# joejep/FOCNeRF

Measured on AMD Instinct MI355X. Metric: train_samples_per_sec, higher is better.
Workload: dtype f16

## Files before the change

focnerf_amd/_lib.py:

```python
import ctypes
import os

import torch

_HERE = os.path.dirname(os.path.abspath(__file__))
LIB_PATH = os.environ.get("FOCNERF_LIB_PATH") or os.path.join(_HERE, "libfocnerf_hip.so")

c_u8p = ctypes.c_void_p
c_vp = ctypes.c_void_p
u32 = ctypes.c_uint32
u64 = ctypes.c_uint64
f32 = ctypes.c_float
f64 = ctypes.c_double
i32 = ctypes.c_int

FOC_F32 = 0
FOC_F16 = 1
FOC_U8 = 2


class FocOccTrainNode(ctypes.Structure):
    _fields_ = [
        ("struct_bytes", u32),
        ("n_rays", u32), ("max_steps", u32), ("cascade", u32), ("grid_size", u32), ("cap", u32), ("pad_align", u32),
# ... 153 lines not shown
                                                      u32, i32, u32, i32, i32, c_vp, c_vp, u64, c_vp]),
    "foc_grad_total_variation": (i32, [c_vp, c_vp, c_vp, c_vp, f32, u32, u32, u32, u32, f32, u32, u32, i32, i32, c_vp]),
    "foc_freq_encode_forward": (i32, [c_vp, u32, u32, u32, u32, c_vp, c_vp]),
    "foc_freq_encode_backward": (i32, [c_vp, c_vp, u32, u32, u32, u32, c_vp, c_vp]),
    "foc_ffmlp_forward": (i32, [c_vp, c_vp, u32, u32, u32, u32, u32, u32, u32, c_vp, c_vp, c_vp]),
    "foc_ffmlp_inference": (i32, [c_vp, c_vp, u32, u32, u32, u32, u32, u32, u32, c_vp, c_vp, c_vp]),
    "foc_ffmlp_backward": (i32, [c_vp, c_vp, c_vp, c_vp, u32, u32, u32, u32, u32, u32, u32, i32,
                                 c_vp, c_vp, c_vp, c_vp, u64, c_vp]),
    "foc_ffmlp_backward_workspace_bytes": (u64, [u32, u32, u32]),
    "foc_ffmlp_forward_planar": (i32, [c_vp, c_vp, u32, u32, u32, u32, u32, u32, u32, c_vp, c_vp]),
    "foc_ffmlp_backward_planar": (i32, [c_vp, c_vp, c_vp, u32, u32, u32, u32, u32, u32, u32, i32, c_vp, c_vp, c_vp, u64, c_vp]),
    "foc_allocate_splitk": (i32, [u64]),
    "foc_free_splitk": (i32, []),
    "foc_combine_select": (i32, [c_vp, c_vp, c_vp, c_vp, u64, c_vp]),
    "foc_combine_pack_keys": (i32, [c_vp, u32, c_vp, u64, c_vp]),
    "foc_combine_unpack": (i32, [c_vp, u32, c_vp, c_vp, c_vp, u64, c_vp]),
    "foc_combine_select_composite": (i32, [c_vp, u32, c_vp, c_vp, u32, u32, c_vp, u32, c_vp, c_vp, c_vp, c_vp]),
    "foc_combine_select4": (i32, [c_vp, c_vp, u64, c_vp]),
    "foc_combine_select_composite_attr": (i32, [c_vp, u32, c_vp, c_vp, u32, c_vp, c_vp, u32, u32, c_vp, u32, c_vp, c_vp, c_vp, c_vp, c_vp, c_vp, c_vp, c_vp]),
    "foc_combine_select_composite_culled": (i32, [ctypes.POINTER(FocCulledField), u32, u32, c_vp, u32, c_vp, c_vp, u32, u32, c_vp, u32, c_vp, c_vp, c_vp, c_vp,
                                                  c_vp, c_vp, c_vp, c_vp]),
    "foc_combine_select4_ids": (i32, [c_vp, u32, c_vp, c_vp, u64, c_vp]),
    "foc_mo_select": (i32, [c_vp, c_vp, c_vp, c_vp, u64, u32, u32, c_vp]),
    "foc_fixed_field_pack": (i32, [c_vp, c_vp, c_vp, c_vp, c_vp, c_vp, f32, u32, u32, f32, f32, c_vp, c_vp, c_vp, c_vp, u32, c_vp]),
    "foc_fixed_cull_scratch_bytes": (u64, [u32, u32]),
    "foc_fixed_cull": (i32, [c_vp, c_vp, c_vp, c_vp, c_vp, u32, u32, f32, c_vp, u32, u32, c_vp, c_vp, c_vp, c_vp, u64, c_vp]),
    "foc_fixed_cull_emit": (i32, [c_vp, c_vp, c_vp, c_vp, c_vp, u32, u32, f32, c_vp, c_vp, u32, c_vp, c_vp, c_vp]),
    "foc_fixed_field_pack_culled": (i32, [c_vp, c_vp, c_vp, c_vp, u32, c_vp, c_vp, u32, u32, f32, f32, c_vp, c_vp]),
    "foc_fixed_cull_placed": (i32, [c_vp, c_vp, c_vp, c_vp, c_vp, u32, u32, c_vp, c_vp, f32, c_vp, u32, u32, c_vp, c_vp, c_vp, c_vp, u64, c_vp]),
    "foc_fixed_cull_emit_placed": (i32, [c_vp, c_vp, c_vp, c_vp, c_vp, u32, u32, c_vp, f32, f32, c_vp, c_vp, u32, c_vp, c_vp, c_vp]),
    "foc_fixed_field_pack_culled_gain": (i32, [c_vp, c_vp, c_vp, c_vp, u32, c_vp, c_vp, u32, u32, f32, f32, f32, c_vp, c_vp]),
    "foc_composite_fixed_steps":(i32, [c_vp, c_vp, c_vp, c_vp, u32, u32, f32, c_vp, c_vp, c_vp]),
    "foc_fixed_sample": (i32, [c_vp, c_vp, c_vp, c_vp, c_vp, c_vp, u32, u32, f32, c_vp, c_vp, c_vp, u32, c_vp]),
    "foc_fixed_tail_forward": (i32, [c_vp, c_vp, c_vp, c_vp, c_vp, c_vp, f32, u32, u32, f32, f32, c_vp, c_vp, c_vp, c_vp, c_vp, c_vp, u32, c_vp, c_vp]),
    "foc_fixed_tail_backward": (i32, [c_vp, c_vp, c_vp, c_vp, c_vp, c_vp, c_vp, c_vp, c_vp, c_vp, c_vp, f32, u32, u32, f32, f32, c_vp, c_vp, u32, c_vp, c_vp]),
    "foc_fixed_tail_forward_dist": (i32, [c_vp, c_vp, c_vp, c_vp, c_vp, c_vp, f32, u32, u32, f32, f32, c_vp, c_vp, c_vp, c_vp, c_vp, c_vp, u32, c_vp, c_vp,
                                          c_vp, c_vp]),
    "foc_fixed_tail_backward_dist": (i32, [c_vp, c_vp, c_vp, c_vp, c_vp, c_vp, c_vp, c_vp, c_vp, c_vp, c_vp, c_vp, f32, u32, u32, f32, f32, c_vp, c_vp, u32,
                                           c_vp, c_vp, c_vp, c_vp, c_vp]),
    "foc_fixed_head_forward": (i32, [c_vp, c_vp, c_vp, c_vp, c_vp, u32, u32, f32, c_vp, c_vp, c_vp, c_vp, c_vp, c_vp, c_vp, u32, c_vp]),
    "foc_fixed_head_backward": (i32, [c_vp, c_vp, c_vp, c_vp, c_vp, c_vp, c_vp, c_vp, c_vp, c_vp, u32, u32, f32, c_vp, u32, c_vp]),
    "foc_color_head_forward": (i32, [c_vp, c_vp, u32, c_vp, u32, u32, u32, u32, c_vp, u32, c_vp, c_vp]),
    "foc_field_forward_train": (i32, [c_vp, c_vp, u32, c_vp, u32, c_vp, u32, u32, u32, u32, c_vp, c_vp, u32, c_vp, c_vp]),
    "foc_color_head_backward": (i32, [c_vp, c_vp, c_vp, u32, c_vp, c_vp, u32, u32, u32, u32, c_vp, c_vp, c_vp, u64, u32, c_vp, c_vp, c_vp]),
    "foc_color_head_forward_pad": (i32, [c_vp, c_vp, u32, c_vp, u32, u32, u32, u32, c_vp, u32, c_vp, f32, c_vp]),
    "foc_color_head_backward_pad": (i32, [c_vp, c_vp, c_vp, u32, c_vp, c_vp, u32, u32, u32, u32, c_vp, c_vp, c_vp, u64, u32, c_vp, c_vp, f32, c_vp]),
    "foc_field_forward_train_pad": (i32, [c_vp, c_vp, u32, c_vp, u32, c_vp, u32, u32, u32, u32, c_vp, c_vp, u32, c_vp, f32, c_vp]),
    "foc_color_head_forward_pad31": (i32, [c_vp, c_vp, u32, c_vp, u32, u32, u32, u32, c_vp, u32, c_vp, f32, c_vp]),
    "foc_color_head_backward_pad31": (i32, [c_vp, c_vp, c_vp, u32, c_vp, c_vp, u32, u32, u32, u32, c_vp, c_vp, c_vp, u64, u32, c_vp, c_vp, f32, c_vp]),
    "foc_field_forward_train_pad31": (i32, [c_vp, c_vp, u32, c_vp, u32, c_vp, u32, u32, u32, u32, c_vp, c_vp, u32, c_vp, f32, c_vp]),
    "foc_fixed_composite_forward": (i32, [c_vp, c_vp, c_vp, f32, u32, u32, f32, c_vp, c_vp]),
    "foc_fixed_composite_backward": (i32, [c_vp, c_vp, c_vp, c_vp, f32, u32, u32, f32, c_vp, c_vp, c_vp]),
    "foc_sample_head_forward": (i32, [c_vp, c_vp, u64, c_vp, c_vp, c_vp, u32, c_vp]),
    "foc_sample_head_backward": (i32, [c_vp, c_vp, c_vp, u64, c_vp, u32, c_vp]),
    "foc_sh_encode": (i32, [c_vp, u64, c_vp, c_vp]),
    "foc_rgb_head_forward": (i32, [c_vp, u64, c_vp, c_vp]),
    "foc_rgb_head_backward": (i32, [c_vp, c_vp, u64, c_vp, c_vp]),
    "foc_fixed_render_inference": (i32, [c_vp, c_vp, c_vp, c_vp, c_vp, c_vp, f32, u32, u32, f32, f32, c_vp, c_vp, c_vp, c_vp, u32, c_vp, c_vp]),
    "foc_nerf_field_inference": (i32, [c_vp, i32, c_vp, u32, u32, u32, c_vp, u32, c_vp, u32, u32, u32, u32, c_vp, c_vp, c_vp, c_vp]),
    "foc_nerf_field_inference_pad": (i32, [c_vp, i32, c_vp, u32, u32, u32, c_vp, u32, c_vp, u32, u32, u32, u32, c_vp, c_vp, c_vp, f32, c_vp]),
    "foc_nerf_field_inference_pad31": (i32, [c_vp, i32, c_vp, u32, u32, u32, c_vp, u32, c_vp, u32, u32, u32, u32, c_vp, c_vp, c_vp, f32, c_vp]),
    "foc_field_normals": (i32, [c_vp, u32, c_vp, c_vp, u32, u32, u32, f32, u32, u32, i32, u32, i32, c_vp, c_vp, u32, u32, u32, c_vp, c_vp, c_vp, c_vp, c_vp,
                                c_vp]),
    "foc_mark_untrained_grid": (i32, [c_vp, u32, f32, f32, f32, f32, f32, u32, u32, c_vp, c_vp, c_vp]),
    "foc_grid_cells_xyz": (i32, [u32, u32, f32, c_vp, c_vp, c_vp]),
    "foc_grid_update_sample_workspace_bytes": (u64, [u32, u32]),
    "foc_grid_update_sample": (i32, [c_vp, u32, u32, f32, u32, c_vp, c_vp, c_vp, c_vp, c_vp, c_vp, u64, c_vp]),
    "foc_grid_update_apply_workspace_bytes": (u64, [u32, u32]),
    "foc_grid_update_apply": (i32, [c_vp, u32, u32, c_vp, c_vp, u32, f32, f32, f32, c_vp, c_vp, c_vp, u64, c_vp]),
    "foc_background_forward": (i32, [c_vp, c_vp, c_vp, f32, u32, c_vp, c_vp, f32, u32, c_vp, c_vp, c_vp]),
    "foc_background_backward_workspace_bytes": (u64, [u32]),
    "foc_background_backward": (i32, [c_vp, c_vp, c_vp, c_vp, f32, u32, c_vp, c_vp, f32, u32, c_vp, c_vp, c_vp, c_vp, u64, c_vp]),
    "foc_mc_workspace_bytes": (u64, [u32, u32, u32]),
    "foc_mc_count": (i32, [c_vp, u32, u32, u32, f32, c_vp, c_vp, c_vp]),
    "foc_mc_emit": (i32, [c_vp, u32, u32, u32, f32, c_vp, c_vp, c_vp, c_vp, c_vp, c_vp, c_vp]),
    "foc_lattice_cull_scratch_bytes": (u64, [u32]),
    "foc_lattice_cull": (i32, [c_vp, c_vp, c_vp, u32, u32, u32, u32, u32, c_vp, c_vp, f32, c_vp, u32, u32, c_vp, c_vp, c_vp, c_vp, u64, c_vp]),
    "foc_lattice_cull_emit": (i32, [c_vp, c_vp, c_vp, u32, u32, u32, u32, u32, c_vp, c_vp, c_vp, u32, c_vp, c_vp]),
    "foc_volume_scatter_max": (i32, [c_vp, c_vp, c_vp, f32, c_vp, u32, c_vp]),
    "foc_score_workspace_bytes": (u64, [u32, u32, u32]),
    "foc_score_quantize": (i32, [c_vp, c_vp, c_vp, c_vp, u32, u32, u32, c_vp, c_vp, c_vp, c_vp]),
    "foc_score_view": (i32, [c_vp, c_vp, u32, u32, u32, c_vp, u32, f64, f64, c_vp, c_vp, u64, c_vp]),
    "foc_optim_workspace_bytes": (ctypes.c_size_t, [i32]),
# ... 16 lines not shown
    try:
        lib = ctypes.CDLL(LIB_PATH)
    except OSError as e:
        raise ImportError(f"focnerf_amd: failed to load {LIB_PATH}: {e}") from e
    for name, (res, args) in SIGNATURES.items():
        fn = getattr(lib, name)
        fn.restype = res
        fn.argtypes = args
    return lib


class _Stream(ctypes.c_void_p):
    device_index = None


_multi_device = None


def _on_tensor_device(fn):
    def call(*args):
        global _multi_device
        if _multi_device is None:
            _multi_device = torch.cuda.device_count() > 1
        if _multi_device and args:
            idx = getattr(args[-1], "device_index", None)
            if idx is not None and idx != torch.cuda.current_device():
                with torch.cuda.device(idx):
                    return fn(*args)
        return fn(*args)
    call.__name__ = getattr(fn, "__name__", "foc_call")
    return call


class _Lib:

    def __init__(self, cdll):
        self._cdll = cdll
        for name, (_, args) in SIGNATURES.items():
            fn = getattr(cdll, name)
            setattr(self, name, _on_tensor_device(fn) if args and args[-1] is c_vp and not name.endswith("_bytes") else fn)


lib = _Lib(_load())


def check(rc, what=""):
    if rc != 0:
        msg = lib.foc_last_error().decode("utf-8", "replace")
        raise RuntimeError(f"focnerf_amd {what}: {msg} (code {rc})")


def ptr(t):
    if t is None:
        return None
    return ctypes.c_void_p(t.data_ptr())


_raw_stream = getattr(torch._C, "_cuda_getCurrentRawStream", None) if os.environ.get("FOC_RAW_STREAM", "1") != "0" else None


def raw_stream(index):
    if _raw_stream is not None:
        return _raw_stream(index)
    return torch.cuda.current_stream(index).cuda_stream


def stream_of(t=None):
    dev = t.device if t is not None else None
    index = dev.index if dev is not None and dev.index is not None else torch.cuda.current_device()
    s = _Stream(raw_stream(index))
    s.device_index = index
    return s

# ... 39 lines not shown
```

focnerf_amd/csrc/combine.hip:

```cpp
#include "common.h"
#include "fs_common.h"
#include <string.h>
#include <cmath>

static thread_local char g_err[512] = "";

void foc_set_error(const char *fmt, ...) {
    va_list ap;
    va_start(ap, fmt);
    vsnprintf(g_err, sizeof(g_err), fmt, ap);
    va_end(ap);
}

__global__ void __launch_bounds__(256) k_combine_select(const float *__restrict__ dens, const float *__restrict__ rgb,
                                                        float *__restrict__ max_dens, float *__restrict__ best_rgb, uint64_t n) {
    for (uint64_t i = (uint64_t)blockIdx.x * 256 + threadIdx.x; i < n; i += (uint64_t)gridDim.x * 256) {
        const float d = dens[i], m = max_dens[i];
        if (d > m) { best_rgb[i * 3] = rgb[i * 3]; best_rgb[i * 3 + 1] = rgb[i * 3 + 1]; best_rgb[i * 3 + 2] = rgb[i * 3 + 2]; }
        max_dens[i] = (d != d || m != m) ? __builtin_nanf("") : (d > m ? d : m);
    }
}

__global__ void __launch_bounds__(256) k_combine_pack(const float *__restrict__ dens, uint32_t rank, uint64_t *__restrict__ keys, uint64_t n) {
    for (uint64_t i = (uint64_t)blockIdx.x * 256 + threadIdx.x; i < n; i += (uint64_t)gridDim.x * 256) {
// ... 327 lines not shown
        best.x = (f.x != f.x || m != m) ? __builtin_nanf("") : (f.x > m ? f.x : m);
        acc4[i] = best;
    }
}

template <typename T>
__global__ void __launch_bounds__(256) k_mo_select(const T *__restrict__ sig_new, const T *__restrict__ feat_new, T *__restrict__ sig_best,
                                                   T *__restrict__ feat_best, uint64_t n, uint32_t width) {
    const uint64_t s0 = ((uint64_t)blockIdx.x * 4u + (threadIdx.x >> 6)) * 64u;
    if (s0 >= n) return;
    const uint32_t lane = threadIdx.x & 63u;
    bool take = false;
    if (s0 + lane < n) {
        const T a_raw = sig_new[s0 + lane];
        const float a = (float)a_raw, b = (float)sig_best[s0 + lane];
        take = (a != a) || (b == b && a >= b);
        if (take) sig_best[s0 + lane] = a_raw;
    }
    const uint64_t rows = __ballot(take);
    const uint32_t live = (uint32_t)(n - s0 < 64u ? n - s0 : 64u);
    const uint64_t base = s0 * width;
    for (uint32_t e = lane; e < live * width; e += 64u)
        if ((rows >> (e / width)) & 1ull) feat_best[base + e] = feat_new[base + e];
}

#include <stdlib.h>
#include <string.h>
#include <atomic>
#include <mutex>
struct FocOptionRow { const char *name; std::atomic<int> value; };
static FocOptionRow foc_option_table[FOC_OPT_COUNT] = {
    {"FOC_MLP_BWD_FUSED", 1}, {"FOC_FIELD_FWD_FUSED", 1}, {"FOC_GB_MERGE_MAX_RES", 480}, {"FOC_GB_FACTORED", 1}, {"FOC_GB_TAIL_SPLIT", 16}, {"FOC_GRID_FUSE_SMALL", 1},
    {"FOC_GRID_PAIRS", 1}, {"FOC_GRID_FAST", 1}, {"FOC_MARCH_SERIAL", -1}, {"FOC_MARCH_RAYS_ROW_MAX", 131072}, {"FOC_OCC_MARCH_FORM", -1},
    {"FOC_OCC_SAMPLE_MAJOR", 1}, {"FOC_OCC_FIELD_PIECE", 1 << 23}, {"FOC_DETERMINISTIC", 0},
};
static int foc_option_parse(int which, const char *text) {
    if (which == FOC_OPT_OCC_MARCH_FORM) {
        if (text[0] == 't') return 0;
        if (text[0] == 'r') return 1;
        if (text[0] == 'l') return 2;
        if (text[0] == 's') return 3;
    }
    return atoi(text);
}
static void foc_options_init() {
    static std::once_flag once;
    std::call_once(once, [] {
        for (int i = 0; i < FOC_OPT_COUNT; i++) {
            const char *e = getenv(foc_option_table[i].name);
            if (e && e[0]) foc_option_table[i].value.store(foc_option_parse(i, e), std::memory_order_relaxed);
        }
    });
}
int foc_opt(FocOpt which) { foc_options_init(); return foc_option_table[which].value.load(std::memory_order_relaxed); }

extern "C" {

int foc_set_option(const char *name, int value) {
    foc_options_init();
    for (int i = 0; i < FOC_OPT_COUNT; i++)
        if (name && strcmp(name, foc_option_table[i].name) == 0) { foc_option_table[i].value.store(value, std::memory_order_relaxed); return FOC_OK; }
    foc_set_error("set_option: unknown option '%s'", name ? name : "(null)");
    return FOC_E_INVALID;
}

int foc_get_option(const char *name, int *value) {
    foc_options_init();
// ... 213 lines not shown
```

focnerf_amd/csrc/common.h:

```cpp
#pragma once
#include <hip/hip_runtime.h>
#include <hip/hip_fp16.h>
#include <stdint.h>
#include <stdio.h>
#include <stdarg.h>
#include "../../include/focnerf.h"

#define FOC_WAVE 64

void foc_set_error(const char *fmt, ...);

enum FocOpt {
    FOC_OPT_MLP_BWD_FUSED,
    FOC_OPT_FIELD_FWD_FUSED,
    FOC_OPT_GB_MERGE_MAX_RES,
    FOC_OPT_GB_FACTORED,
    FOC_OPT_GB_TAIL_SPLIT,
    FOC_OPT_GRID_FUSE_SMALL,
    FOC_OPT_GRID_PAIRS,
    FOC_OPT_GRID_FAST,
    FOC_OPT_MARCH_SERIAL,
    FOC_OPT_MARCH_RAYS_ROW_MAX,
    FOC_OPT_OCC_MARCH_FORM,
    FOC_OPT_OCC_SAMPLE_MAJOR,
    FOC_OPT_OCC_FIELD_PIECE,
    FOC_OPT_DETERMINISTIC,
    FOC_OPT_COUNT
};
int foc_opt(FocOpt which);

#define FOC_REQUIRE(cond, code, ...)                    \
    do {                                                \
        if (!(cond)) {                                  \
            foc_set_error(__VA_ARGS__);                 \
            return (code);                              \
        }                                               \
    } while (0)

#define FOC_CHECK_LAUNCH(name)                                                     \
    do {                                                                           \
        hipError_t e_ = hipGetLastError();                                         \
        if (e_ != hipSuccess) {                                                    \
            foc_set_error("%s: launch failed: %s", name, hipGetErrorString(e_));   \
            return FOC_E_LAUNCH;                                                   \
        }                                                                          \
    } while (0)

static inline int foc_guard_pick(bool stream_is_null, int stream_device, int pointer_device, int current_device) {
    if (!stream_is_null && stream_device >= 0) return stream_device;
    if (pointer_device >= 0) return pointer_device;
    return current_device;
}
struct FocDeviceGuard {
    int prev = -1;
    explicit FocDeviceGuard(void *stream, const void *first_pointer = nullptr) {
        static int n_devices = -1;
        if (n_devices < 0 && hipGetDeviceCount(&n_devices) != hipSuccess) { (void)hipGetLastError(); n_devices = 0; }
        if (n_devices == 1) return;
        int cur = 0;
// ... 83 lines not shown
```

focnerf_amd/csrc/ffmlp.hip:

```cpp
#include "common.h"
#include "activations.h"
#include <stdlib.h>

#include <type_traits>
#include "mlp_common.h"

template <int HIDDEN, int NB, bool TRAIN, int IMODE, bool GEN = false>
__global__ void __launch_bounds__(MLP_BLOCK, 2) k_mlp_fwd(const _Float16 *__restrict__ inputs, const _Float16 *__restrict__ weights,
                                                       _Float16 *__restrict__ fwd_buf, _Float16 *__restrict__ outputs,
                                                       uint32_t B, uint32_t in_dim, uint32_t num_layers, int act, MlpHead hd) {
    const int relu = act == FOC_ACT_RELU;
    constexpr int MT = (HIDDEN + 31) / 32, KC = HIDDEN / 16;
    constexpr bool planar = IMODE == 1;
    extern __shared__ __attribute__((aligned(16))) _Float16 lds[];
    const uint32_t KS0 = IMODE == 2 ? 2u : in_dim / 16;
    const uint32_t f_hidden = MT * KS0, f_out = f_hidden + (num_layers - 1) * MT * KC;
    const float *obj_bias = reinterpret_cast<const float *>(lds + (size_t)(f_out + KC) * 512);
    if constexpr (IMODE == 2) {
        stage_weights_fwd<HIDDEN>(weights, lds, in_dim, num_layers, true, head_ld0(hd));
        if (head_bias(hd)) stage_head_bias(weights, hd, const_cast<float *>(obj_bias), HIDDEN);
    } else stage_weights_fwd<HIDDEN>(weights, lds, in_dim, num_layers);
    __syncthreads();

    const uint32_t lane = threadIdx.x & 63, wave = threadIdx.x >> 6;
// ... 301 lines not shown
                    if (!(o < OUT)) av = u32x4{0u, 0u, 0u, 0u};
                    if (!(i < IN)) bv = u32x4{0u, 0u, 0u, 0u};
                    acc[t] = mfma16(__builtin_bit_cast(h8, av), __builtin_bit_cast(h8, bv), acc[t]);
                }
            }
        }
    }
#pragma unroll
    for (int t = 0; t < 4; t++) {
        const uint32_t tile = wave + t * MLP_WAVES + 16 * blockIdx.z;
        if (tile < n_out_tiles) {
            const uint32_t mt = tile / NTi, nt = tile % NTi;
            const uint32_t i = 32 * nt + r;
#pragma unroll
            for (int reg = 0; reg < 16; reg++) {
                const uint32_t o = 32 * mt + acc_row(reg, h);
                if (o < OUT && i < IN) (void)__hip_atomic_fetch_add(ws + ws_off + (uint64_t)o * IN + i, acc[t][reg], __ATOMIC_RELAXED, __HIP_MEMORY_SCOPE_AGENT);
            }
        }
    }
}

__global__ void __launch_bounds__(256) k_mlp_dw_finalize(const float *__restrict__ ws, _Float16 *__restrict__ gw, uint32_t n) {
    for (uint32_t i = blockIdx.x * 256 + threadIdx.x; i < n; i += gridDim.x * 256) gw[i] = (_Float16)ws[i];
}
__global__ void __launch_bounds__(256) k_mlp_dw_finalize_slots(const float *__restrict__ ws, uint32_t slots, uint64_t stride, _Float16 *__restrict__ gw, uint32_t n) {
    for (uint32_t i = blockIdx.x * 256 + threadIdx.x; i < n; i += gridDim.x * 256) {
        float v = 0.0f;
        for (uint32_t k = 0; k < slots; k++) v += ws[k * stride + i];
        gw[i] = (_Float16)v;
    }
}

template <int HIDDEN, int NL, int NB, bool RECOMP, int IMODE, bool RELU_CT, bool IN32 = false, bool LEAN = false>
__global__ void __launch_bounds__(MLP_BLOCK, 2) k_mlp_bwd_fused(const _Float16 *__restrict__ grad, const _Float16 *__restrict__ inputs,
                                                             const _Float16 *__restrict__ weights, const _Float16 *__restrict__ fwd_buf,
                                                             _Float16 *__restrict__ bwd_buf_arg, _Float16 *__restrict__ grad_inputs, float *__restrict__ ws,
                                                             uint32_t B, uint32_t in_dim, int relu_rt, uint32_t lds_w_halfs, MlpHead hd) {
    const int relu = RELU_CT ? 1 : relu_rt;
    f16v FZ;
#pragma unroll
    for (int e = 0; e < 16; e++) FZ[e] = 0.0f;
    constexpr int MT = (HIDDEN + 31) / 32, KC = HIDDEN / 16, RW = 32 * NB;
    constexpr bool planar = IMODE == 1, HEAD = IMODE >= 2, NARROW = IMODE == 3;
    static_assert(!HEAD || RECOMP, "the head input modes have no stored-activation form");
    constexpr int WD = (HIDDEN < 32 ? 32 : HIDDEN) + 8;
    extern __shared__ __attribute__((aligned(16))) _Float16 lds[];
    const bool with_dx = LEAN ? true : grad_inputs != nullptr;
    _Float16 *const bwd_buf = LEAN ? nullptr : bwd_buf_arg;
    uint32_t ld0 = in_dim;
    bool has_obj = false;
    if constexpr (HEAD) { ld0 = head_ld0(hd); has_obj = hd.obj != nullptr; }
    bool col31_set = false;
    _Float16 col31 = (_Float16)0.0f;
    if constexpr (HEAD) { col31_set = head_bias(hd); col31 = has_obj ? (_Float16)1.0f : (_Float16)hd.pad; }
    stage_weights_bwd<HIDDEN>(weights, lds, in_dim, NL, with_dx, HEAD, ld0);
    const uint32_t WA = (in_dim > (uint32_t)HIDDEN ? in_dim : (uint32_t)(HIDDEN < 32 ? 32 : HIDDEN)) + 8;
    _Float16 *sD = lds + lds_w_halfs;
    _Float16 *sA = sD + 4 * RW * WD;
    _Float16 *ldsF = sA + 4 * RW * WA;
    const float *obj_bias = reinterpret_cast<const float *>(ldsF + (size_t)(((HIDDEN + 31) / 32) * (in_dim / 16) + (NL - 1) * ((HIDDEN + 31) / 32) * (HIDDEN / 16)) * 512);
    if constexpr (RECOMP) {
        stage_weights_fwd<HIDDEN>(weights, ldsF, in_dim, NL, false, ld0);
        if constexpr (HEAD) { if (head_bias(hd)) stage_head_bias(weights, hd, const_cast<float *>(obj_bias), HIDDEN); }
    }
    __syncthreads();

    const uint32_t lane = threadIdx.x & 63, wave = threadIdx.x >> 6;
    const int c = lane & 31, h = lane >> 5;
    const uint32_t MT0 = (HEAD || IN32) ? 1u : (in_dim + 31) / 32;
    const uint32_t f_hidden = MT, f_dx = MT + (NL - 1) * MT * KC;
    _Float16 *myD = sD + wave * RW * WD, *myA = sA + wave * RW * WA;

    f16v dwacc[NL + 1];
#pragma unroll
    for (int s = 0; s <= NL; s++)
#pragma unroll
        for (int e = 0; e < 16; e++) dwacc[s][e] = 0.0f;

    const uint32_t rows_per_group = 4 * RW;
    const uint32_t n_groups = (B + rows_per_group - 1) / rows_per_group;
    constexpr int KS0M = (HEAD || IN32) ? 2 : 4;
    const uint32_t KS0 = HEAD ? 2u : in_dim / 16;
    h8 g_nxt[(RW * 2 + 63) / 64];
    h8 x_nxt[KS0M][NB];
    _Float16 h0_nxt[NB];
    uint32_t hx_nxt[NB];
    static_assert((RW * 2) % 64 == 0, "a wave's grad rows are whole 64-lane passes");
    auto fetch_group = [&](uint32_t grp) {
        const uint64_t r0 = (uint64_t)grp * rows_per_group + wave * RW;
        if constexpr (HEAD) {
#pragma unroll
            for (int nb = 0; nb < NB; nb++) {
                const uint64_t row = min(r0 + nb * 32 + c, (uint64_t)B - 1);
                const _Float16 *p = hd.grad_h0 ? hd.grad_h0 + row : grad;
                h0_nxt[nb] = *p;
            }
// ... 334 lines not shown
                        }
            }
            __builtin_amdgcn_s_setprio(0);
#ifndef FOC_TIMING_NO_BARRIER
            foc_lds_barrier();
#endif
        }
    }
    float *slot = ws + (uint64_t)blockIdx.x * ((NL + 1) * MLP_DW_SLOT_STAGE);
    float *meet = reinterpret_cast<float *>(sD);
#pragma unroll
    for (int s = 0; s <= NL; s++) {
        const uint32_t OUT = s == 0 ? 16u : (uint32_t)HIDDEN;
        const uint32_t IN = s < NL ? (uint32_t)HIDDEN : in_dim;
        const uint32_t ntile = ((OUT + 31) / 32) * ((IN + 31) / 32), ksplit = (ntile * 2 <= 4) ? 2u : 1u;
        if (ksplit == 2u) {
            __syncthreads();
            if (wave >= ntile && wave < 2u * ntile) {
#pragma unroll
                for (int reg = 0; reg < 16; reg++) meet[((wave - ntile) * 16 + reg) * 64 + lane] = dwacc[s][reg];
            }
            __syncthreads();
            if (wave < ntile) {
#pragma unroll
                for (int reg = 0; reg < 16; reg++) slot[(s * 4 + wave) * 1024 + reg * 64 + lane] = dwacc[s][reg] + meet[(wave * 16 + reg) * 64 + lane];
            }
        } else if (wave < ntile) {
#pragma unroll
            for (int reg = 0; reg < 16; reg++) slot[(s * 4 + wave) * 1024 + reg * 64 + lane] = dwacc[s][reg];
        }
    }
}

template <int HIDDEN>
__global__ void __launch_bounds__(1024) k_mlp_dw_reduce(const float *__restrict__ slots, uint32_t n_slots, uint32_t NL, uint32_t in_dim, uint32_t ld0,
                                                        _Float16 *__restrict__ gw, float *__restrict__ wsb) {
    __shared__ float part[16][64];
    const uint32_t lane = threadIdx.x & 63, slice = threadIdx.x >> 6;
    const uint32_t s = blockIdx.x / 64, w = (blockIdx.x / 16) % 4, reg = blockIdx.x % 16;
    const uint32_t OUT = s == 0 ? 16u : (uint32_t)HIDDEN, IN = s < NL ? (uint32_t)HIDDEN : in_dim;
    const uint32_t NTi = (IN + 31) / 32, MTo = (OUT + 31) / 32, ntile = MTo * NTi, ksplit = 1u;
    if (w >= ntile) return;
    const uint32_t mt = w / NTi, nt = w % NTi, h = lane >> 5;
    const uint32_t o = 32 * mt + (uint32_t)acc_row((int)reg, (int)h), i = 32 * nt + (lane & 31);
    if (!(o < OUT) && !(32 * mt + (uint32_t)acc_row((int)reg, 1 - (int)h) < OUT)) return;
    const uint64_t stride = (uint64_t)(NL + 1) * MLP_DW_SLOT_STAGE;
    const float *p = slots + (uint64_t)(s * 4 + w) * 1024 + reg * 64 + lane;
    float a0 = 0.f, a1 = 0.f, a2 = 0.f, a3 = 0.f;
    for (uint32_t k = 0; k < ksplit; k++) {
        const float *q = p + (uint64_t)k * ntile * 1024;
        uint32_t g = slice;
        for (; g + 48 < n_slots; g += 64) {
            a0 += q[(uint64_t)g * stride]; a1 += q[(uint64_t)(g + 16) * stride]; a2 += q[(uint64_t)(g + 32) * stride]; a3 += q[(uint64_t)(g + 48) * stride];
        }
        for (; g < n_slots; g += 16) a0 += q[(uint64_t)g * stride];
    }
    part[slice][lane] = (a0 + a1) + (a2 + a3);
    __syncthreads();
    if (slice == 0 && o < OUT && i < IN) {
        float v = 0.f;
#pragma unroll
        for (int k = 0; k < 16; k++) v += part[k][lane];
        const uint64_t first = (uint64_t)HIDDEN * ld0, lsz = (uint64_t)HIDDEN * HIDDEN;
        const uint32_t fl = NL - s;
        const uint64_t off = (s == 0 ? first + (uint64_t)(NL - 1) * lsz : (fl == 0 ? 0 : first + (uint64_t)(fl - 1) * lsz)) + (uint64_t)o * (s == NL ? ld0 : IN) + i;
        if (wsb) wsb[off] = v; else gw[off] = (_Float16)v;
    }
}

__global__ void __launch_bounds__(256) k_mlp_dw_finalize_obj(const float *__restrict__ ws, _Float16 *__restrict__ gw, uint32_t n, uint32_t hidden,
                                                             const _Float16 *__restrict__ W, const _Float16 *__restrict__ obj, float *__restrict__ grad_obj,
                                                             float pad) {
    const uint32_t n0 = hidden * HEAD_OBJ_LD;
    for (uint32_t i = blockIdx.x * 256 + threadIdx.x; i < n; i += gridDim.x * 256) {
        float v = ws[i];
        if (i < n0) {
            const uint32_t o = i / HEAD_OBJ_LD, col = i % HEAD_OBJ_LD;
            if (col >= 31) v = col < 47 ? ws[o * HEAD_OBJ_LD + 31] * (float)obj[col - 31] : (pad != 0.0f ? ws[o * HEAD_OBJ_LD + 31] * pad : 0.0f);
        }
        gw[i] = (_Float16)v;
    }
    if (blockIdx.x == 0 && threadIdx.x < 16 && grad_obj) {
        float a = 0.0f;
        for (uint32_t o = 0; o < hidden; o++) a = fmaf((float)W[o * HEAD_OBJ_LD + 31 + threadIdx.x], ws[o * HEAD_OBJ_LD + 31], a);
        grad_obj[threadIdx.x] = a;
    }
}

__device__ __forceinline__ void nf_sh16_half(float x, float y, float z, int h, h8 &out) {
    const float xy = x * y, xz = x * z, yz = y * z, x2 = x * x, y2 = y * y, z2 = z * z;
    float o[8];
    if (h == 0) {
        o[0] = 0.28209479177387814f; o[1] = -0.48860251190291987f * y; o[2] = 0.48860251190291987f * z; o[3] = -0.48860251190291987f * x;
        o[4] = 1.0925484305920792f * xy; o[5] = -1.0925484305920792f * yz; o[6] = 0.94617469575755997f * z2 - 0.31539156525251999f;
        o[7] = -1.0925484305920792f * xz;
    } else {
        o[0] = 0.54627421529603959f * x2 - 0.54627421529603959f * y2; o[1] = 0.59004358992664352f * y * (-3.0f * x2 + y2);
        o[2] = 2.8906114426405538f * xy * z; o[3] = 0.45704579946446572f * y * (1.0f - 5.0f * z2);
        o[4] = 0.3731763325901154f * z * (5.0f * z2 - 3.0f); o[5] = 0.45704579946446572f * x * (1.0f - 5.0f * z2);
// ... 277 lines not shown
    if (lds > 64 * 1024) (void)hipFuncSetAttribute(reinterpret_cast<const void *>(kern), hipFuncAttributeMaxDynamicSharedMemorySize, (int)lds);
    const uint32_t n_tiles = foc_div_up(B, 32 * NB);
    uint32_t grid = foc_div_up(n_tiles, MLP_WAVES);
    const uint32_t cap = mlp_num_cus() * mlp_resident_blocks(reinterpret_cast<const void *>(kern), lds);
    if (grid > cap) grid = cap;
    hipLaunchKernelGGL(kern, dim3(grid), dim3(MLP_BLOCK), lds, st, (const _Float16 *)inputs, (const _Float16 *)weights, (_Float16 *)fwd_buf,
                       (_Float16 *)outputs, B, in_dim, num_layers, act, head ? *head : MlpHead{nullptr, nullptr, 1u, 16u, nullptr, 0.0f});
    FOC_CHECK_LAUNCH(TRAIN ? "ffmlp_forward" : "ffmlp_inference");
    return FOC_OK;
}

template <bool TRAIN>
static int mlp_fwd(const void *inputs, const void *weights, uint32_t B, uint32_t input_dim, uint32_t output_dim, uint32_t hidden_dim,
                   uint32_t num_layers, uint32_t activation, uint32_t output_activation, void *buffer, void *outputs, void *stream, int planar = 0) {
    const char *who = TRAIN ? "ffmlp_forward" : "ffmlp_inference";
    int rc = mlp_check(who, B, input_dim, output_dim, hidden_dim, num_layers, activation, output_activation);
    if (rc) return rc;
    if (B == 0) return FOC_OK;
    FOC_REQUIRE(inputs && weights && outputs && (!TRAIN || buffer), FOC_E_INVALID, "%s: null pointer", who);
    const int act = (int)activation;
    hipStream_t st = (hipStream_t)stream;
    switch (hidden_dim) {
        case 16: return mlp_fwd_launch<16, TRAIN>(inputs, weights, B, input_dim, num_layers, act, buffer, outputs, planar, st);
        case 32: return mlp_fwd_launch<32, TRAIN>(inputs, weights, B, input_dim, num_layers, act, buffer, outputs, planar, st);
        case 64: return mlp_fwd_launch<64, TRAIN>(inputs, weights, B, input_dim, num_layers, act, buffer, outputs, planar, st);
        case 128: return mlp_fwd_launch<128, TRAIN>(inputs, weights, B, input_dim, num_layers, act, buffer, outputs, planar, st);
        case 256:
            FOC_REQUIRE(!planar, FOC_E_INVALID, "%s: planar inputs are served up to hidden_dim 128", who);
            return mlp_wide_forward(TRAIN, inputs, weights, B, input_dim, 256, num_layers, act, buffer, outputs, st);
    }
    return FOC_E_INVALID;
}

template <int HIDDEN, int NL>
static int mlp_bwd_fused_launch(const void *grad, const void *inputs, const void *weights, const void *fwd_buf, uint32_t B, uint32_t in_dim, int relu,
                                void *bwd_buf, void *grad_inputs, void *grad_weights, float *ws, int planar, hipStream_t st, const MlpHead *head = nullptr,
                                float *grad_obj = nullptr) {
    FOC_REQUIRE(!planar || fwd_buf == nullptr, FOC_E_INVALID, "ffmlp_backward: planar inputs need the re-evaluating form (forward_buffer NULL)");
    constexpr int NB = 1, RW = 32 * NB, WD = (HIDDEN < 32 ? 32 : HIDDEN) + 8;
    const bool dx = grad_inputs != nullptr;
    const size_t lds_w = mlp_bwd_lds<HIDDEN>(in_dim, NL, dx);
    const uint32_t WA = (in_dim > (uint32_t)HIDDEN ? in_dim : (uint32_t)(HIDDEN < 32 ? 32 : HIDDEN)) + 8;
    const bool recomp = fwd_buf == nullptr;
    constexpr int MT = (HIDDEN + 31) / 32, KC = HIDDEN / 16;
    const bool has_obj = head && head->obj;
    const size_t lds = lds_w + (size_t)4 * RW * (WD + WA) * sizeof(_Float16) + (recomp ? (size_t)(MT * (in_dim / 16) + (NL - 1) * MT * KC) * 1024 : 0) +
                       (head && head_bias(*head) ? 256 : 0);
    FOC_REQUIRE(lds <= 160 * 1024, FOC_E_INVALID, "ffmlp_backward: fused kernel needs %zu B of LDS", lds);
#ifdef FOC_TIMING_ONE_WG
    const size_t lds_launch = lds < 84 * 1024 ? 84 * 1024 : lds;
#else
    const size_t lds_launch = lds;
#endif
    auto kern = recomp ? (planar ? (relu ? k_mlp_bwd_fused<HIDDEN, NL, NB, true, 1, true> : k_mlp_bwd_fused<HIDDEN, NL, NB, true, 1, false>)
                                 : (relu ? k_mlp_bwd_fused<HIDDEN, NL, NB, true, 0, true> : k_mlp_bwd_fused<HIDDEN, NL, NB, true, 0, false>))
                       : k_mlp_bwd_fused<HIDDEN, NL, NB, false, 0, false>;
    const bool lean = !bwd_buf && dx;
    if constexpr (HIDDEN == 64) {
        if (recomp && relu && in_dim <= 32 && !head) {
            if (lean) kern = planar ? k_mlp_bwd_fused<HIDDEN, NL, NB, true, 1, true, true, true> : k_mlp_bwd_fused<HIDDEN, NL, NB, true, 0, true, true, true>;
            else kern = planar ? k_mlp_bwd_fused<HIDDEN, NL, NB, true, 1, true, true> : k_mlp_bwd_fused<HIDDEN, NL, NB, true, 0, true, true>;
        }
    }
    if constexpr (HIDDEN == 64 && NL >= 2 && NL <= 3) {
        if (head) kern = head->out_width == 4u ? (relu ? (lean ? k_mlp_bwd_fused<HIDDEN, NL, NB, true, 3, true, false, true> : k_mlp_bwd_fused<HIDDEN, NL, NB, true, 3, true>)
                                                       : k_mlp_bwd_fused<HIDDEN, NL, NB, true, 3, false>)
                                               : (relu ? (lean ? k_mlp_bwd_fused<HIDDEN, NL, NB, true, 2, true, false, true> : k_mlp_bwd_fused<HIDDEN, NL, NB, true, 2, true>)
                                                       : k_mlp_bwd_fused<HIDDEN, NL, NB, true, 2, false>);
    }
    else FOC_REQUIRE(!head, FOC_E_INVALID, "color_head_backward: hidden_dim must be 64 and num_layers 2 or 3");
    if (lds_launch > 64 * 1024) (void)hipFuncSetAttribute(reinterpret_cast<const void *>(kern), hipFuncAttributeMaxDynamicSharedMemorySize, (int)lds_launch);
    const uint32_t n_w = HIDDEN * ((has_obj ? HEAD_OBJ_LD : in_dim) + HIDDEN * (NL - 1) + 16);
    uint32_t grid = foc_div_up(B, 4 * RW);
    const uint32_t cap = min(mlp_num_cus() * 2, MLP_DW_MAX_SLOTS);
    if (grid > cap) grid = cap;
    float *slots = ws + mlp_dw_blob_floats(has_obj ? HEAD_OBJ_LD : in_dim, HIDDEN, NL);
    hipLaunchKernelGGL(kern, dim3(grid), dim3(MLP_BLOCK), lds_launch, st, (const _Float16 *)grad, (const _Float16 *)inputs, (const _Float16 *)weights,
                       (const _Float16 *)fwd_buf, (_Float16 *)bwd_buf, (_Float16 *)grad_inputs, slots, B, in_dim, relu, (uint32_t)(lds_w / sizeof(_Float16)),
                       head ? *head : MlpHead{nullptr, nullptr, 1u, 16u, nullptr, 0.0f});
    FOC_CHECK_LAUNCH("ffmlp_backward(fused)");
    hipLaunchKernelGGL((k_mlp_dw_reduce<HIDDEN>), dim3((NL + 1) * 64), dim3(1024), 0, st, (const float *)slots, grid, (uint32_t)NL, in_dim,
                       has_obj ? (uint32_t)HEAD_OBJ_LD : in_dim, (_Float16 *)grad_weights, has_obj ? ws : (float *)nullptr);
    FOC_CHECK_LAUNCH("ffmlp_backward(reduce)");
    if (has_obj) {
        hipLaunchKernelGGL(k_mlp_dw_finalize_obj, dim3(foc_grid_1d(n_w, 256)), dim3(256), 0, st, ws, (_Float16 *)grad_weights, n_w, (uint32_t)HIDDEN,
                           (const _Float16 *)weights, head->obj, grad_obj, head->pad);
        FOC_CHECK_LAUNCH("ffmlp_backward(finalize)");
    }
    return FOC_OK;
}

template <int HIDDEN>
static int mlp_dw_launch(const void *grad, const void *inputs, const void *fwd_buf, const void *bwd_buf, uint32_t B, uint32_t in_dim, uint32_t num_layers,
                         void *grad_weights, float *ws, bool det, hipStream_t st) {
    const uint32_t n_w = HIDDEN * (in_dim + HIDDEN * (num_layers - 1) + 16);
    const uint64_t det_stride = det ? mlp_dw_blob_floats(in_dim, HIDDEN, num_layers) : 0;
    uint32_t gx = foc_div_up(B, DW_CHUNK);
    if (det && gx > MLP_DW_DET_SLOTS) gx = MLP_DW_DET_SLOTS;
    if (foc_zero_async(ws, det ? (size_t)gx * det_stride * sizeof(float) : (size_t)n_w * sizeof(float), st) != hipSuccess) { foc_set_error("ffmlp_backward: memset of workspace failed"); return FOC_E_LAUNCH; }
    const int wgs_per_cu = 8;
    const uint32_t tiles = ((HIDDEN + 31) / 32) * ((max((uint32_t)HIDDEN, in_dim) + 31) / 32), GZ = (tiles + 15) / 16;
    const uint32_t capx = foc_div_up(mlp_num_cus() * (uint32_t)wgs_per_cu, (num_layers + 1) * GZ);
    if (gx > capx) gx = capx;
    if (gx < 1) gx = 1;
    auto kern = k_mlp_dw<HIDDEN>;
    if constexpr (HIDDEN <= 128) { if (in_dim > 128) kern = k_mlp_dw<HIDDEN, 256>; }
    hipLaunchKernelGGL(kern, dim3(gx, num_layers + 1, GZ), dim3(MLP_BLOCK), 0, st, (const _Float16 *)grad, (const _Float16 *)inputs,
                       (const _Float16 *)fwd_buf, (const _Float16 *)bwd_buf, ws, B, in_dim, num_layers, det_stride);
    FOC_CHECK_LAUNCH("ffmlp_backward(weights)");
    if (det) hipLaunchKernelGGL(k_mlp_dw_finalize_slots, dim3(foc_grid_1d(n_w, 256)), dim3(256), 0, st, ws, gx, det_stride, (_Float16 *)grad_weights, n_w);
    else hipLaunchKernelGGL(k_mlp_dw_finalize, dim3(foc_grid_1d(n_w, 256)), dim3(256), 0, st, ws, (_Float16 *)grad_weights, n_w);
    FOC_CHECK_LAUNCH("ffmlp_backward(finalize)");
    return FOC_OK;
}

// ... 256 lines not shown
                "color_head_backward: workspace of %llu bytes, foc_ffmlp_backward_workspace_bytes(%u, 64, %u) asks for %llu", (unsigned long long)workspace_bytes,
                obj_feat ? HEAD_OBJ_LD : 32u, num_layers, (unsigned long long)foc_ffmlp_backward_workspace_bytes(obj_feat ? HEAD_OBJ_LD : 32u, 64, num_layers));
    FOC_REQUIRE(out_width == 16 || out_width == 4, FOC_E_INVALID, "color_head_backward: out_width must be 16 or 4 (got %u)", out_width);
    FOC_REQUIRE(activation == FOC_ACT_RELU || activation == FOC_ACT_NONE, FOC_E_INVALID, "color_head_backward: hidden activation must be relu(0) or none(6)");
    rc = head_pad_check("color_head_backward", pad31, obj_feat, input_pad);
    if (rc) return rc;
    const MlpHead hd{(const _Float16 *)ray_sh, (const _Float16 *)grad_h0, samples_per_ray, out_width, (const _Float16 *)obj_feat, input_pad};
    const int relu = activation == 0;
    if (num_layers == 2) return mlp_bwd_fused_launch<64, 2>(grad, h, weights, nullptr, B, 32, relu, nullptr, grad_h, grad_weights, (float *)workspace, 0, (hipStream_t)stream, &hd, grad_obj);
    return mlp_bwd_fused_launch<64, 3>(grad, h, weights, nullptr, B, 32, relu, nullptr, grad_h, grad_weights, (float *)workspace, 0, (hipStream_t)stream, &hd, grad_obj);
}

int foc_color_head_backward(const void *grad, const void *h, const void *ray_sh, uint32_t samples_per_ray, const void *grad_h0, const void *weights,
                            uint32_t B, uint32_t hidden_dim, uint32_t num_layers, uint32_t activation, void *grad_h, void *grad_weights, void *workspace,
                            uint64_t workspace_bytes, uint32_t out_width, const void *obj_feat, float *grad_obj, void *stream) {
    return color_head_backward(grad, h, ray_sh, samples_per_ray, grad_h0, weights, B, hidden_dim, num_layers, activation, grad_h, grad_weights, workspace,
                               workspace_bytes, out_width, obj_feat, grad_obj, 0.0f, false, stream);
}

int foc_color_head_backward_pad(const void *grad, const void *h, const void *ray_sh, uint32_t samples_per_ray, const void *grad_h0, const void *weights,
                                uint32_t B, uint32_t hidden_dim, uint32_t num_layers, uint32_t activation, void *grad_h, void *grad_weights, void *workspace,
                                uint64_t workspace_bytes, uint32_t out_width, const void *obj_feat, float *grad_obj, float input_pad, void *stream) {
    return color_head_backward(grad, h, ray_sh, samples_per_ray, grad_h0, weights, B, hidden_dim, num_layers, activation, grad_h, grad_weights, workspace,
                               workspace_bytes, out_width, obj_feat, grad_obj, input_pad, false, stream);
}

int foc_color_head_backward_pad31(const void *grad, const void *h, const void *ray_sh, uint32_t samples_per_ray, const void *grad_h0, const void *weights,
                                  uint32_t B, uint32_t hidden_dim, uint32_t num_layers, uint32_t activation, void *grad_h, void *grad_weights, void *workspace,
                                  uint64_t workspace_bytes, uint32_t out_width, const void *obj_feat, float *grad_obj, float input_pad, void *stream) {
    return color_head_backward(grad, h, ray_sh, samples_per_ray, grad_h0, weights, B, hidden_dim, num_layers, activation, grad_h, grad_weights, workspace,
                               workspace_bytes, out_width, obj_feat, grad_obj, input_pad, true, stream);
}

int foc_allocate_splitk(uint64_t size) { (void)size; return FOC_OK; }
int foc_free_splitk(void) { return FOC_OK; }

}
```

focnerf_amd/csrc/field_fwd.hip:

```cpp
#include "mlp_common.h"

typedef uint32_t ff_u2 __attribute__((ext_vector_type(2)));

__device__ __forceinline__ uint32_t ff_pack(float a, float b) {
    typedef _Float16 h2 __attribute__((ext_vector_type(2)));
    const h2 p = {(_Float16)a, (_Float16)b};
    return __builtin_bit_cast(uint32_t, p);
}

#ifndef FF_MIN_WAVES
#define FF_MIN_WAVES 2
#endif
template <int NLS, int NLC, bool RELU>
__global__ void __launch_bounds__(MLP_BLOCK, FF_MIN_WAVES) k_field_fwd_train(const _Float16 *__restrict__ planes, const _Float16 *__restrict__ w_sigma,
                                                               const _Float16 *__restrict__ w_color, _Float16 *__restrict__ h_out,
                                                               _Float16 *__restrict__ c_out, uint32_t B, MlpHead hd) {
    constexpr int HIDDEN = 64, MT = 2, KC = 4, KS0 = 2;
    constexpr int FS = MT * KS0 + (NLS - 1) * MT * KC + KC;
    constexpr int FC = MT * KS0 + (NLC - 1) * MT * KC + KC;
    extern __shared__ __attribute__((aligned(16))) _Float16 lds[];
    _Float16 *ldsS = lds, *ldsC = lds + FS * 512;
    const float *obj_bias = reinterpret_cast<const float *>(ldsC + FC * 512);
    stage_weights_fwd<HIDDEN>(w_sigma, ldsS, 32, NLS);
    stage_weights_fwd<HIDDEN>(w_color, ldsC, 32, NLC, true, head_ld0(hd));
    if (head_bias(hd)) stage_head_bias(w_color, hd, const_cast<float *>(obj_bias), HIDDEN);
    __syncthreads();

    const uint32_t lane = threadIdx.x & 63, wave = threadIdx.x >> 6;
    const int c = lane & 31, h = lane >> 5;
    const uint32_t n_tiles = (B + 31) / 32;
    const uint32_t tstride = gridDim.x * MLP_WAVES;
    uint32_t tile = blockIdx.x * MLP_WAVES + wave;
    h8 x_nxt[KS0], sh_nxt;
    auto fetch = [&](uint32_t t) {
#ifdef FF_TIMING_NO_LOAD
        const uint64_t r = (uint64_t)c + 0 * t;
#else
        const uint64_t r = min((uint64_t)min(t, n_tiles - 1u) * 32 + c, (uint64_t)B - 1);
#endif
#pragma unroll
        for (int kc = 0; kc < KS0; kc++) x_nxt[kc] = ld_planar8(planes, B, r, kc, h);
        sh_nxt = ld_head8(planes, hd, r, 0, h);
    };
    fetch(tile);
    for (; tile < n_tiles; tile += tstride) {
#ifndef FF_TIMING_HOIST
        asm volatile("" ::: "memory");
#endif
        const uint64_t row_raw = (uint64_t)tile * 32 + c;
        h8 x_cur[KS0];
#pragma unroll
        for (int kc = 0; kc < KS0; kc++) x_cur[kc] = x_nxt[kc];
        const h8 sh = sh_nxt;
        fetch(tile + tstride);
        f16v acc[MT];
#pragma unroll
        for (int mt = 0; mt < MT; mt++)
#pragma unroll
// ... 56 lines not shown
            if (l < (uint32_t)NLC) {
                const uint32_t fbase = MT * KS0 + (l - 1) * MT * KC;
#pragma unroll
                for (int mt = 0; mt < MT; mt++)
#pragma unroll
                    for (int e = 0; e < 16; e++) acc[mt][e] = 0.0f;
#pragma unroll
                for (int kc = 0; kc < KC; kc++)
#pragma unroll
                    for (int mt = 0; mt < MT; mt++) acc[mt] = mfma16(ld_frag(ldsC, fbase + mt * KC + kc, lane), bf[kc], acc[mt]);
            } else {
#pragma unroll
                for (int e = 0; e < 16; e++) o[e] = 0.0f;
#pragma unroll
                for (int kc = 0; kc < KC; kc++) o = mfma16(ld_frag(ldsC, FC - KC + kc, lane), bf[kc], o);
                if (hd.out_width == 4u) {
#ifdef FF_TIMING_NO_STORE
                    if (h == 0 && row_raw == 0xFFFFFFFFFFull) *reinterpret_cast<ff_u2 *>(c_out + row_raw * 4) = ff_u2{ff_pack(o[0], o[1]), ff_pack(o[2], o[3])};
#else
                    if (h == 0 && row_raw < B) *reinterpret_cast<ff_u2 *>(c_out + row_raw * 4) = ff_u2{ff_pack(o[0], o[1]), ff_pack(o[2], o[3])};
#endif
                } else store_tile<false>(c_out, 16, row_raw, B, 0, 16, o, h);
            }
        }
    }
}

static uint32_t ff_num_cus() {
    int dev = 0, n = 0;
    if (hipGetDevice(&dev) != hipSuccess || hipDeviceGetAttribute(&n, hipDeviceAttributeMultiprocessorCount, dev) != hipSuccess || n <= 0) n = 256;
    return (uint32_t)n;
}

template <int NLS, int NLC, bool RELU>
static int ff_launch(const void *planes, const void *w_sigma, const void *w_color, void *h, void *c, uint32_t B, const MlpHead &hd, hipStream_t st) {
    auto kern = k_field_fwd_train<NLS, NLC, RELU>;
    const size_t lds = (size_t)((4 + (NLS - 1) * 8 + 4) + (4 + (NLC - 1) * 8 + 4)) * 1024 + 256;
    if (lds > 64 * 1024) (void)hipFuncSetAttribute(reinterpret_cast<const void *>(kern), hipFuncAttributeMaxDynamicSharedMemorySize, (int)lds);
    static int resident = 0;
    if (!resident) {
        int n = 0;
        if (hipOccupancyMaxActiveBlocksPerMultiprocessor(&n, kern, MLP_BLOCK, lds) != hipSuccess || n < 1) n = 2;
        resident = n > 8 ? 8 : n;
    }
    uint32_t grid = foc_div_up(foc_div_up(B, 32), MLP_WAVES);
    const uint32_t cap = ff_num_cus() * (uint32_t)resident;
    if (grid > cap) grid = cap;
    hipLaunchKernelGGL(kern, dim3(grid), dim3(MLP_BLOCK), lds, st, (const _Float16 *)planes, (const _Float16 *)w_sigma, (const _Float16 *)w_color,
                       (_Float16 *)h, (_Float16 *)c, B, hd);
    FOC_CHECK_LAUNCH("field_forward_train");
    return FOC_OK;
}

template <int NLS, int NLC>
static int ff_launch_act(const void *planes, const void *w_sigma, const void *w_color, void *h, void *c, uint32_t B, int relu, const MlpHead &hd, hipStream_t st) {
    return relu ? ff_launch<NLS, NLC, true>(planes, w_sigma, w_color, h, c, B, hd, st) : ff_launch<NLS, NLC, false>(planes, w_sigma, w_color, h, c, B, hd, st);
}

int field_forward_train(const void *planes, const void *sigma_weights, uint32_t sigma_layers, const void *ray_sh, uint32_t samples_per_ray,
                        const void *color_weights, uint32_t color_layers, uint32_t hidden_dim, uint32_t activation, uint32_t B, void *h, void *c,
                        uint32_t out_width, const void *obj_feat, float input_pad, bool pad31, void *stream) {
    FocDeviceGuard foc_guard_(stream, planes);
    if (B == 0) return FOC_OK;
    FOC_REQUIRE(planes && sigma_weights && ray_sh && color_weights && h && c, FOC_E_INVALID, "field_forward_train: null pointer");
    FOC_REQUIRE(hidden_dim == 64 && samples_per_ray >= 1, FOC_E_INVALID, "field_forward_train: hidden_dim must be 64 (got %u), samples_per_ray >= 1", hidden_dim);
    FOC_REQUIRE(activation == FOC_ACT_RELU || activation == FOC_ACT_NONE, FOC_E_INVALID, "field_forward_train: hidden activation must be relu(0) or none(6)");
    FOC_REQUIRE(out_width == 16 || out_width == 4, FOC_E_INVALID, "field_forward_train: out_width must be 16 or 4 (got %u)", out_width);
    const int prc = head_pad_check("field_forward_train", pad31, obj_feat, input_pad);
    if (prc) return prc;
    const MlpHead hd{(const _Float16 *)ray_sh, nullptr, samples_per_ray, out_width, (const _Float16 *)obj_feat, input_pad};
    const int relu = activation == FOC_ACT_RELU;
    hipStream_t st = (hipStream_t)stream;
    switch (sigma_layers * 10 + color_layers) {
        case 12: return ff_launch_act<1, 2>(planes, sigma_weights, color_weights, h, c, B, relu, hd, st);
        case 13: return ff_launch_act<1, 3>(planes, sigma_weights, color_weights, h, c, B, relu, hd, st);
        case 22: return ff_launch_act<2, 2>(planes, sigma_weights, color_weights, h, c, B, relu, hd, st);
        case 23: return ff_launch_act<2, 3>(planes, sigma_weights, color_weights, h, c, B, relu, hd, st);
        case 33: return ff_launch_act<3, 3>(planes, sigma_weights, color_weights, h, c, B, relu, hd, st);
        default: foc_set_error("field_forward_train: layer counts (%u, %u) are not built (1/2, 1/3, 2/2, 2/3, 3/3)", sigma_layers, color_layers); return FOC_E_INVALID;
    }
}

extern "C" {

int foc_field_forward_train(const void *planes, const void *sigma_weights, uint32_t sigma_layers, const void *ray_sh, uint32_t samples_per_ray,
                            const void *color_weights, uint32_t color_layers, uint32_t hidden_dim, uint32_t activation, uint32_t B, void *h, void *c,
                            uint32_t out_width, const void *obj_feat, void *stream) {
    return field_forward_train(planes, sigma_weights, sigma_layers, ray_sh, samples_per_ray, color_weights, color_layers, hidden_dim, activation, B, h, c,
                               out_width, obj_feat, 0.0f, false, stream);
}

int foc_field_forward_train_pad(const void *planes, const void *sigma_weights, uint32_t sigma_layers, const void *ray_sh, uint32_t samples_per_ray,
                                const void *color_weights, uint32_t color_layers, uint32_t hidden_dim, uint32_t activation, uint32_t B, void *h, void *c,
                                uint32_t out_width, const void *obj_feat, float input_pad, void *stream) {
    return field_forward_train(planes, sigma_weights, sigma_layers, ray_sh, samples_per_ray, color_weights, color_layers, hidden_dim, activation, B, h, c,
                               out_width, obj_feat, input_pad, false, stream);
}

int foc_field_forward_train_pad31(const void *planes, const void *sigma_weights, uint32_t sigma_layers, const void *ray_sh, uint32_t samples_per_ray,
                                  const void *color_weights, uint32_t color_layers, uint32_t hidden_dim, uint32_t activation, uint32_t B, void *h, void *c,
                                  uint32_t out_width, const void *obj_feat, float input_pad, void *stream) {
    return field_forward_train(planes, sigma_weights, sigma_layers, ray_sh, samples_per_ray, color_weights, color_layers, hidden_dim, activation, B, h, c,
                               out_width, obj_feat, input_pad, true, stream);
}

}
```

focnerf_amd/csrc/fixedstep.hip:

```cpp
#include "common.h"
#include "fs_common.h"
#include <float.h>

__global__ void __launch_bounds__(256) k_fs_sample(const float *__restrict__ rays_o, const float *__restrict__ rays_d, const float *__restrict__ nears,
                                                   const float *__restrict__ fars, const float *__restrict__ aabb, const float *__restrict__ noise,
                                                   uint32_t N, uint32_t T, float bound, float *__restrict__ xyzs, float *__restrict__ enc_in,
                                                   _Float16 *__restrict__ ray_sh, uint32_t ray_block) {
    const uint64_t total = ray_block ? (uint64_t)((N + FS_RAY_BLOCK - 1) / FS_RAY_BLOCK) * FS_RAY_BLOCK * T : (uint64_t)N * T;
    const FsBox box = fs_box(aabb);
    const float two_b = 2 * bound;
    for (uint64_t s = (uint64_t)blockIdx.x * 256 + threadIdx.x; s < total; s += (uint64_t)gridDim.x * 256) {
        uint32_t n, i;
        bool own = true;
        if (ray_block) {
            const uint32_t blk = (uint32_t)(s / ((uint64_t)FS_RAY_BLOCK * T)), in = (uint32_t)(s - (uint64_t)blk * FS_RAY_BLOCK * T);
            i = in / FS_RAY_BLOCK;
            n = blk * FS_RAY_BLOCK + in % FS_RAY_BLOCK;
            own = n < N;
            n = own ? n : N - 1;
        } else {
            n = (uint32_t)(s / T); i = (uint32_t)(s - (uint64_t)n * T);
        }
        const FsGeom g = fs_geom(nears, fars, n, T);
        const float z = fs_z(g, i, T, noise, (uint64_t)n * T + i);
        float x, y, w;
        fs_point(rays_o[n * 3], rays_o[n * 3 + 1], rays_o[n * 3 + 2], rays_d[n * 3], rays_d[n * 3 + 1], rays_d[n * 3 + 2], z, box, x, y, w);
        if (xyzs) { xyzs[s * 3] = x; xyzs[s * 3 + 1] = y; xyzs[s * 3 + 2] = w; }
        if (enc_in) { enc_in[s * 3] = fs_norm(x, bound, two_b); enc_in[s * 3 + 1] = fs_norm(y, bound, two_b); enc_in[s * 3 + 2] = fs_norm(w, bound, two_b); }
        if (ray_sh && i == 0 && own) {
            h8 lo, hi;
            foc_sh16_h(rays_d[n * 3], rays_d[n * 3 + 1], rays_d[n * 3 + 2], lo, hi);
            h8 *dst = reinterpret_cast<h8 *>(ray_sh + (uint64_t)n * 16);
            dst[0] = lo; dst[1] = hi;
        }
    }
}

__global__ void __launch_bounds__(256) k_fs_head_fwd(const _Float16 *__restrict__ h, const float *__restrict__ rays_d, const float *__restrict__ nears,
                                                     const float *__restrict__ fars, const float *__restrict__ noise, uint32_t N, uint32_t T,
                                                     float density_scale, float *__restrict__ sigma_out, float *__restrict__ trans_out,
                                                     float *__restrict__ weights_out, float *__restrict__ weights_sum, float *__restrict__ depth,
                                                     _Float16 *__restrict__ cin, const _Float16 *__restrict__ obj, uint32_t cin_ld) {
    const uint32_t lane = threadIdx.x & 63;
    const uint32_t n = blockIdx.x * 4 + (threadIdx.x >> 6);
    if (n >= N) return;
    const FsGeom g = fs_geom(nears, fars, n, T);
    h8 shlo, shhi;
    h8 ob1 = {0, 0, 0, 0, 0, 0, 0, 0}, ob2 = {0, 0, 0, 0, 0, 0, 0, 0};
    _Float16 ob0 = (_Float16)0;
    if (cin) {
        foc_sh16_h(rays_d[n * 3], rays_d[n * 3 + 1], rays_d[n * 3 + 2], shlo, shhi);
        if (obj) {
            ob0 = obj[0];
#pragma unroll
            for (int k = 0; k < 8; k++) ob1[k] = obj[1 + k];
#pragma unroll
            for (int k = 0; k < 7; k++) ob2[k] = obj[9 + k];
        }
    }
    float Tc = 1.0f, ws = 0, dp = 0;
    for (uint32_t base = 0; base < T; base += 64) {
        const uint32_t i = base + lane;
        const bool valid = i < T;
        const uint64_t s = (uint64_t)n * T + (valid ? i : T - 1);
// ... 309 lines not shown
    const uint32_t fe = st->first_enc, W = fe ? N - fe + 2u : 0u;
    const uint32_t H = W ? N / W : 0u;
    const bool grid = W >= 16u && N % W == 0u && H >= 8u && st->count == 2u * (H - 1u) && st->bad == 0u;
    for (uint32_t p = blockIdx.x * 256 + threadIdx.x; p < N; p += gridDim.x * 256) {
        uint32_t src = p;
        if (grid) {
            const uint64_t wt = (uint64_t)W * th;
            const uint32_t ty = (uint32_t)(p / wt), rem = (uint32_t)(p - ty * wt);
            const uint32_t rows_here = min(th, H - ty * th);
            const uint32_t tx = min(rem / (rows_here * tw), (W - 1u) / tw), r2 = rem - tx * rows_here * tw;
            const uint32_t cols_here = min(tw, W - tx * tw);
            src = (ty * th + r2 / cols_here) * W + tx * tw + r2 % cols_here;
        }
        perm[p] = (int64_t)src;
    }
}

extern "C" {

int foc_fixed_sample(const float *rays_o, const float *rays_d, const float *nears, const float *fars, const float *aabb, const float *noise,
                     uint32_t N, uint32_t T, float bound, float *xyzs, float *enc_in, void *ray_sh, uint32_t ray_block, void *stream) {
    FocDeviceGuard foc_guard_(stream, rays_o);
    if (N == 0) return FOC_OK;
    FOC_REQUIRE(rays_o && rays_d && nears && fars && aabb && (xyzs || enc_in), FOC_E_INVALID, "fixed_sample: null pointer");
    FOC_REQUIRE(T >= 2, FOC_E_INVALID, "fixed_sample: T must be >= 2");
    FOC_REQUIRE(ray_block == 0 || ray_block == FS_RAY_BLOCK, FOC_E_INVALID, "fixed_sample: ray_block must be 0 (ray-major) or %u (got %u)", FS_RAY_BLOCK, ray_block);
    const uint64_t rows = ray_block ? (uint64_t)foc_div_up(N, FS_RAY_BLOCK) * FS_RAY_BLOCK * T : (uint64_t)N * T;
    hipLaunchKernelGGL(k_fs_sample, dim3(foc_grid_1d(rows, 256, 256 * 16)), dim3(256), 0, (hipStream_t)stream, rays_o, rays_d, nears, fars, aabb,
                       noise, N, T, bound, xyzs, enc_in, (_Float16 *)ray_sh, ray_block);
    FOC_CHECK_LAUNCH("fixed_sample");
    return FOC_OK;
}

int foc_fixed_head_forward(const void *h, const float *rays_d, const float *nears, const float *fars, const float *noise, uint32_t N, uint32_t T,
                           float density_scale, float *sigma, float *trans, float *weights, float *weights_sum, float *depth, void *cin,
                           const void *obj_feat, uint32_t cin_width, void *stream) {
    FocDeviceGuard foc_guard_(stream, h);
    if (N == 0) return FOC_OK;
    FOC_REQUIRE(h && rays_d && nears && fars && sigma && trans && weights && weights_sum && depth, FOC_E_INVALID, "fixed_head_forward: null pointer");
    FOC_REQUIRE(T >= 2, FOC_E_INVALID, "fixed_head_forward: T must be >= 2");
    FOC_REQUIRE(cin_width == 32 || cin_width == 48, FOC_E_INVALID, "fixed_head_forward: cin_width must be 32 or 48 (got %u)", cin_width);
    FOC_REQUIRE(!obj_feat || cin_width == 48, FOC_E_INVALID, "fixed_head_forward: an object feature needs the 48-wide colour input");
    hipLaunchKernelGGL(k_fs_head_fwd, dim3(foc_div_up(N, 4)), dim3(256), 0, (hipStream_t)stream, (const _Float16 *)h, rays_d, nears, fars, noise, N, T,
                       density_scale, sigma, trans, weights, weights_sum, depth, (_Float16 *)cin, (const _Float16 *)obj_feat, cin_width);
    FOC_CHECK_LAUNCH("fixed_head_forward");
    return FOC_OK;
}

int foc_fixed_head_backward(const void *h, const float *sigma, const float *trans, const float *nears, const float *fars, const float *noise,
                            const float *grad_w, const float *grad_ws, const float *grad_depth, const void *grad_cin, uint32_t N, uint32_t T,
                            float density_scale, void *grad_h, uint32_t cin_width, void *stream) {
    FocDeviceGuard foc_guard_(stream, h);
    if (N == 0) return FOC_OK;
    FOC_REQUIRE(h && sigma && trans && nears && fars && grad_h, FOC_E_INVALID, "fixed_head_backward: null pointer");
    FOC_REQUIRE(T >= 2, FOC_E_INVALID, "fixed_head_backward: T must be >= 2");
    FOC_REQUIRE(cin_width == 32 || cin_width == 48, FOC_E_INVALID, "fixed_head_backward: cin_width must be 32 or 48 (got %u)", cin_width);
    hipLaunchKernelGGL(k_fs_head_bwd, dim3(foc_div_up(N, 4)), dim3(256), 0, (hipStream_t)stream, (const _Float16 *)h, sigma, trans, nears, fars, noise,
                       grad_w, grad_ws, grad_depth, (const _Float16 *)grad_cin, N, T, density_scale, (_Float16 *)grad_h, cin_width);
    FOC_CHECK_LAUNCH("fixed_head_backward");
    return FOC_OK;
}

int foc_fixed_composite_forward(const void *c, const float *weights, const float *bg_ray, float bg_scalar, uint32_t N, uint32_t T, float thresh,
                                float *image, void *stream) {
    FocDeviceGuard foc_guard_(stream, c);
    if (N == 0) return FOC_OK;
// ... 149 lines not shown
```

focnerf_amd/csrc/fs_common.h:

```cpp
#pragma once
#include "common.h"
#include "sample_math.h"

struct FsGeom { float near, far, span, sample_dist, step; };

#define FS_RAY_BLOCK 64u
__host__ __device__ __forceinline__ uint64_t fs_block_row(uint32_t n, uint32_t i, uint32_t T) {
    return (uint64_t)(n / FS_RAY_BLOCK) * FS_RAY_BLOCK * T + (uint64_t)i * FS_RAY_BLOCK + n % FS_RAY_BLOCK;
}

__device__ __forceinline__ FsGeom fs_geom(const float *__restrict__ nears, const float *__restrict__ fars, uint32_t n, uint32_t T) {
    FsGeom g;
    g.near = nears[n]; g.far = fars[n];
    g.span = g.far - g.near;
    g.sample_dist = g.span / (float)T;
    g.step = 1.0f / (float)(T - 1);
    return g;
}
__device__ __forceinline__ float fs_z0(const FsGeom &g, uint32_t i, uint32_t T) {
    const float lin = (i < T / 2) ? (g.step * (float)i) : fmaf(-g.step, (float)(T - 1 - i), 1.0f);
    return g.near + g.span * lin;
}
__device__ __forceinline__ float fs_jitter(const FsGeom &g, float z, float u) { return z + (u - 0.5f) * g.sample_dist; }
__device__ __forceinline__ float fs_z(const FsGeom &g, uint32_t i, uint32_t T, const float *__restrict__ noise, uint64_t s) {
    float z = fs_z0(g, i, T);
    if (noise) z = fs_jitter(g, z, noise[s]);
    return z;
}
__device__ __forceinline__ float fs_zu(const FsGeom &g, uint32_t i, uint32_t T, bool jitter, float u) {
    float z = fs_z0(g, i, T);
    if (jitter) z = fs_jitter(g, z, u);
    return z;
}

struct FsSample { float z, delta, oz; };
__device__ __forceinline__ FsSample fs_sample(const FsGeom &g, uint32_t i, uint32_t ic, uint32_t T, bool jitter, float u0, float u1) {
    FsSample p;
    p.z = fs_zu(g, ic, T, jitter, u0);
    p.delta = g.sample_dist;
    if (i + 1 < T) p.delta = fs_zu(g, i + 1, T, jitter, u1) - p.z;
    p.oz = (p.z - g.near) / g.span;
    p.oz = p.oz < 0.0f ? 0.0f : (p.oz > 1.0f ? 1.0f : p.oz);
    return p;
}
__device__ __forceinline__ FsSample fs_sample_ld(const FsGeom &g, uint32_t i, uint32_t ic, uint32_t T, const float *__restrict__ noise, uint64_t s) {
    const bool jitter = noise != nullptr;
    return fs_sample(g, i, ic, T, jitter, jitter ? noise[s] : 0.0f, jitter && i + 1 < T ? noise[s + 1] : 0.0f);
}

__device__ __forceinline__ float fs_trans_scan(float om, uint32_t lane, float &Tc) {
// ... 102 lines not shown
```

focnerf_amd/csrc/mlp_common.h:

```cpp
#pragma once
#include "common.h"
#include "activations.h"

typedef _Float16 h8 __attribute__((ext_vector_type(8)));
typedef _Float16 h4 __attribute__((ext_vector_type(4)));
typedef float f16v __attribute__((ext_vector_type(16)));
typedef short s4 __attribute__((__vector_size__(4 * sizeof(short))));
typedef __attribute__((address_space(3))) s4 lds_s4;
typedef uint32_t u32x2 __attribute__((ext_vector_type(2)));
typedef uint32_t u32x4 __attribute__((ext_vector_type(4)));

#define MLP_BLOCK 256
#define MLP_WAVES 4
#define MLP_DW_SLOT_STAGE 4096u
#define MLP_DW_MAX_SLOTS 1024u
#ifndef FOC_MLP_SETPRIO
#define FOC_MLP_SETPRIO 1
#endif

__device__ __forceinline__ int acc_row(int reg, int h) { return (reg & 3) + 8 * (reg >> 2) + 4 * h; }
__device__ __forceinline__ int chain_k(int kc, int h, int j) { return 16 * kc + 8 * (j >> 2) + 4 * h + (j & 3); }

__device__ __forceinline__ f16v mfma16(const h8 a, const h8 b, const f16v c) {
    return __builtin_amdgcn_mfma_f32_32x32x16_f16(a, b, c, 0, 0, 0);
// ... 100 lines not shown
}
__device__ __forceinline__ void stage_head_bias(const _Float16 *__restrict__ W0, const MlpHead &hd, float *bias, uint32_t hidden) {
    if (hd.obj) stage_obj_bias(W0, hd.obj, bias, hidden, hd.pad);
    else stage_pad31_bias(W0, hd.pad, bias, hidden);
}
__device__ __forceinline__ f16v ld_obj_bias(const float *bias, int mt, int h) {
    typedef float f4 __attribute__((ext_vector_type(4)));
    const f4 *p = reinterpret_cast<const f4 *>(bias + (mt * 2 + h) * 16);
    const f4 a = p[0], b = p[1], c = p[2], d = p[3];
    return f16v{a.x, a.y, a.z, a.w, b.x, b.y, b.z, b.w, c.x, c.y, c.z, c.w, d.x, d.y, d.z, d.w};
}
__device__ __forceinline__ void ld_head_raw(const _Float16 *__restrict__ hrows, uint64_t row, int h, u32x4 &v, uint32_t &nxt) {
    const uint32_t *p = reinterpret_cast<const uint32_t *>(hrows + row * 16) + 4 * h;
    v = *reinterpret_cast<const u32x4 *>(p);
    nxt = h == 0 ? p[4] : 0u;
}
__device__ __forceinline__ void ld_head_raw_all(const _Float16 *__restrict__ hrows, uint64_t row, int h, u32x4 &v, uint32_t &nxt) {
    const uint32_t *p = reinterpret_cast<const uint32_t *>(hrows + row * 16) + 4 * h;
    v = *reinterpret_cast<const u32x4 *>(p);
    nxt = p[h == 0 ? 4 : 3];
}
__device__ __forceinline__ h8 head_shift(const u32x4 v, uint32_t nxt) {
    const u32x4 r = {__builtin_amdgcn_alignbit(v.y, v.x, 16), __builtin_amdgcn_alignbit(v.z, v.y, 16), __builtin_amdgcn_alignbit(v.w, v.z, 16),
                     __builtin_amdgcn_alignbit(nxt, v.w, 16)};
    return __builtin_bit_cast(h8, r);
}
__device__ __forceinline__ h8 ld_head8(const _Float16 *__restrict__ hrows, const MlpHead &hd, uint64_t row, uint32_t kc, int h) {
    if (kc == 0) return *reinterpret_cast<const h8 *>(hd.ray_sh + (uint64_t)((uint32_t)row / hd.samples_per_ray) * 16 + 8 * h);
    u32x4 v; uint32_t nxt;
    ld_head_raw_all(hrows, row, h, v, nxt);
    return head_shift(v, h == 0 ? nxt : 0u);
}

template <int HIDDEN>
__device__ void stage_weights_fwd(const _Float16 *__restrict__ W, _Float16 *lds, uint32_t in_dim, uint32_t num_layers, bool with_out = true, uint32_t ld0 = 0) {
    constexpr int MT = (HIDDEN + 31) / 32, KC = HIDDEN / 16;
    const uint32_t KS0 = in_dim / 16;
    if (!ld0) ld0 = in_dim;
    const uint32_t n0 = MT * KS0, nh = (num_layers - 1) * MT * KC, total = n0 + nh + (with_out ? KC : 0);
    const _Float16 *Wh = W + (size_t)HIDDEN * ld0;
    const _Float16 *Wo = Wh + (size_t)(num_layers - 1) * HIDDEN * HIDDEN;
    for (uint32_t idx = threadIdx.x; idx < total * 64; idx += MLP_BLOCK) {
        const uint32_t f = idx >> 6, lane = idx & 63, r = lane & 31, h = lane >> 5;
        h8 v;
#pragma unroll
        for (int j = 0; j < 8; j++) v[j] = (_Float16)0;
        if (f < n0) {
            const uint32_t mt = f / KS0, kc = f % KS0, row = 32 * mt + r;
            if (row < HIDDEN) v = *reinterpret_cast<const h8 *>(W + (size_t)row * ld0 + 16 * kc + 8 * h);
        } else if (f < n0 + nh) {
            const uint32_t g = f - n0, l = g / (MT * KC), mt = (g / KC) % MT, kc = g % KC, row = 32 * mt + r;
            if (row < HIDDEN) {
                const _Float16 *p = Wh + (size_t)l * HIDDEN * HIDDEN + (size_t)row * HIDDEN + 16 * kc + 4 * h;
                const h4 lo = *reinterpret_cast<const h4 *>(p), hi = *reinterpret_cast<const h4 *>(p + 8);
#pragma unroll
                for (int j = 0; j < 4; j++) { v[j] = lo[j]; v[4 + j] = hi[j]; }
            }
        } else {
            const uint32_t kc = f - n0 - nh;
            if (r < 16) {
                const _Float16 *p = Wo + (size_t)r * HIDDEN + 16 * kc + 4 * h;
                const h4 lo = *reinterpret_cast<const h4 *>(p), hi = *reinterpret_cast<const h4 *>(p + 8);
#pragma unroll
                for (int j = 0; j < 4; j++) { v[j] = lo[j]; v[4 + j] = hi[j]; }
            }
        }
        *reinterpret_cast<h8 *>(lds + (size_t)f * 512 + lane * 8) = v;
    }
}

template <int HIDDEN>
__device__ void stage_weights_bwd(const _Float16 *__restrict__ W, _Float16 *lds, uint32_t in_dim, uint32_t num_layers, bool with_dx, bool head = false,
                                  uint32_t ld0 = 0) {
    constexpr int MT = (HIDDEN + 31) / 32, KC = HIDDEN / 16;
    const uint32_t MT0 = (in_dim + 31) / 32;
    if (!ld0) ld0 = in_dim;
    const uint32_t no = MT, nh = (num_layers - 1) * MT * KC, nx = with_dx ? MT0 * KC : 0, total = no + nh + nx;
    const _Float16 *Wh = W + (size_t)HIDDEN * ld0;
    const _Float16 *Wo = Wh + (size_t)(num_layers - 1) * HIDDEN * HIDDEN;
    for (uint32_t idx = threadIdx.x; idx < total * 64; idx += MLP_BLOCK) {
        const uint32_t f = idx >> 6, lane = idx & 63, r = lane & 31, h = lane >> 5;
        h8 v;
#pragma unroll
        for (int j = 0; j < 8; j++) v[j] = (_Float16)0;
        if (f < no) {
            const uint32_t i = 32 * f + r;
            if (i < HIDDEN) {
#pragma unroll
                for (int j = 0; j < 8; j++) v[j] = Wo[(size_t)(8 * h + j) * HIDDEN + i];
            }
        } else if (f < no + nh) {
            const uint32_t g = f - no, l = g / (MT * KC), mt = (g / KC) % MT, kc = g % KC, i = 32 * mt + r;
            if (i < HIDDEN) {
#pragma unroll
                for (int j = 0; j < 8; j++) v[j] = Wh[(size_t)l * HIDDEN * HIDDEN + (size_t)chain_k(kc, h, j) * HIDDEN + i];
            }
        } else {
            const uint32_t g = f - no - nh, mt0 = g / KC, kc = g % KC, i = 32 * mt0 + r;
            if (head) {
                if (i >= 17 && i < 32) {
#pragma unroll
                    for (int j = 0; j < 8; j++) v[j] = W[(size_t)chain_k(kc, h, j) * ld0 + (i - 1)];
                }
            } else if (i < in_dim) {
#pragma unroll
                for (int j = 0; j < 8; j++) v[j] = W[(size_t)chain_k(kc, h, j) * ld0 + i];
            }
        }
        *reinterpret_cast<h8 *>(lds + (size_t)f * 512 + lane * 8) = v;
    }
}

template <bool RELU>
__device__ __forceinline__ void store_tile(_Float16 *__restrict__ dst, uint32_t ld, uint64_t row, uint64_t nrows, uint32_t col0, uint32_t ncols,
                                           const f16v &acc, int h) {
    if (row >= nrows) return;
#pragma unroll
    for (int q = 0; q < 4; q++) {
        const uint32_t col = col0 + 8 * q + 4 * h;
        if (col < ncols) {
            h4 v;
#pragma unroll
            for (int e = 0; e < 4; e++) {
                _Float16 x = (_Float16)acc[4 * q + e];
                if (RELU) x = x > (_Float16)0 ? x : (_Float16)0;
                v[e] = x;
            }
            *reinterpret_cast<h4 *>(dst + row * ld + col) = v;
        }
    }
}

__device__ __forceinline__ void store_tile_act(_Float16 *__restrict__ dst, uint32_t ld, uint64_t row, uint64_t nrows, uint32_t col0, uint32_t ncols,
                                               const f16v &acc, int h, int act) {
    if (row >= nrows) return;
#pragma unroll
    for (int q = 0; q < 4; q++) {
        const uint32_t col = col0 + 8 * q + 4 * h;
        if (col < ncols) {
// ... 8 lines not shown
```

focnerf_amd/csrc/raymarching.hip:

```cpp
#include "common.h"
#include "occ_cell.h"
#include "sample_math.h"
#include "ragged.h"
#include <float.h>

#define RM_SQRT3 1.7320508075688772f
#define RM_RPI   0.3183098861837907f

__device__ __forceinline__ float rm_sign(float x) { return copysignf(1.0f, x); }

__device__ __forceinline__ void rm_near_far(float ox, float oy, float oz, float dx, float dy, float dz, float a0, float a1, float a2, float a3, float a4, float a5,
                                            float min_near, float &near_out, float &far_out) {
    const float rdx = 1 / dx, rdy = 1 / dy, rdz = 1 / dz;
    float near = (a0 - ox) * rdx, far = (a3 - ox) * rdx, t;
    if (near > far) { t = near; near = far; far = t; }
    float near_y = (a1 - oy) * rdy, far_y = (a4 - oy) * rdy;
    if (near_y > far_y) { t = near_y; near_y = far_y; far_y = t; }
    bool miss = (near > far_y || near_y > far);
    if (!miss) {
        if (near_y > near) near = near_y;
        if (far_y < far) far = far_y;
        float near_z = (a2 - oz) * rdz, far_z = (a5 - oz) * rdz;
        if (near_z > far_z) { t = near_z; near_z = far_z; far_z = t; }
        miss = (near > far_z || near_z > far);
        if (!miss) {
            if (near_z > near) near = near_z;
            if (far_z < far) far = far_z;
            if (near < min_near) near = min_near;
        }
    }
    near_out = miss ? FLT_MAX : near;
    far_out = miss ? FLT_MAX : far;
}

__global__ void __launch_bounds__(256) k_near_far_from_aabb(const float *__restrict__ rays_o, const float *__restrict__ rays_d,
                                     const float *__restrict__ aabb, uint32_t N, float min_near,
                                     float *__restrict__ nears, float *__restrict__ fars) {
    const float a0 = aabb[0], a1 = aabb[1], a2 = aabb[2], a3 = aabb[3], a4 = aabb[4], a5 = aabb[5];
    for (uint32_t n = blockIdx.x * blockDim.x + threadIdx.x; n < N; n += gridDim.x * blockDim.x) {
        float near, far;
        rm_near_far(rays_o[n * 3], rays_o[n * 3 + 1], rays_o[n * 3 + 2], rays_d[n * 3], rays_d[n * 3 + 1], rays_d[n * 3 + 2], a0, a1, a2, a3, a4, a5, min_near, near, far);
        nears[n] = near;
        fars[n] = far;
    }
}

__global__ void __launch_bounds__(256) k_sph_from_ray(const float *__restrict__ rays_o, const float *__restrict__ rays_d, float radius,
                               uint32_t N, float *__restrict__ coords) {
    for (uint32_t n = blockIdx.x * blockDim.x + threadIdx.x; n < N; n += gridDim.x * blockDim.x) {
        const float ox = rays_o[n * 3], oy = rays_o[n * 3 + 1], oz = rays_o[n * 3 + 2];
        const float dx = rays_d[n * 3], dy = rays_d[n * 3 + 1], dz = rays_d[n * 3 + 2];
        const float A = fmaf(dz, dz, fmaf(dy, dy, dx * dx));
        const float B = fmaf(oz, dz, fmaf(oy, dy, ox * dx));
        const float C = fmaf(-radius, radius, fmaf(oz, oz, fmaf(oy, oy, ox * ox)));
        const float t = (-B + sqrtf(fmaf(B, B, -(A * C)))) / A;
        const float x = fmaf(t, dx, ox), y = fmaf(t, dy, oy), z = fmaf(t, dz, oz);
        const float theta = atan2f(sqrtf(fmaf(z, z, x * x)), y);
        const float phi = atan2f(z, x);
        coords[n * 2] = fmaf(2 * theta, RM_RPI, -1.0f);
        coords[n * 2 + 1] = phi * RM_RPI;
    }
}

__global__ void __launch_bounds__(256) k_morton3D(const int32_t *__restrict__ coords, uint32_t N, int32_t *__restrict__ indices) {
    for (uint32_t n = blockIdx.x * blockDim.x + threadIdx.x; n < N; n += gridDim.x * blockDim.x)
        indices[n] = (int32_t)rm_morton3D((uint32_t)coords[n * 3], (uint32_t)coords[n * 3 + 1], (uint32_t)coords[n * 3 + 2]);
// ... 1153 lines not shown
```

focnerf_amd/csrc/sample_math.h:

```cpp
#pragma once
#include "common.h"

typedef _Float16 h8 __attribute__((ext_vector_type(8)));

__device__ __forceinline__ void foc_sh16(float x, float y, float z, float (&o)[16]) {
    const float xy = x * y, xz = x * z, yz = y * z, x2 = x * x, y2 = y * y, z2 = z * z;
    o[0] = 0.28209479177387814f;
    o[1] = -0.48860251190291987f * y;
    o[2] = 0.48860251190291987f * z;
    o[3] = -0.48860251190291987f * x;
    o[4] = 1.0925484305920792f * xy;
    o[5] = -1.0925484305920792f * yz;
    o[6] = 0.94617469575755997f * z2 - 0.31539156525251999f;
    o[7] = -1.0925484305920792f * xz;
    o[8] = 0.54627421529603959f * x2 - 0.54627421529603959f * y2;
    o[9] = 0.59004358992664352f * y * (-3.0f * x2 + y2);
    o[10] = 2.8906114426405538f * xy * z;
    o[11] = 0.45704579946446572f * y * (1.0f - 5.0f * z2);
    o[12] = 0.3731763325901154f * z * (5.0f * z2 - 3.0f);
    o[13] = 0.45704579946446572f * x * (1.0f - 5.0f * z2);
    o[14] = 1.4453057213202769f * z * (x2 - y2);
    o[15] = 0.59004358992664352f * x * (-x2 + 3.0f * y2);
}
__device__ __forceinline__ void foc_sh16_h(float x, float y, float z, h8 &lo, h8 &hi) {
    float sh[16];
    foc_sh16(x, y, z, sh);
#pragma unroll
    for (int k = 0; k < 8; k++) { lo[k] = foc_f2h(sh[k]); hi[k] = foc_f2h(sh[8 + k]); }
}

__device__ __forceinline__ float foc_sigmoid_h(float x) { return (float)(_Float16)(1.0f / (1.0f + expf(-x))); }

__device__ __forceinline__ float foc_clamp15(float x) { return x < -15.0f ? -15.0f : (x > 15.0f ? 15.0f : x); }
__device__ __forceinline__ float foc_trunc_exp_bwd(float x) { return expf(foc_clamp15(x)); }
__device__ __forceinline__ float foc_trunc_exp_bwd(float x, float e) {
    const float xc = foc_clamp15(x);
    return xc != x ? expf(xc) : e;
}
struct FocExp15 { float lo, hi; };
__device__ __forceinline__ FocExp15 foc_exp15() {
    float a = -15.0f, b = 15.0f;
    asm volatile("" : "+v"(a));
    asm volatile("" : "+v"(b));
    return FocExp15{expf(a), expf(b)};
}
__device__ __forceinline__ float foc_trunc_exp_bwd_of_sigma(float sigma, const FocExp15 &e) { return fminf(fmaxf(sigma, e.lo), e.hi); }

struct FocBg { float b0, b1, b2; };
__device__ __forceinline__ FocBg foc_bg(const float *__restrict__ bg_ray, float bg_scalar, uint32_t k) {
    return FocBg{bg_ray ? bg_ray[k * 3] : bg_scalar, bg_ray ? bg_ray[k * 3 + 1] : bg_scalar, bg_ray ? bg_ray[k * 3 + 2] : bg_scalar};
}
```

focnerf_amd/field.py:

```python
import os
from dataclasses import dataclass
from typing import Optional

import torch
from torch.autograd import Function
from torch.amp import custom_bwd, custom_fwd

from .backend import _gridencoder, _ffmlp
from .ffmlp import FFMLP, PackedMLP, single_pass_backward
from .gridencoder import GridEncoder, GridSpec


def fused_mlp(model, name):
    get = getattr(model, "fused_mlp", None)
    return get(name) if get is not None else getattr(model, name, None)


@dataclass(frozen=True)
class MlpShape:
    input_dim: int
    hidden_dim: int
    num_layers: int
    activation: int
    output_activation: int
    padded_output_dim: int

    @staticmethod
    def of(mlp):
        if not isinstance(mlp, (FFMLP, PackedMLP)):
            return None
        return MlpShape(mlp.input_dim, mlp.hidden_dim, mlp.num_layers, mlp.activation, mlp.output_activation, mlp.padded_output_dim)

    def blob_numel(self):
        return self.hidden_dim * (self.input_dim + self.hidden_dim * (self.num_layers - 1) + self.padded_output_dim)


@dataclass(frozen=True)
class FieldPlan:
    grid: Optional[GridSpec]
    levels: int
    sigma: Optional[MlpShape]
    colour: Optional[MlpShape]
    uses_object_feature: bool
    field: bool
    train_forward: bool
    tail: bool
    infer: bool
    occ: bool
    native_loop: bool
    head: bool
    colour_input_pad: float = 0.0
    background: bool = False
    occ_object: bool = False
    native_loop_object: bool = False
    normals: bool = False


def pad_twin(name, pad, obj):
    from ._lib import lib
    if pad == 0:
        return getattr(lib, name), ()
    return getattr(lib, name + ("_pad" if obj else "_pad31")), (float(pad),)


def object_feature_half(obj_feat, who):
    if obj_feat is None:
        return None
    obj16 = obj_feat.detach().reshape(-1).half().contiguous()
    if obj16.numel() != 16:
        raise RuntimeError(f"{who}: the encoded object feature has {obj16.numel()} elements, the colour head takes 16")
    return obj16


def _on(switch):
    return os.environ.get(switch, "1") != "0"


def field_plan(model):
    from ._lib import get_option
    from .shencoder import SHEncoder
    enc, enc_dir = getattr(model, "encoder", None), getattr(model, "encoder_dir", None)
    sigma, colour = MlpShape.of(fused_mlp(model, "sigma_net")), MlpShape.of(fused_mlp(model, "color_net"))
    obj = bool(getattr(model, "uses_object_feature", False))
    pad = float(getattr(model, "colour_input_pad", 0.0))
    grid = enc.spec() if isinstance(enc, GridEncoder) else None

    hash_grid = grid is not None and enc.input_dim == 3 and enc.level_dim == 2 and sigma is not None and sigma.input_dim == enc.output_dim
    plain_grid = grid is not None and grid.gridtype == 0 and not grid.align_corners and grid.interpolation == 0
    sigma_one_pass = sigma is not None and single_pass_backward(sigma.input_dim, sigma.hidden_dim, sigma.num_layers, sigma.activation)
    sigma_16 = sigma is not None and sigma.padded_output_dim == 16
    sigma_32_64 = sigma is not None and sigma.input_dim == 32 and sigma.hidden_dim == 64
    colour_in = 48 if obj else 32
    colour_64 = colour is not None and colour.input_dim == colour_in and colour.hidden_dim == 64 and colour.padded_output_dim == 16
    colour_rows = (isinstance(enc_dir, SHEncoder) and enc_dir.degree == 4 and getattr(model, "geo_feat_dim", 0) == 15
                   and (not obj or getattr(model, "yolo_encoding_dim", 0) == 16))
    colour_relu_or_none = colour is not None and colour.activation in (0, 6)
    both = sigma is not None and colour is not None
    same_activation = both and sigma.activation == colour.activation
    layer_pair = both and (sigma.num_layers, colour.num_layers) in ((1, 2), (1, 3), (2, 2), (2, 3), (3, 3))
    whole_field = sigma_32_64 and colour_64 and colour_rows and layer_pair and same_activation

    field = hash_grid and sigma_one_pass and sigma_16 and _on("FOC_FUSED_FIELD")
    tail = colour_64 and colour.num_layers in (2, 3) and colour_relu_or_none and colour_rows and _on("FOC_FUSED_TAIL")
    infer = field and whole_field and (not obj or sigma.activation == 0) and _on("FOC_FUSED_INFER")
    enc_bg, bg_mlp = getattr(model, "encoder_bg", None), fused_mlp(model, "bg_net")
    bg_grid = enc_bg.spec() if isinstance(enc_bg, GridEncoder) else None
    background = (bg_grid is not None and enc_bg.input_dim == 2 and enc_bg.level_dim == 2 and enc_bg.offsets.numel() == 5
                  and bg_grid.gridtype == 0 and not bg_grid.align_corners and bg_grid.interpolation == 0
                  and isinstance(bg_mlp, PackedMLP) and bg_mlp.in_features == 24 and MlpShape.of(bg_mlp) == MlpShape(32, 64, 1, 0, 6, 16)
                  and bg_mlp.output_dim == 3 and isinstance(enc_dir, SHEncoder) and enc_dir.degree == 4 and _on("FOC_FUSED_BG"))
    bg_radius = getattr(model, "bg_radius", 0)
    occ_common = field and tail and same_activation and _on("FOC_FUSED_OCC")
    native_common = infer and getattr(model, "density_scale", 1) == 1 and plain_grid and _on("FOC_RENDER_NATIVE")
    normals = (hash_grid and plain_grid and enc.offsets.numel() == 17 and sigma_32_64 and sigma_16 and sigma.activation == 0
               and 1 <= sigma.num_layers <= 3 and _on("FOC_FUSED_NORMALS"))
    return FieldPlan(
        grid=grid, levels=enc.offsets.numel() - 1 if grid is not None else 0, sigma=sigma, colour=colour, uses_object_feature=obj,
        field=field, tail=tail, infer=infer,
        train_forward=(field and tail and whole_field and sigma.output_activation == 6 and get_option("FOC_FIELD_FWD_FUSED") != 0),
        occ=occ_common and not obj and (bg_radius <= 0 or background),
        native_loop=native_common and not obj,
        head=both and colour.input_dim == colour_in and colour_rows and pad == 0 and _on("FOC_FUSED_HEAD"), colour_input_pad=pad,
        background=background,
        occ_object=occ_common and obj and whole_field and bg_radius <= 0,
        native_loop_object=native_common and obj and bg_radius <= 0,
        normals=normals)


def _raw_stream_of(device):
    from ._lib import raw_stream
    return raw_stream(device.index if device.index is not None else torch.cuda.current_device())


_half_scope = None


class half_cache_scope:

    def __enter__(self):
        global _half_scope
        self._outer = _half_scope
        if _half_scope is None:
            _half_scope = {}
        return self

    def __exit__(self, *exc):
        global _half_scope
        _half_scope = self._outer
        return False


def _half_of(param):
    if param.dtype == torch.half:
        return param.contiguous()
    if _half_scope is None:
        return param.detach().to(torch.half).contiguous()
    hit = _half_scope.get(id(param))
    if hit is not None and hit[0] is param and hit[1].device == param.device:
        if hit[2] is not None and _raw_stream_of(param.device) != hit[3]:
            torch.cuda.current_stream(param.device).wait_event(hit[2])
        return hit[1]
    h = param.detach().to(torch.half).contiguous()
    ev = st = None
    if h.is_cuda:
        st = _raw_stream_of(h.device)
        ev = torch.cuda.Event()
        ev.record(torch.cuda.current_stream(h.device))
    _half_scope[id(param)] = (param, h, ev, st)
    return h


def scope_cached(key, owner, make):
    if _half_scope is None:
        return make()
    hit = _half_scope.get(key)
    if hit is not None and hit[0] is owner:
        if hit[2] is not None and _raw_stream_of(hit[1].device) != hit[3]:
            torch.cuda.current_stream(hit[1].device).wait_event(hit[2])
        return hit[1]
    v = make()
    ev = st = None
    if v.is_cuda:
        st = _raw_stream_of(v.device)
        ev = torch.cuda.Event()
        ev.record(torch.cuda.current_stream(v.device))
    _half_scope[key] = (owner, v, ev, st)
    return v


def _check_colour_branch(colour, B):
    cweights, shape, ray_sh, T, c_width, obj_feat = colour[:6]
    T = int(T)
    if not (ray_sh.dtype == torch.half and ray_sh.dim() == 2 and ray_sh.shape[1] == 16 and ray_sh.is_contiguous() and T > 0
            and B == ray_sh.shape[0] * T):
        raise RuntimeError(f"hashgrid_mlp colour branch: ray_sh must be a contiguous half [B / T, 16] tensor with B = {B}, T = {T}; got "
                           f"{tuple(ray_sh.shape)} {ray_sh.dtype}{'' if ray_sh.is_contiguous() else ' (strided)'}")
    if c_width not in (4, 16):
        raise RuntimeError(f"hashgrid_mlp colour branch: c_width must be 4 or 16, got {c_width}")
    if shape.input_dim not in (32, 48) or (obj_feat is not None) != (shape.input_dim == 48) or (obj_feat is not None and obj_feat.numel() != 16):
        raise RuntimeError(f"hashgrid_mlp colour branch: a {shape.input_dim}-wide colour input takes "
                           f"{'a 16-element object feature' if shape.input_dim == 48 else 'no object feature'}, got "
                           f"{'none' if obj_feat is None else f'{obj_feat.numel()} elements'}")
    if cweights.numel() != 64 * (shape.input_dim + 64 * (shape.num_layers - 1) + 16):
        raise RuntimeError(f"hashgrid_mlp colour branch: the colour weights hold {cweights.numel()} elements, a {shape.input_dim}-wide "
                           f"{shape.num_layers}-layer network has {64 * (shape.input_dim + 64 * (shape.num_layers - 1) + 16)}")


class _hashgrid_mlp(Function):
    @staticmethod
    @custom_fwd(device_type="cuda")
    def forward(ctx, x, embeddings, weights, offsets, grid, sigma, training, colour=None):
        x = x.contiguous().float()
        B = x.shape[0]
        if colour is not None:
            _check_colour_branch(colour, B)
        S, H, (gridtype, align_corners, interp) = grid.log2_scale, grid.base_resolution, grid.tail()
        L = offsets.shape[0] - 1
        emb = _half_of(embeddings)
        w = _half_of(weights)
        enc = torch.empty(L, B, 2, device=x.device, dtype=torch.half)
        ticket = _gridencoder.grid_encode_forward_counted(x, emb, offsets, enc, B, 3, 2, L, S, H, gridtype, align_corners, interp,
                                                          standalone=_gridencoder.precount_standalone()) if training else None
        if ticket is None:
            _gridencoder.grid_encode_forward(x, emb, offsets, enc, B, 3, 2, L, S, H, None, gridtype, align_corners, interp)
        h = torch.empty(B, 16, device=x.device, dtype=torch.half)
        c = None
        if colour is not None:
            from ._lib import ptr, stream_of, check
            cweights, cshape, ray_sh, T, c_width, obj_feat = colour[:6]
            pad = float(colour[6]) if len(colour) > 6 else 0.0
            wc = _half_of(cweights)
            obj16 = object_feature_half(obj_feat, "hashgrid_mlp colour branch")
            c = torch.empty(B, c_width, device=x.device, dtype=torch.half)
            args = (ptr(enc), ptr(w), sigma.num_layers, ptr(ray_sh), int(T), ptr(wc), int(cshape.num_layers), 64, int(sigma.activation), B, ptr(h),
                    ptr(c), int(c_width), ptr(obj16))
            fn, extra = pad_twin("foc_field_forward_train", pad, obj16 is not None)
            check(fn(*args, *extra, stream_of(enc)), "field_forward_train")
        else:
            _ffmlp.ffmlp_forward_planar(enc, w, B, sigma.input_dim, 16, sigma.hidden_dim, sigma.num_layers, sigma.activation, sigma.output_activation, h)
        if training:
            ctx.save_for_backward(x, emb, w, offsets, enc)
            ctx.cfg = (grid, sigma, B, L)
            ctx.ticket = ticket
        if c is None:
            return h
        ctx.mark_non_differentiable(c)
        ctx.set_materialize_grads(False)
        return h, c

    @staticmethod
    @custom_bwd(device_type="cuda")
    def backward(ctx, grad_h, _grad_c=None):
        x, emb, w, offsets, enc = ctx.saved_tensors
        grid, sigma, B, L = ctx.cfg
        if grad_h is None:
            return (None,) * 8
        grad_h = grad_h.contiguous().half()
        g_enc = torch.empty_like(enc)
        g_w = torch.empty_like(w)
        _ffmlp.ffmlp_backward_planar(grad_h, enc, w, B, sigma.input_dim, 16, sigma.hidden_dim, sigma.num_layers, sigma.activation,
                                     sigma.output_activation, True, g_enc, g_w)
        g_emb = torch.zeros_like(emb)
        _gridencoder.grid_encode_backward(g_enc, x, emb, offsets, g_emb, B, 3, 2, L, grid.log2_scale, grid.base_resolution, None, None, *grid.tail(),
                                          grad_bl=False, precount=ctx.ticket)
        return None, g_emb, g_w, None, None, None, None, None


@torch.no_grad()
def field_infer(model, xn, dirs, dir_div=1, dir_block=0, obj_feat=None):
    from ._lib import ptr, stream_of, check
    enc, sn, cn = model.encoder, fused_mlp(model, "sigma_net"), fused_mlp(model, "color_net")
    grid = enc.spec()
    xn = xn.contiguous().float()
    dirs = dirs.contiguous().float()
    M = xn.shape[0]
    L = enc.offsets.shape[0] - 1
    emb, ws, wc = _half_of(enc.embeddings), _half_of(sn.weights), _half_of(cn.weights)
    planes = torch.empty(L, M, 2, device=xn.device, dtype=torch.half)
    _gridencoder.grid_encode_forward(xn, emb, enc.offsets, planes, M, 3, 2, L, grid.log2_scale, grid.base_resolution, None, *grid.tail())
    sigma = torch.empty(M, dtype=torch.float32, device=xn.device)
    rgb = torch.empty(M, 3, dtype=torch.float32, device=xn.device)
    obj16 = None
    if getattr(model, "uses_object_feature", False):
        if obj_feat is None:
            raise RuntimeError("field_infer: an object-conditioned network needs its encoded object feature")
        obj16 = object_feature_half(obj_feat, "field_infer")
    args = (ptr(planes), 1, ptr(dirs), int(dir_div), int(dir_block), dirs.shape[0], ptr(ws), sn.num_layers, ptr(wc), cn.num_layers, 64, sn.activation, M,
            ptr(sigma), ptr(rgb), ptr(obj16))
    fn, extra = pad_twin("foc_nerf_field_inference", float(getattr(model, "colour_input_pad", 0.0)), obj16 is not None)
    check(fn(*args, *extra, stream_of(xn)), "nerf_field_inference")
    return sigma, rgb


def hashgrid_mlp(encoder, mlp, x, bound=1, colour=None):
# ... 9 lines not shown
```

focnerf_amd/fixedstep.py:

```python
import torch
from torch.autograd import Function

from . import raymarching
from ._lib import lib, ptr, stream_of, check
from .gridencoder import grid_encode


RAY_BLOCK = 64


def ray_block_default():
    import os
    return RAY_BLOCK if os.environ.get("FOC_RAY_BLOCK", str(RAY_BLOCK)) != "0" else 0


def blocked_rows(N, T, ray_block):
    return N * T if not ray_block else -(-N // ray_block) * ray_block * T


def fixed_sample(rays_o, rays_d, nears, fars, aabb, noise, T, bound, want_xyzs=False, want_ray_sh=False, ray_block=0):
    N = rays_o.shape[0]
    dev = rays_o.device
    rows = blocked_rows(N, T, ray_block)
    enc_in = torch.empty(rows, 3, dtype=torch.float32, device=dev)
    xyzs = torch.empty(rows, 3, dtype=torch.float32, device=dev) if want_xyzs else None
    ray_sh = torch.empty(N, 16, dtype=torch.float16, device=dev) if want_ray_sh else None
    check(lib.foc_fixed_sample(ptr(rays_o), ptr(rays_d), ptr(nears), ptr(fars), ptr(aabb), ptr(noise), N, T, float(bound), ptr(xyzs), ptr(enc_in),
                               ptr(ray_sh), int(ray_block), stream_of(rays_o)), "fixed_sample")
    if want_ray_sh:
        return enc_in, xyzs, ray_sh
    return enc_in, xyzs


def ray_sh_rows(rays_d):
    rays_d = rays_d.contiguous().float()
    N, dev = rays_d.shape[0], rays_d.device
    zeros, ones = torch.zeros(N, device=dev), torch.ones(N, device=dev)
    aabb = torch.tensor([-1., -1., -1., 1., 1., 1.], device=dev)
    return fixed_sample(torch.zeros_like(rays_d), rays_d, zeros, ones, aabb, None, 2, 1.0, want_ray_sh=True)[2]


class _density_head(Function):

    @staticmethod
    def forward(ctx, h, rays_d, nears, fars, noise, N, T, density_scale, obj_feat=None):
        from .field import object_feature_half
        h = h.contiguous()
        assert h.dtype == torch.float16 and h.shape == (N * T, 16)
        dev = h.device
        M = N * T
        sigma = torch.empty(M, dtype=torch.float32, device=dev)
        trans = torch.empty(M, dtype=torch.float32, device=dev)
        weights = torch.empty(M, dtype=torch.float32, device=dev)
        ws = torch.empty(N, dtype=torch.float32, device=dev)
        depth = torch.empty(N, dtype=torch.float32, device=dev)
        width = 32 if obj_feat is None else 48
        obj_feat = object_feature_half(obj_feat, "_density_head")
        cin = torch.empty(M, width, dtype=torch.float16, device=dev)
        check(lib.foc_fixed_head_forward(ptr(h), ptr(rays_d), ptr(nears), ptr(fars), ptr(noise), N, T, float(density_scale), ptr(sigma), ptr(trans),
                                         ptr(weights), ptr(ws), ptr(depth), ptr(cin), ptr(obj_feat), width, stream_of(h)), "fixed_head_forward")
        ctx.save_for_backward(h, sigma, trans, nears, fars, noise if noise is not None else torch.empty(0, device=dev))
        ctx.has_noise = noise is not None
        ctx.dims = (N, T, float(density_scale))
        ctx.width = width
# ... 29 lines not shown
        image = torch.empty(N, 3, dtype=torch.float32, device=c.device)
        check(lib.foc_fixed_composite_forward(ptr(c), ptr(weights), ptr(bg_ray), float(bg_scalar), N, T, float(thresh), ptr(image), stream_of(c)),
              "fixed_composite_forward")
        ctx.bg_grad = bg_ray is not None and ctx.needs_input_grad[2]
        if ctx.bg_grad and weights_sum is None:
            raise RuntimeError("_fixed_composite: a background that needs a gradient needs weights_sum")
        empty = torch.empty(0, device=c.device)
        ctx.save_for_backward(c, weights, bg_ray if bg_ray is not None else empty, weights_sum.detach() if ctx.bg_grad else empty)
        ctx.has_bg = bg_ray is not None
        ctx.dims = (N, T, float(thresh), float(bg_scalar))
        return image

    @staticmethod
    def backward(ctx, g_image):
        c, weights, bg_ray, weights_sum = ctx.saved_tensors
        N, T, thresh, bg_scalar = ctx.dims
        bg_ray = bg_ray if ctx.has_bg else None
        g_image = g_image.contiguous().float()
        grad_c = torch.empty_like(c)
        grad_w = torch.empty_like(weights)
        check(lib.foc_fixed_composite_backward(ptr(g_image), ptr(c), ptr(weights), ptr(bg_ray), bg_scalar, N, T, thresh, ptr(grad_c), ptr(grad_w),
                                               stream_of(c)), "fixed_composite_backward")
        g_bg = g_image * (1 - weights_sum).unsqueeze(-1) if ctx.bg_grad else None
        return grad_c, grad_w, g_bg, None, None, None, None, None


_C_WIDTH = 4


class _render_tail(Function):

    @staticmethod
    def forward(ctx, h, cweights, ray_sh, nears, fars, noise, bg_ray, bg_scalar, N, T, density_scale, thresh, num_layers, activation, obj_feat=None,
                want_sumsq=False, c_pre=None, w16_pre=None, input_pad=0.0, want_dist=False):
        from .field import _half_of, pad_twin, object_feature_half
        h = h.contiguous()
        assert h.dtype == torch.float16 and h.shape == (N * T, 16)
        assert ray_sh.dtype == torch.float16 and ray_sh.shape == (N, 16) and ray_sh.is_contiguous()
        dev, M = h.device, N * T
        st = stream_of(h)
        w16 = w16_pre if w16_pre is not None else _half_of(cweights)
        obj16 = object_feature_half(obj_feat, "_render_tail")
        assert obj16 is None or w16.numel() == 64 * (48 + 64 * (int(num_layers) - 1) + 16)
        if c_pre is not None:
            assert c_pre.dtype == torch.float16 and c_pre.shape == (M, _C_WIDTH) and c_pre.is_contiguous()
            c = c_pre
        else:
            c = torch.empty(M, _C_WIDTH, dtype=torch.float16, device=dev)
            args = (ptr(h), ptr(ray_sh), T, ptr(w16), M, 64, int(num_layers), int(activation), ptr(c), _C_WIDTH, ptr(obj16))
            fn, extra = pad_twin("foc_color_head_forward", input_pad, obj16 is not None)
            check(fn(*args, *extra, st), "color_head_forward")
        sigma = torch.empty(M, dtype=torch.float32, device=dev)
        trans = torch.empty(M, dtype=torch.float32, device=dev)
        weights = torch.empty(M, dtype=torch.float32, device=dev)
        ws = torch.empty(N, dtype=torch.float32, device=dev)
        depth = torch.empty(N, dtype=torch.float32, device=dev)
        image = torch.empty(N, 3, dtype=torch.float32, device=dev)
        sumsq = torch.empty(N, dtype=torch.float32, device=dev) if want_sumsq else None
        tail = (ptr(h), ptr(c), ptr(nears), ptr(fars), ptr(noise), ptr(bg_ray), float(bg_scalar), N, T, float(density_scale), float(thresh), ptr(sigma),
                ptr(trans), ptr(weights), ptr(ws), ptr(depth), ptr(image), _C_WIDTH, ptr(sumsq))
        dist = wm = None
        if want_dist:
            dist, wm = torch.empty(N, dtype=torch.float32, device=dev), torch.empty(N, dtype=torch.float32, device=dev)
            check(lib.foc_fixed_tail_forward_dist(*tail, ptr(dist), ptr(wm), st), "fixed_tail_forward_dist")
        else:
            check(lib.foc_fixed_tail_forward(*tail, st), "fixed_tail_forward")
        empty = torch.empty(0, device=dev)
        ctx.bg_grad = bg_ray is not None and ctx.needs_input_grad[6]
        ctx.save_for_backward(h, w16, sigma, trans, weights, c, ray_sh, nears, fars, noise if noise is not None else empty,
                              bg_ray if bg_ray is not None else empty, obj16 if obj16 is not None else empty,
                              ws if ctx.bg_grad or want_dist else empty, wm if want_dist else empty)
        ctx.outputs = (bool(want_sumsq), bool(want_dist))
        ctx.flags = (noise is not None, bg_ray is not None, obj16 is not None, obj_feat.dtype if obj_feat is not None else None,
                     tuple(obj_feat.shape) if obj_feat is not None else None)
        ctx.dims = (N, T, float(density_scale), float(thresh), float(bg_scalar), int(num_layers), int(activation), float(input_pad))
        ctx.mark_non_differentiable(sigma, weights, c)
        ctx.set_materialize_grads(False)
        return (image, ws, depth, sigma, weights, c) + ((sumsq,) if want_sumsq else ()) + ((dist,) if want_dist else ())

    @staticmethod
    def backward(ctx, g_image, g_ws, g_depth, _g_sigma, _g_weights, _g_c, *g_extra):
        from .backend import _scratch
        from .field import pad_twin
        h, w16, sigma, trans, weights, c, ray_sh, nears, fars, noise, bg_ray, obj16, ws, wm = ctx.saved_tensors
        g_extra = list(g_extra)
        g_sumsq = g_extra.pop(0) if ctx.outputs[0] else None
        g_dist = g_extra.pop(0) if ctx.outputs[1] else None
        has_noise, has_bg, has_obj, obj_dtype, obj_shape = ctx.flags
        obj16 = obj16 if has_obj else None
        N, T, ds, thresh, bg_scalar, num_layers, activation, input_pad = ctx.dims
        noise = noise if has_noise else None
        bg_ray = bg_ray if has_bg else None
        dev, M = h.device, N * T
        st = stream_of(h)
        g_image = g_image.contiguous().float() if g_image is not None else torch.zeros(N, 3, dtype=torch.float32, device=dev)
        g_ws = g_ws.contiguous().float() if g_ws is not None else None
        g_depth = g_depth.contiguous().float() if g_depth is not None else None
        g_sumsq = g_sumsq.contiguous().float() if g_sumsq is not None else None
        grad_c = torch.empty_like(c)
        grad_h0 = torch.empty(M, dtype=torch.float16, device=dev)
        if g_dist is not None:
            g_dist = g_dist.contiguous().float()
            check(lib.foc_fixed_tail_backward_dist(ptr(g_image), ptr(g_ws), ptr(g_depth), ptr(c), ptr(sigma), ptr(trans), ptr(weights), ptr(ws), ptr(nears),
                                                   ptr(fars), ptr(noise), ptr(bg_ray), bg_scalar, N, T, ds, thresh, ptr(grad_c), ptr(grad_h0), _C_WIDTH,
                                                   ptr(g_sumsq), ptr(wm), None, ptr(g_dist), st), "fixed_tail_backward_dist")
        else:
            check(lib.foc_fixed_tail_backward(ptr(g_image), ptr(g_ws), ptr(g_depth), ptr(c), ptr(sigma), ptr(trans), ptr(weights), ptr(nears), ptr(fars),
                                              ptr(noise), ptr(bg_ray), bg_scalar, N, T, ds, thresh, ptr(grad_c), ptr(grad_h0), _C_WIDTH, ptr(g_sumsq), st),
                  "fixed_tail_backward")
        grad_h = torch.empty_like(h)
        g_w = torch.empty_like(w16)
        wsb = _scratch.get("ffmlp_ws", lib.foc_ffmlp_backward_workspace_bytes(48 if has_obj else 32, 64, num_layers), dev)
        g_obj32 = torch.empty(16, dtype=torch.float32, device=dev) if has_obj and ctx.needs_input_grad[14] else None
        args = (ptr(grad_c), ptr(h), ptr(ray_sh), T, ptr(grad_h0), ptr(w16), M, 64, num_layers, activation, ptr(grad_h), ptr(g_w), ptr(wsb),
                wsb.numel(), _C_WIDTH, ptr(obj16), ptr(g_obj32))
        fn, extra = pad_twin("foc_color_head_backward", input_pad, has_obj)
        check(fn(*args, *extra, st), "color_head_backward")
        g_obj = g_obj32.to(obj_dtype).view(obj_shape) if g_obj32 is not None else None
        g_bg = g_image * (1 - ws).unsqueeze(-1) if ctx.bg_grad else None
        return (grad_h, g_w, None, None, None, None, g_bg) + (None,) * 7 + (g_obj, None, None, None, None, None)


class _masked_norm(Function):

    @staticmethod
    def forward(ctx, sumsq, outside):
        crit = torch.sqrt((sumsq * outside).sum())
        ctx.save_for_backward(crit, outside)
        return crit

    @staticmethod
    def backward(ctx, g):
        crit, outside = ctx.saved_tensors
        coef = torch.where(crit > 0, g / (2 * crit), torch.zeros_like(crit))
        return outside * coef, None


def _unfused_distortion(weights, nears, fars, noise, N, T):
    from .loss import ray_distortion
    span = (fars - nears).unsqueeze(-1)
    z = span * torch.linspace(0.0, 1.0, T, device=weights.device).unsqueeze(0)
    if noise is not None:
        z = z + (noise.view(N, T) - 0.5) * (span / T)
    delta = torch.cat([z[:, 1:] - z[:, :-1], span / T], dim=-1)
    live = (fars > nears).unsqueeze(-1)
    zero = torch.zeros_like(z)
    return ray_distortion(torch.where(live, weights.view(N, T), zero), torch.where(live, z + 0.5 * delta, zero), torch.where(live, delta, zero))


def _background(bg_color, N, dev):
    if bg_color is None:
        return None, 1.0
    if torch.is_tensor(bg_color):
        if bg_color.numel() > 1:
            return bg_color.to(dev, torch.float32).reshape(-1, 3).expand(N, 3).contiguous(), 0.0
        return None, float(bg_color)
    return None, float(bg_color)


def render_fixed_steps(model, rays_o, rays_d, yolo_details=None, num_steps=512, bg_color=None, perturb=False, weight_thresh=1e-10,
                       return_fields=None, _out=None, distortion=False, **kwargs):
    import time
    if return_fields is None:
        return_fields = not model.training
    t_start = time.time()
    prefix = rays_o.shape[:-1]
    rays_o = rays_o.contiguous().view(-1, 3).float()
    rays_d = rays_d.contiguous().view(-1, 3).float()
    N, T = rays_o.shape[0], int(num_steps)
    dev = rays_o.device
    aabb = model.aabb_train if model.training else model.aabb_infer
    nears, fars = raymarching.near_far_from_aabb(rays_o, rays_d, aabb, model.min_near)
    noise = torch.rand(N * T, dtype=torch.float32, device=dev) if perturb else None
    from .field import field_plan, field_infer
    plan = field_plan(model)
    if getattr(model, "bg_radius", 0) > 0:
        bg_color = model._background_colour(rays_o, rays_d, bg_color)
    want_tail = plan.tail and model.training and torch.is_grad_enabled()
    fused_infer = not torch.is_grad_enabled() and plan.infer
    if distortion and not torch.is_grad_enabled():
        raise ValueError("render_fixed_steps: distortion=True needs the training route (gradients enabled): the inference paths form no "
                         "differentiable weights; call it under torch.enable_grad() with model.train()")
    rb = ray_block_default() if fused_infer else 0
    enc_in, _, ray_sh = fixed_sample(rays_o, rays_d, nears, fars, aabb, noise, T, model.bound, want_ray_sh=True) if want_tail else \
        fixed_sample(rays_o, rays_d, nears, fars, aabb, noise, T, model.bound, ray_block=rb) + (None,)

    if fused_infer:
        obj_feat = model.encode_object_feature(yolo_details, dev) if plan.uses_object_feature else None
        sigma, rgb = field_infer(model, enc_in, rays_d, dir_div=T, dir_block=rb, obj_feat=obj_feat)
        bg_ray, bg_scalar = _background(bg_color, N, dev)
        direct = (_out is not None and _out[0].dtype == torch.float32 and _out[1].dtype == torch.float32 and _out[0].is_contiguous()
                  and _out[1].is_contiguous() and _out[0].numel() == N and _out[1].numel() == 3 * N and _out[0].device == dev)
        depth, image = (_out[0].view(N), _out[1].view(N, 3)) if direct else (torch.empty(N, dtype=torch.float32, device=dev),
                                                                              torch.empty(N, 3, dtype=torch.float32, device=dev))
        weights_sum = torch.empty(N, dtype=torch.float32, device=dev)
        rgb_masked = densities = None
        if return_fields:
            if direct and len(_out) == 4 and all(t.dtype == torch.float32 and t.is_contiguous() and t.device == dev for t in _out[2:]) \
                    and _out[2].numel() == N * T and _out[3].numel() == 3 * N * T and rb:
                densities, rgb_masked = _out[2].view(N * T), _out[3].view(N * T, 3)
            else:
                rgb_masked = torch.empty(N * T, 3, dtype=torch.float32, device=dev)
                densities = torch.empty(N * T, dtype=torch.float32, device=dev) if rb else None
        check(lib.foc_fixed_render_inference(ptr(sigma), ptr(rgb), ptr(nears), ptr(fars), ptr(noise), ptr(bg_ray), float(bg_scalar), N, T,
                                             float(model.density_scale), float(weight_thresh), ptr(image), ptr(depth), ptr(weights_sum), ptr(rgb_masked),
                                             rb, ptr(densities), stream_of(sigma)), "fixed_render_inference")
        t_mid = time.time()
        results = {'depth': depth.view(*prefix), 'image': image.view(*prefix, 3), 'weights_sum': weights_sum, 'criterion_outside_mask': None,
                   'timing': [t_mid - t_start, time.time() - t_mid]}
        if return_fields:
            results['densities'] = (densities if rb else sigma).view(N, T, 1)
            results['rgbs'] = rgb_masked.view(N, T, 3)
        return results

    enc = model.encoder
    from .field import hashgrid_mlp, fused_mlp
    c_pre = obj_feat = None
    cweights = fused_mlp(model, "color_net").weights if want_tail else None
    with torch.autocast("cuda", dtype=torch.float16):
        if plan.uses_object_feature:
            obj_feat = model.encode_object_feature(yolo_details, dev)
        if plan.field:
            colour = wc16 = None
            if want_tail and plan.train_forward:
                from .field import _half_of
                wc16 = _half_of(cweights)
                colour = (wc16, plan.colour, ray_sh, T, _C_WIDTH, obj_feat, plan.colour_input_pad)
            h = hashgrid_mlp(enc, fused_mlp(model, "sigma_net"), enc_in, None, colour)
            if colour is not None:
                h, c_pre = h
        else:
            feats = grid_encode(enc_in, enc.embeddings, enc.offsets, enc.per_level_scale, enc.base_resolution, False, enc.gridtype_id,
                                enc.align_corners, enc.interp_id)
            h = fused_mlp(model, "sigma_net")(feats)
        if h.shape[1] != 16:
            raise RuntimeError("render_fixed_steps expects a 16-wide sigma head (1 + geo_feat_dim = 16)")
        fused_tail = want_tail
        want_crit = model.training and yolo_details is not None and yolo_details[0] is not None
        criterion_outside_mask = None
        if fused_tail:
            cn = fused_mlp(model, "color_net")
            bg_ray, bg_scalar = _background(bg_color, N, dev)
            outs = _render_tail.apply(h, cweights, ray_sh, nears, fars, noise, bg_ray, bg_scalar, N, T, model.density_scale, weight_thresh,
                                      cn.num_layers, cn.activation, obj_feat, want_crit and yolo_details[0].numel() == N, c_pre,
                                      wc16 if c_pre is not None else None, plan.colour_input_pad, *((True,) if distortion else ()))
            image, weights_sum, depth, sigma, weights, c = outs[:6]
            ray_dist = outs[-1] if distortion else None
            if len(outs) - bool(distortion) == 7:
                criterion_outside_mask = _masked_norm.apply(outs[6], (~yolo_details[0].reshape(N)).to(torch.float32))
        else:
            weights, weights_sum, depth, sigma, cin = _density_head.apply(h, rays_d, nears, fars, noise, N, T, model.density_scale, obj_feat)
            if plan.colour_input_pad != 0:
                cin = torch.cat([cin[:, :-1], cin.new_full((cin.shape[0], 1), plan.colour_input_pad)], dim=1)
            if distortion:
                ray_dist = _unfused_distortion(weights, nears, fars, noise, N, T)
        if want_crit and criterion_outside_mask is None:
            from .activation import trunc_exp
            criterion_outside_mask = torch.norm(trunc_exp(h[:, 0]).view(N, T)[~yolo_details[0].squeeze(0)] - 0)
        if not fused_tail:
            c = fused_mlp(model, "color_net").forward_padded(cin)
    t_mid = time.time()

    if not fused_tail:
        bg_ray, bg_scalar = _background(bg_color, N, dev)
        image = _fixed_composite.apply(c, weights, bg_ray, bg_scalar, N, T, weight_thresh, weights_sum)

    results = {'depth': depth.view(*prefix), 'image': image.view(*prefix, 3), 'weights_sum': weights_sum,
               'criterion_outside_mask': criterion_outside_mask, 'timing': [t_mid - t_start, time.time() - t_mid]}
    if distortion:
        results['distortion'] = ray_dist.view(*prefix)
    if return_fields:
        from .head import rgb_head
        c16 = c.detach()
        if c16.shape[1] != 16:
            c16 = torch.nn.functional.pad(c16, (0, 16 - c16.shape[1]))
        rgb = rgb_head(c16) * (weights > weight_thresh).unsqueeze(-1)
        results['densities'] = sigma.view(N, T, 1)
        results['rgbs'] = rgb.view(N, T, 3)
# ... 51 lines not shown
```

include/focnerf.h:

```cpp
#ifndef FOCNERF_H
#define FOCNERF_H

#include <stddef.h>
#include <stdint.h>

#ifdef __cplusplus
extern "C" {
#endif

#define FOC_OK            0
#define FOC_E_INVALID     1
#define FOC_E_DTYPE       2
#define FOC_E_LAUNCH      3

#define FOC_F32 0
#define FOC_F16 1

#define FOC_ABI_VERSION 2
int         foc_abi_version(void);
const char *foc_last_error(void);
int foc_set_option(const char *name, int value);
int foc_get_option(const char *name, int *value);
int foc_guard_pick_device(int stream_is_null, int stream_device, int pointer_device, int current_device);
const char *foc_arch(void);
// ... 196 lines not shown
                           uint32_t B, uint32_t hidden_dim, uint32_t num_layers, uint32_t activation,
                           void *outputs, uint32_t out_width, const void *obj_feat, void *stream);
int foc_color_head_backward(const void *grad, const void *h, const void *ray_sh, uint32_t samples_per_ray,
                            const void *grad_h0, const void *weights, uint32_t B, uint32_t hidden_dim,
                            uint32_t num_layers, uint32_t activation, void *grad_h, void *grad_weights,
                            void *workspace, uint64_t workspace_bytes, uint32_t out_width, const void *obj_feat, float *grad_obj, void *stream);
int foc_color_head_forward_pad(const void *h, const void *ray_sh, uint32_t samples_per_ray, const void *weights,
                               uint32_t B, uint32_t hidden_dim, uint32_t num_layers, uint32_t activation,
                               void *outputs, uint32_t out_width, const void *obj_feat, float input_pad, void *stream);
int foc_color_head_backward_pad(const void *grad, const void *h, const void *ray_sh, uint32_t samples_per_ray,
                                const void *grad_h0, const void *weights, uint32_t B, uint32_t hidden_dim,
                                uint32_t num_layers, uint32_t activation, void *grad_h, void *grad_weights,
                                void *workspace, uint64_t workspace_bytes, uint32_t out_width, const void *obj_feat, float *grad_obj,
                                float input_pad, void *stream);
int foc_color_head_forward_pad31(const void *h, const void *ray_sh, uint32_t samples_per_ray, const void *weights,
                                 uint32_t B, uint32_t hidden_dim, uint32_t num_layers, uint32_t activation,
                                 void *outputs, uint32_t out_width, const void *obj_feat, float input_pad, void *stream);
int foc_color_head_backward_pad31(const void *grad, const void *h, const void *ray_sh, uint32_t samples_per_ray,
                                  const void *grad_h0, const void *weights, uint32_t B, uint32_t hidden_dim,
                                  uint32_t num_layers, uint32_t activation, void *grad_h, void *grad_weights,
                                  void *workspace, uint64_t workspace_bytes, uint32_t out_width, const void *obj_feat, float *grad_obj,
                                  float input_pad, void *stream);

int foc_field_forward_train(const void *planes, const void *sigma_weights, uint32_t sigma_layers, const void *ray_sh, uint32_t samples_per_ray,
                            const void *color_weights, uint32_t color_layers, uint32_t hidden_dim, uint32_t activation, uint32_t B,
                            void *h, void *c, uint32_t out_width, const void *obj_feat, void *stream);
int foc_field_forward_train_pad(const void *planes, const void *sigma_weights, uint32_t sigma_layers, const void *ray_sh, uint32_t samples_per_ray,
                                const void *color_weights, uint32_t color_layers, uint32_t hidden_dim, uint32_t activation, uint32_t B,
                                void *h, void *c, uint32_t out_width, const void *obj_feat, float input_pad, void *stream);
int foc_field_forward_train_pad31(const void *planes, const void *sigma_weights, uint32_t sigma_layers, const void *ray_sh, uint32_t samples_per_ray,
                                  const void *color_weights, uint32_t color_layers, uint32_t hidden_dim, uint32_t activation, uint32_t B,
                                  void *h, void *c, uint32_t out_width, const void *obj_feat, float input_pad, void *stream);

int foc_allocate_splitk(uint64_t size);
int foc_free_splitk(void);


int foc_combine_select(const float *dens, const float *rgb, float *max_dens, float *best_rgb,
                       uint64_t n, void *stream);

int foc_combine_pack_keys(const float *dens, uint32_t rank, uint64_t *keys, uint64_t n, void *stream);
int foc_combine_unpack(const uint64_t *keys, uint32_t rank, const float *rgb,
                       float *max_dens, float *masked_rgb, uint64_t n, void *stream);

int foc_composite_fixed_steps(const float *sigmas, const float *rgbs, const float *nears,
                              const float *fars, uint32_t N, uint32_t T, float bg,
                              float *image4, float *depth, void *stream);

#define FOC_COMBINE_MAX_OBJECTS 16

int foc_combine_select_composite(const float *const *fields4, uint32_t K, const float *nears, const float *fars,
                                 uint32_t N, uint32_t T, const float *bgs, uint32_t n_bg, float *image4, float *depth,
                                 float *merged4, void *stream);

int foc_combine_select4(const float *field4, float *acc4, uint64_t n, void *stream);

int foc_combine_select_composite_attr(const float *const *fields4, uint32_t K, const uint8_t *const *id_planes,
                                      const uint32_t *ids, uint32_t n_obj, const float *nears, const float *fars,
                                      uint32_t N, uint32_t T, const float *bgs, uint32_t n_bg, float *image4, float *depth,
                                      float *merged4, float *obj_weights, float *obj_depth, int32_t *instance,
                                      uint8_t *winner, void *stream);

typedef struct FocCulledField {
    const uint64_t *mask;
    const uint32_t *offsets;
    const float *sigma_c;
    const float *rgb_c;
    uint32_t m_occ;
    float density_scale;
    float thresh;
    float sigma_gain;
} FocCulledField;
int foc_combine_select_composite_culled(const FocCulledField *objs, uint32_t K, uint32_t struct_bytes, const uint32_t *ids,
                                        uint32_t n_obj, const float *nears, const float *fars, uint32_t N, uint32_t T,
                                        const float *bgs, uint32_t n_bg, float *image4, float *depth, float *merged4,
                                        float *obj_weights, float *obj_depth, int32_t *instance, uint8_t *winner, void *stream);

int foc_combine_select4_ids(const float *field4, uint32_t id, float *acc4, uint8_t *acc_ids, uint64_t n, void *stream);

int foc_mo_select(const void *sigma_new, const void *feat_new, void *sigma_best, void *feat_best, uint64_t n,
                  uint32_t feat_width, uint32_t elem_bytes, void *stream);


int foc_fixed_sample(const float *rays_o, const float *rays_d, const float *nears, const float *fars,
                     const float *aabb, const float *noise, uint32_t N, uint32_t T, float bound,
                     float *xyzs, float *enc_in, void *ray_sh, uint32_t ray_block, void *stream);

int foc_fixed_head_forward(const void *h, const float *rays_d, const float *nears, const float *fars,
                           const float *noise, uint32_t N, uint32_t T, float density_scale,
                           float *sigma, float *trans, float *weights, float *weights_sum, float *depth,
                           void *cin, const void *obj_feat, uint32_t cin_width, void *stream);
int foc_fixed_head_backward(const void *h, const float *sigma, const float *trans, const float *nears,
                            const float *fars, const float *noise, const float *grad_w, const float *grad_ws,
                            const float *grad_depth, const void *grad_cin, uint32_t N, uint32_t T,
                            float density_scale, void *grad_h, uint32_t cin_width, void *stream);

int foc_fixed_tail_forward(const void *h, const void *c, const float *nears, const float *fars, const float *noise,
                           const float *bg_ray, float bg_scalar, uint32_t N, uint32_t T, float density_scale, float thresh,
                           float *sigma, float *trans, float *weights, float *weights_sum, float *depth, float *image,
                           uint32_t c_width, float *ray_sumsq, void *stream);
int foc_fixed_tail_backward(const float *grad_image, const float *grad_ws, const float *grad_depth, const void *c,
                            const float *sigma, const float *trans, const float *weights, const float *nears,
                            const float *fars, const float *noise, const float *bg_ray, float bg_scalar, uint32_t N,
                            uint32_t T, float density_scale, float thresh, void *grad_c, void *grad_h0, uint32_t c_width,
                            const float *grad_sumsq, void *stream);

int foc_occ_tail_forward(const void *h, const void *c, uint32_t c_width, const float *deltas, const int32_t *rays,
                         uint32_t M, uint32_t N, float T_thresh, float density_scale, const float *bg_ray, float bg_scalar,
                         const float *nears, const float *fars, float *weights_sum, float *image_raw, float *image,
                         float *depth, void *stream);
int foc_occ_tail_backward(const float *grad_image, const float *grad_ws, const void *h, const void *c, uint32_t c_width,
                          const float *deltas, const int32_t *rays, const int32_t *counter, const float *weights_sum,
                          const float *image_raw, uint32_t M, uint32_t N, float T_thresh, float density_scale,
                          const float *bg_ray, float bg_scalar, void *grad_c, void *grad_h0, void *stream);
int foc_occ_tail_forward_sumsq(const void *h, const void *c, uint32_t c_width, const float *deltas, const int32_t *rays,
                               uint32_t M, uint32_t N, float T_thresh, float density_scale, const float *bg_ray, float bg_scalar,
                               const float *nears, const float *fars, float *weights_sum, float *image_raw, float *image,
                               float *depth, float *ray_sumsq, void *stream);
int foc_occ_tail_backward_sumsq(const float *grad_image, const float *grad_ws, const void *h, const void *c, uint32_t c_width,
// ... 232 lines not shown
```

Baseline: 1.414 billion.

## Read fp32 weight blobs directly in MLP kernels and fuse near/far into sampling

Adds fp32-weight variants of the fused field forward, sigma MLP backward and colour head backward kernels. They convert the master fp32 weights to half while staging them into LDS and write fp32 gradients straight from the reduction, so the separate per-step half casts of weights and gradients go away. A new sampling entry point computes ray near/far inside the sampling kernel instead of a separate launch. Both are on by default through a FOC_STEP_DIRECT option. The price is more kernel instances, stricter shape requirements, and the gradient is rounded through half before being stored as fp32.

```diff
diff --git a/focnerf_amd/_lib.py b/focnerf_amd/_lib.py
--- a/focnerf_amd/_lib.py
+++ b/focnerf_amd/_lib.py
@@ -209,6 +209,7 @@
     "foc_fixed_field_pack_culled_gain": (i32, [c_vp, c_vp, c_vp, c_vp, u32, c_vp, c_vp, u32, u32, f32, f32, f32, c_vp, c_vp]),
     "foc_composite_fixed_steps":(i32, [c_vp, c_vp, c_vp, c_vp, u32, u32, f32, c_vp, c_vp, c_vp]),
     "foc_fixed_sample": (i32, [c_vp, c_vp, c_vp, c_vp, c_vp, c_vp, u32, u32, f32, c_vp, c_vp, c_vp, u32, c_vp]),
+    "foc_fixed_sample_near_far": (i32, [c_vp, c_vp, c_vp, f32, c_vp, u32, u32, f32, c_vp, c_vp, c_vp, c_vp, c_vp, u32, c_vp]),
     "foc_fixed_tail_forward": (i32, [c_vp, c_vp, c_vp, c_vp, c_vp, c_vp, f32, u32, u32, f32, f32, c_vp, c_vp, c_vp, c_vp, c_vp, c_vp, u32, c_vp, c_vp]),
     "foc_fixed_tail_backward": (i32, [c_vp, c_vp, c_vp, c_vp, c_vp, c_vp, c_vp, c_vp, c_vp, c_vp, c_vp, f32, u32, u32, f32, f32, c_vp, c_vp, u32, c_vp, c_vp]),
     "foc_fixed_tail_forward_dist": (i32, [c_vp, c_vp, c_vp, c_vp, c_vp, c_vp, f32, u32, u32, f32, f32, c_vp, c_vp, c_vp, c_vp, c_vp, c_vp, u32, c_vp, c_vp,
@@ -226,6 +227,9 @@
     "foc_color_head_forward_pad31": (i32, [c_vp, c_vp, u32, c_vp, u32, u32, u32, u32, c_vp, u32, c_vp, f32, c_vp]),
     "foc_color_head_backward_pad31": (i32, [c_vp, c_vp, c_vp, u32, c_vp, c_vp, u32, u32, u32, u32, c_vp, c_vp, c_vp, u64, u32, c_vp, c_vp, f32, c_vp]),
     "foc_field_forward_train_pad31": (i32, [c_vp, c_vp, u32, c_vp, u32, c_vp, u32, u32, u32, u32, c_vp, c_vp, u32, c_vp, f32, c_vp]),
+    "foc_field_forward_train_w32": (i32, [c_vp, c_vp, u32, u64, c_vp, u32, u32, c_vp, u32, u64, u32, u32, u32, c_vp, c_vp, u32, c_vp]),
+    "foc_ffmlp_backward_planar_w32": (i32, [c_vp, c_vp, c_vp, u64, u32, u32, u32, u32, u32, c_vp, c_vp, c_vp, u64, c_vp]),
+    "foc_color_head_backward_w32": (i32, [c_vp, c_vp, c_vp, u32, u32, c_vp, c_vp, u64, u32, u32, u32, u32, c_vp, c_vp, c_vp, u64, u32, c_vp]),
     "foc_fixed_composite_forward": (i32, [c_vp, c_vp, c_vp, f32, u32, u32, f32, c_vp, c_vp]),
     "foc_fixed_composite_backward": (i32, [c_vp, c_vp, c_vp, c_vp, f32, u32, u32, f32, c_vp, c_vp, c_vp]),
     "foc_sample_head_forward": (i32, [c_vp, c_vp, u64, c_vp, c_vp, c_vp, u32, c_vp]),
@@ -308,6 +312,24 @@
     return call
 
 
+class _BlobForm:
+    """Type of `W32`."""
+
+
+W32 = _BlobForm()
+W32_FORMS = {"foc_field_forward_train": "foc_field_forward_train_w32", "foc_ffmlp_backward_planar": "foc_ffmlp_backward_planar_w32",
+             "foc_color_head_backward": "foc_color_head_backward_w32"}
+
+
+def _two_forms(f16, f32):
+    def call(*args):
+        if args and args[0] is W32:
+            return f32(*args[1:])
+        return f16(*args)
+    call.__name__ = getattr(f16, "__name__", "foc_call")
+    return call
+
+
 class _Lib:
 
     def __init__(self, cdll):
@@ -315,6 +337,8 @@
         for name, (_, args) in SIGNATURES.items():
             fn = getattr(cdll, name)
             setattr(self, name, _on_tensor_device(fn) if args and args[-1] is c_vp and not name.endswith("_bytes") else fn)
+        for name, form in W32_FORMS.items():
+            setattr(self, name, _two_forms(getattr(self, name), getattr(self, form)))
 
 
 lib = _Lib(_load())
diff --git a/focnerf_amd/csrc/combine.hip b/focnerf_amd/csrc/combine.hip
--- a/focnerf_amd/csrc/combine.hip
+++ b/focnerf_amd/csrc/combine.hip
@@ -383,7 +383,7 @@
 static FocOptionRow foc_option_table[FOC_OPT_COUNT] = {
     {"FOC_MLP_BWD_FUSED", 1}, {"FOC_FIELD_FWD_FUSED", 1}, {"FOC_GB_MERGE_MAX_RES", 480}, {"FOC_GB_FACTORED", 1}, {"FOC_GB_TAIL_SPLIT", 16}, {"FOC_GRID_FUSE_SMALL", 1},
     {"FOC_GRID_PAIRS", 1}, {"FOC_GRID_FAST", 1}, {"FOC_MARCH_SERIAL", -1}, {"FOC_MARCH_RAYS_ROW_MAX", 131072}, {"FOC_OCC_MARCH_FORM", -1},
-    {"FOC_OCC_SAMPLE_MAJOR", 1}, {"FOC_OCC_FIELD_PIECE", 1 << 23}, {"FOC_DETERMINISTIC", 0},
+    {"FOC_OCC_SAMPLE_MAJOR", 1}, {"FOC_OCC_FIELD_PIECE", 1 << 23}, {"FOC_DETERMINISTIC", 0}, {"FOC_STEP_DIRECT", 1},
 };
 static int foc_option_parse(int which, const char *text) {
     if (which == FOC_OPT_OCC_MARCH_FORM) {
diff --git a/focnerf_amd/csrc/common.h b/focnerf_amd/csrc/common.h
--- a/focnerf_amd/csrc/common.h
+++ b/focnerf_amd/csrc/common.h
@@ -25,6 +25,7 @@
     FOC_OPT_OCC_SAMPLE_MAJOR,
     FOC_OPT_OCC_FIELD_PIECE,
     FOC_OPT_DETERMINISTIC,
+    FOC_OPT_STEP_DIRECT,
     FOC_OPT_COUNT
 };
 int foc_opt(FocOpt which);
diff --git a/focnerf_amd/csrc/ffmlp.hip b/focnerf_amd/csrc/ffmlp.hip
--- a/focnerf_amd/csrc/ffmlp.hip
+++ b/focnerf_amd/csrc/ffmlp.hip
@@ -357,7 +357,7 @@
     }
 }
 
-template <int HIDDEN, int NL, int NB, bool RECOMP, int IMODE, bool RELU_CT, bool IN32 = false, bool LEAN = false>
+template <int HIDDEN, int NL, int NB, bool RECOMP, int IMODE, bool RELU_CT, bool IN32 = false, bool LEAN = false, bool W32 = false>
 __global__ void __launch_bounds__(MLP_BLOCK, 2) k_mlp_bwd_fused(const _Float16 *__restrict__ grad, const _Float16 *__restrict__ inputs,
                                                              const _Float16 *__restrict__ weights, const _Float16 *__restrict__ fwd_buf,
                                                              _Float16 *__restrict__ bwd_buf_arg, _Float16 *__restrict__ grad_inputs, float *__restrict__ ws,
@@ -379,15 +379,17 @@
     bool col31_set = false;
     _Float16 col31 = (_Float16)0.0f;
     if constexpr (HEAD) { col31_set = head_bias(hd); col31 = has_obj ? (_Float16)1.0f : (_Float16)hd.pad; }
-    stage_weights_bwd<HIDDEN>(weights, lds, in_dim, NL, with_dx, HEAD, ld0);
+    if constexpr (W32) stage_weights_bwd<HIDDEN>(reinterpret_cast<const float *>(weights), lds, in_dim, NL, with_dx, HEAD, ld0);
+    else stage_weights_bwd<HIDDEN>(weights, lds, in_dim, NL, with_dx, HEAD, ld0);
     const uint32_t WA = (in_dim > (uint32_t)HIDDEN ? in_dim : (uint32_t)(HIDDEN < 32 ? 32 : HIDDEN)) + 8;
     _Float16 *sD = lds + lds_w_halfs;
     _Float16 *sA = sD + 4 * RW * WD;
     _Float16 *ldsF = sA + 4 * RW * WA;
     const float *obj_bias = reinterpret_cast<const float *>(ldsF + (size_t)(((HIDDEN + 31) / 32) * (in_dim / 16) + (NL - 1) * ((HIDDEN + 31) / 32) * (HIDDEN / 16)) * 512);
     if constexpr (RECOMP) {
-        stage_weights_fwd<HIDDEN>(weights, ldsF, in_dim, NL, false, ld0);
-        if constexpr (HEAD) { if (head_bias(hd)) stage_head_bias(weights, hd, const_cast<float *>(obj_bias), HIDDEN); }
+        if constexpr (W32) stage_weights_fwd<HIDDEN>(reinterpret_cast<const float *>(weights), ldsF, in_dim, NL, false, ld0);
+        else stage_weights_fwd<HIDDEN>(weights, ldsF, in_dim, NL, false, ld0);
+        if constexpr (HEAD && !W32) { if (head_bias(hd)) stage_head_bias(weights, hd, const_cast<float *>(obj_bias), HIDDEN); }
     }
     __syncthreads();
 
@@ -788,7 +790,7 @@
     }
 }
 
-template <int HIDDEN>
+template <int HIDDEN, bool F32R = false>
 __global__ void __launch_bounds__(1024) k_mlp_dw_reduce(const float *__restrict__ slots, uint32_t n_slots, uint32_t NL, uint32_t in_dim, uint32_t ld0,
                                                         _Float16 *__restrict__ gw, float *__restrict__ wsb) {
     __shared__ float part[16][64];
@@ -820,7 +822,8 @@
         const uint64_t first = (uint64_t)HIDDEN * ld0, lsz = (uint64_t)HIDDEN * HIDDEN;
         const uint32_t fl = NL - s;
         const uint64_t off = (s == 0 ? first + (uint64_t)(NL - 1) * lsz : (fl == 0 ? 0 : first + (uint64_t)(fl - 1) * lsz)) + (uint64_t)o * (s == NL ? ld0 : IN) + i;
-        if (wsb) wsb[off] = v; else gw[off] = (_Float16)v;
+        if constexpr (F32R) wsb[off] = (float)(_Float16)v;
+        else if (wsb) wsb[off] = v; else gw[off] = (_Float16)v;
     }
 }
 
@@ -1164,7 +1167,7 @@
     return FOC_E_INVALID;
 }
 
-template <int HIDDEN, int NL>
+template <int HIDDEN, int NL, bool W32 = false>
 static int mlp_bwd_fused_launch(const void *grad, const void *inputs, const void *weights, const void *fwd_buf, uint32_t B, uint32_t in_dim, int relu,
                                 void *bwd_buf, void *grad_inputs, void *grad_weights, float *ws, int planar, hipStream_t st, const MlpHead *head = nullptr,
                                 float *grad_obj = nullptr) {
@@ -1201,6 +1204,17 @@
                                                        : k_mlp_bwd_fused<HIDDEN, NL, NB, true, 2, false>);
     }
     else FOC_REQUIRE(!head, FOC_E_INVALID, "color_head_backward: hidden_dim must be 64 and num_layers 2 or 3");
+    if constexpr (W32) {
+        static_assert(HIDDEN == 64 && NL >= 1 && NL <= 3, "the fp32-blob instances are built for 64 neurons and 1..3 layers");
+        FOC_REQUIRE(recomp && lean && relu && in_dim == 32 && (head ? (!head_bias(*head) && head->out_width == 4u) : planar != 0), FOC_E_INVALID,
+                    "ffmlp_backward(w32): built for relu, 32 inputs, input gradients and no stored buffers; the sigma network planar, the colour head "
+                    "with [B,4] gradients and no object feature or pad");
+        if constexpr (NL >= 2) kern = head ? k_mlp_bwd_fused<HIDDEN, NL, NB, true, 3, true, false, true, true> : k_mlp_bwd_fused<HIDDEN, NL, NB, true, 1, true, true, true, true>;
+        else {
+            FOC_REQUIRE(!head, FOC_E_INVALID, "color_head_backward_w32: num_layers must be 2 or 3");
+            kern = k_mlp_bwd_fused<HIDDEN, NL, NB, true, 1, true, true, true, true>;
+        }
+    }
     if (lds_launch > 64 * 1024) (void)hipFuncSetAttribute(reinterpret_cast<const void *>(kern), hipFuncAttributeMaxDynamicSharedMemorySize, (int)lds_launch);
     const uint32_t n_w = HIDDEN * ((has_obj ? HEAD_OBJ_LD : in_dim) + HIDDEN * (NL - 1) + 16);
     uint32_t grid = foc_div_up(B, 4 * RW);
@@ -1211,8 +1225,12 @@
                        (const _Float16 *)fwd_buf, (_Float16 *)bwd_buf, (_Float16 *)grad_inputs, slots, B, in_dim, relu, (uint32_t)(lds_w / sizeof(_Float16)),
                        head ? *head : MlpHead{nullptr, nullptr, 1u, 16u, nullptr, 0.0f});
     FOC_CHECK_LAUNCH("ffmlp_backward(fused)");
-    hipLaunchKernelGGL((k_mlp_dw_reduce<HIDDEN>), dim3((NL + 1) * 64), dim3(1024), 0, st, (const float *)slots, grid, (uint32_t)NL, in_dim,
-                       has_obj ? (uint32_t)HEAD_OBJ_LD : in_dim, (_Float16 *)grad_weights, has_obj ? ws : (float *)nullptr);
+    if constexpr (W32)
+        hipLaunchKernelGGL((k_mlp_dw_reduce<HIDDEN, true>), dim3((NL + 1) * 64), dim3(1024), 0, st, (const float *)slots, grid, (uint32_t)NL, in_dim, in_dim,
+                           (_Float16 *)nullptr, (float *)grad_weights);
+    else
+        hipLaunchKernelGGL((k_mlp_dw_reduce<HIDDEN>), dim3((NL + 1) * 64), dim3(1024), 0, st, (const float *)slots, grid, (uint32_t)NL, in_dim,
+                           has_obj ? (uint32_t)HEAD_OBJ_LD : in_dim, (_Float16 *)grad_weights, has_obj ? ws : (float *)nullptr);
     FOC_CHECK_LAUNCH("ffmlp_backward(reduce)");
     if (has_obj) {
         hipLaunchKernelGGL(k_mlp_dw_finalize_obj, dim3(foc_grid_1d(n_w, 256)), dim3(256), 0, st, ws, (_Float16 *)grad_weights, n_w, (uint32_t)HIDDEN,
@@ -1535,6 +1553,60 @@
                                workspace_bytes, out_width, obj_feat, grad_obj, input_pad, true, stream);
 }
 
+static int mlp_w32_check(const char *who, const void *weights, const void *grad_weights, uint64_t weight_elems, uint32_t hidden_dim, uint32_t num_layers,
+                         uint32_t min_layers, uint32_t activation, const void *workspace, uint64_t workspace_bytes) {
+    FOC_REQUIRE(hidden_dim == 64 && activation == FOC_ACT_RELU && num_layers >= min_layers && num_layers <= 3, FOC_E_INVALID,
+                "%s: built for hidden_dim 64, relu(0) and %u..3 layers (got %u, %u, %u)", who, min_layers, hidden_dim, activation, num_layers);
+    FOC_REQUIRE(weight_elems == 64ull * (32 + 64 * (num_layers - 1) + 16), FOC_E_INVALID, "%s: a blob of %llu elements, %u layers of 64 on 32 inputs hold %llu",
+                who, (unsigned long long)weight_elems, num_layers, 64ull * (32 + 64 * (num_layers - 1) + 16));
+    FOC_REQUIRE(weights && grad_weights && workspace, FOC_E_INVALID, "%s: null pointer", who);
+    FOC_REQUIRE((((uintptr_t)weights | (uintptr_t)grad_weights) & 15) == 0, FOC_E_INVALID, "%s: the weight and gradient blobs must be 16-byte aligned", who);
+    FOC_REQUIRE(workspace_bytes >= foc_ffmlp_backward_workspace_bytes(32, 64, num_layers), FOC_E_INVALID,
+                "%s: workspace of %llu bytes, foc_ffmlp_backward_workspace_bytes(32, 64, %u) asks for %llu", who, (unsigned long long)workspace_bytes, num_layers,
+                (unsigned long long)foc_ffmlp_backward_workspace_bytes(32, 64, num_layers));
+    return FOC_OK;
+}
+
+int foc_ffmlp_backward_planar_w32(const void *grad, const void *inputs_planar, const float *weights, uint64_t weight_elems, uint32_t B, uint32_t input_dim,
+                                  uint32_t hidden_dim, uint32_t num_layers, uint32_t activation, void *grad_inputs_planar, float *grad_weights,
+                                  void *workspace, uint64_t workspace_bytes, void *stream) {
+    FocDeviceGuard foc_guard_(stream, grad);
+    FOC_REQUIRE(input_dim == 32, FOC_E_INVALID, "ffmlp_backward_planar_w32: input_dim must be 32 (got %u)", input_dim);
+    int rc = mlp_w32_check("ffmlp_backward_planar_w32", weights, grad_weights, weight_elems, hidden_dim, num_layers, 1, activation, workspace, workspace_bytes);
+    if (rc) return rc;
+    hipStream_t st = (hipStream_t)stream;
+    if (B == 0) {
+        if (foc_zero_async(grad_weights, weight_elems * sizeof(float), st) != hipSuccess) { foc_set_error("ffmlp_backward_planar_w32: memset failed"); return FOC_E_LAUNCH; }
+        return FOC_OK;
+    }
+    FOC_REQUIRE(grad && inputs_planar && grad_inputs_planar, FOC_E_INVALID, "ffmlp_backward_planar_w32: null pointer");
+    switch (num_layers) {
+        case 1: return mlp_bwd_fused_launch<64, 1, true>(grad, inputs_planar, weights, nullptr, B, 32, 1, nullptr, grad_inputs_planar, grad_weights, (float *)workspace, 1, st);
+        case 2: return mlp_bwd_fused_launch<64, 2, true>(grad, inputs_planar, weights, nullptr, B, 32, 1, nullptr, grad_inputs_planar, grad_weights, (float *)workspace, 1, st);
+        default: return mlp_bwd_fused_launch<64, 3, true>(grad, inputs_planar, weights, nullptr, B, 32, 1, nullptr, grad_inputs_planar, grad_weights, (float *)workspace, 1, st);
+    }
+}
+
+int foc_color_head_backward_w32(const void *grad, const void *h, const void *ray_sh, uint32_t ray_sh_rows, uint32_t samples_per_ray, const void *grad_h0,
+                                const float *weights, uint64_t weight_elems, uint32_t B, uint32_t hidden_dim, uint32_t num_layers, uint32_t activation,
+                                void *grad_h, float *grad_weights, void *workspace, uint64_t workspace_bytes, uint32_t out_width, void *stream) {
+    FocDeviceGuard foc_guard_(stream, grad);
+    int rc = mlp_w32_check("color_head_backward_w32", weights, grad_weights, weight_elems, hidden_dim, num_layers, 2, activation, workspace, workspace_bytes);
+    if (rc) return rc;
+    FOC_REQUIRE(out_width == 4, FOC_E_INVALID, "color_head_backward_w32: built for [B,4] output gradients (out_width 4, got %u)", out_width);
+    FOC_REQUIRE(samples_per_ray >= 1 && (uint64_t)ray_sh_rows * samples_per_ray == B, FOC_E_INVALID,
+                "color_head_backward_w32: B = %u is not ray_sh_rows %u x samples_per_ray %u", B, ray_sh_rows, samples_per_ray);
+    hipStream_t st = (hipStream_t)stream;
+    if (B == 0) {
+        if (foc_zero_async(grad_weights, weight_elems * sizeof(float), st) != hipSuccess) { foc_set_error("color_head_backward_w32: memset failed"); return FOC_E_LAUNCH; }
+        return FOC_OK;
+    }
+    FOC_REQUIRE(grad && h && ray_sh && grad_h, FOC_E_INVALID, "color_head_backward_w32: null pointer");
+    const MlpHead hd{(const _Float16 *)ray_sh, (const _Float16 *)grad_h0, samples_per_ray, out_width, nullptr, 0.0f};
+    if (num_layers == 2) return mlp_bwd_fused_launch<64, 2, true>(grad, h, weights, nullptr, B, 32, 1, nullptr, grad_h, grad_weights, (float *)workspace, 0, st, &hd, nullptr);
+    return mlp_bwd_fused_launch<64, 3, true>(grad, h, weights, nullptr, B, 32, 1, nullptr, grad_h, grad_weights, (float *)workspace, 0, st, &hd, nullptr);
+}
+
 int foc_allocate_splitk(uint64_t size) { (void)size; return FOC_OK; }
 int foc_free_splitk(void) { return FOC_OK; }
 
diff --git a/focnerf_amd/csrc/field_fwd.hip b/focnerf_amd/csrc/field_fwd.hip
--- a/focnerf_amd/csrc/field_fwd.hip
+++ b/focnerf_amd/csrc/field_fwd.hip
@@ -11,7 +11,7 @@
 #ifndef FF_MIN_WAVES
 #define FF_MIN_WAVES 2
 #endif
-template <int NLS, int NLC, bool RELU>
+template <int NLS, int NLC, bool RELU, bool W32 = false>
 __global__ void __launch_bounds__(MLP_BLOCK, FF_MIN_WAVES) k_field_fwd_train(const _Float16 *__restrict__ planes, const _Float16 *__restrict__ w_sigma,
                                                                const _Float16 *__restrict__ w_color, _Float16 *__restrict__ h_out,
                                                                _Float16 *__restrict__ c_out, uint32_t B, MlpHead hd) {
@@ -21,9 +21,14 @@
     extern __shared__ __attribute__((aligned(16))) _Float16 lds[];
     _Float16 *ldsS = lds, *ldsC = lds + FS * 512;
     const float *obj_bias = reinterpret_cast<const float *>(ldsC + FC * 512);
-    stage_weights_fwd<HIDDEN>(w_sigma, ldsS, 32, NLS);
-    stage_weights_fwd<HIDDEN>(w_color, ldsC, 32, NLC, true, head_ld0(hd));
-    if (head_bias(hd)) stage_head_bias(w_color, hd, const_cast<float *>(obj_bias), HIDDEN);
+    if constexpr (W32) {
+        stage_weights_fwd<HIDDEN>(reinterpret_cast<const float *>(w_sigma), ldsS, 32, NLS);
+        stage_weights_fwd<HIDDEN>(reinterpret_cast<const float *>(w_color), ldsC, 32, NLC, true, head_ld0(hd));
+    } else {
+        stage_weights_fwd<HIDDEN>(w_sigma, ldsS, 32, NLS);
+        stage_weights_fwd<HIDDEN>(w_color, ldsC, 32, NLC, true, head_ld0(hd));
+        if (head_bias(hd)) stage_head_bias(w_color, hd, const_cast<float *>(obj_bias), HIDDEN);
+    }
     __syncthreads();
 
     const uint32_t lane = threadIdx.x & 63, wave = threadIdx.x >> 6;
@@ -146,9 +151,9 @@
     return (uint32_t)n;
 }
 
-template <int NLS, int NLC, bool RELU>
+template <int NLS, int NLC, bool RELU, bool W32 = false>
 static int ff_launch(const void *planes, const void *w_sigma, const void *w_color, void *h, void *c, uint32_t B, const MlpHead &hd, hipStream_t st) {
-    auto kern = k_field_fwd_train<NLS, NLC, RELU>;
+    auto kern = k_field_fwd_train<NLS, NLC, RELU, W32>;
     const size_t lds = (size_t)((4 + (NLS - 1) * 8 + 4) + (4 + (NLC - 1) * 8 + 4)) * 1024 + 256;
     if (lds > 64 * 1024) (void)hipFuncSetAttribute(reinterpret_cast<const void *>(kern), hipFuncAttributeMaxDynamicSharedMemorySize, (int)lds);
     static int resident = 0;
@@ -195,7 +200,45 @@
     }
 }
 
+static int field_forward_train_w32(const void *planes, const float *sigma_weights, uint32_t sigma_layers, uint64_t sigma_weight_elems, const void *ray_sh,
+                                   uint32_t ray_sh_rows, uint32_t samples_per_ray, const float *color_weights, uint32_t color_layers,
+                                   uint64_t color_weight_elems, uint32_t hidden_dim, uint32_t activation, uint32_t B, void *h, void *c, uint32_t out_width,
+                                   void *stream) {
+    FocDeviceGuard foc_guard_(stream, planes);
+    const char *who = "field_forward_train_w32";
+    FOC_REQUIRE(hidden_dim == 64 && activation == FOC_ACT_RELU, FOC_E_INVALID, "%s: built for hidden_dim 64 and relu(0) (got %u, %u)", who, hidden_dim, activation);
+    FOC_REQUIRE(head_layer_pair(sigma_layers, color_layers), FOC_E_INVALID, "%s: layer counts (%u, %u) are not built (1/2, 1/3, 2/2, 2/3, 3/3)", who,
+                sigma_layers, color_layers);
+    FOC_REQUIRE(sigma_weight_elems == 64ull * (32 + 64 * (sigma_layers - 1) + 16) && color_weight_elems == 64ull * (32 + 64 * (color_layers - 1) + 16),
+                FOC_E_INVALID, "%s: blobs of %llu and %llu elements, %u and %u layers of 64 on 32 inputs hold %llu and %llu", who,
+                (unsigned long long)sigma_weight_elems, (unsigned long long)color_weight_elems, sigma_layers, color_layers,
+                64ull * (32 + 64 * (sigma_layers - 1) + 16), 64ull * (32 + 64 * (color_layers - 1) + 16));
+    FOC_REQUIRE(samples_per_ray >= 1 && (uint64_t)ray_sh_rows * samples_per_ray == B, FOC_E_INVALID, "%s: B = %u is not ray_sh_rows %u x samples_per_ray %u",
+                who, B, ray_sh_rows, samples_per_ray);
+    FOC_REQUIRE(out_width == 16 || out_width == 4, FOC_E_INVALID, "%s: out_width must be 16 or 4 (got %u)", who, out_width);
+    if (B == 0) return FOC_OK;
+    FOC_REQUIRE(planes && sigma_weights && ray_sh && color_weights && h && c, FOC_E_INVALID, "%s: null pointer", who);
+    FOC_REQUIRE((((uintptr_t)sigma_weights | (uintptr_t)color_weights) & 15) == 0, FOC_E_INVALID, "%s: the weight blobs must be 16-byte aligned", who);
+    const MlpHead hd{(const _Float16 *)ray_sh, nullptr, samples_per_ray, out_width, nullptr, 0.0f};
+    hipStream_t st = (hipStream_t)stream;
+    switch (sigma_layers * 10 + color_layers) {
+        case 12: return ff_launch<1, 2, true, true>(planes, sigma_weights, color_weights, h, c, B, hd, st);
+        case 13: return ff_launch<1, 3, true, true>(planes, sigma_weights, color_weights, h, c, B, hd, st);
+        case 22: return ff_launch<2, 2, true, true>(planes, sigma_weights, color_weights, h, c, B, hd, st);
+        case 23: return ff_launch<2, 3, true, true>(planes, sigma_weights, color_weights, h, c, B, hd, st);
+        default: return ff_launch<3, 3, true, true>(planes, sigma_weights, color_weights, h, c, B, hd, st);
+    }
+}
+
 extern "C" {
+
+int foc_field_forward_train_w32(const void *planes, const float *sigma_weights, uint32_t sigma_layers, uint64_t sigma_weight_elems, const void *ray_sh,
+                                uint32_t ray_sh_rows, uint32_t samples_per_ray, const float *color_weights, uint32_t color_layers,
+                                uint64_t color_weight_elems, uint32_t hidden_dim, uint32_t activation, uint32_t B, void *h, void *c, uint32_t out_width,
+                                void *stream) {
+    return field_forward_train_w32(planes, sigma_weights, sigma_layers, sigma_weight_elems, ray_sh, ray_sh_rows, samples_per_ray, color_weights, color_layers,
+                                   color_weight_elems, hidden_dim, activation, B, h, c, out_width, stream);
+}
 
 int foc_field_forward_train(const void *planes, const void *sigma_weights, uint32_t sigma_layers, const void *ray_sh, uint32_t samples_per_ray,
                             const void *color_weights, uint32_t color_layers, uint32_t hidden_dim, uint32_t activation, uint32_t B, void *h, void *c,
diff --git a/focnerf_amd/csrc/fixedstep.hip b/focnerf_amd/csrc/fixedstep.hip
--- a/focnerf_amd/csrc/fixedstep.hip
+++ b/focnerf_amd/csrc/fixedstep.hip
@@ -30,6 +30,39 @@
         if (ray_sh && i == 0 && own) {
             h8 lo, hi;
             foc_sh16_h(rays_d[n * 3], rays_d[n * 3 + 1], rays_d[n * 3 + 2], lo, hi);
+            h8 *dst = reinterpret_cast<h8 *>(ray_sh + (uint64_t)n * 16);
+            dst[0] = lo; dst[1] = hi;
+        }
+    }
+}
+
+__global__ void __launch_bounds__(256) k_fs_sample_nf(const float *__restrict__ rays_o, const float *__restrict__ rays_d, const float *__restrict__ aabb,
+                                                      float min_near, const float *__restrict__ noise, uint32_t N, uint32_t T, float bound,
+                                                      float *__restrict__ nears_out, float *__restrict__ fars_out, float *__restrict__ xyzs,
+                                                      float *__restrict__ enc_in, _Float16 *__restrict__ ray_sh, uint32_t ray_block) {
+    const uint32_t lane = threadIdx.x & 63;
+    const uint32_t n_rows = ray_block ? (N + FS_RAY_BLOCK - 1) / FS_RAY_BLOCK * FS_RAY_BLOCK : N;
+    const FsBox box = fs_box(aabb);
+    const float two_b = 2 * bound;
+    for (uint32_t r = blockIdx.x * 4 + (threadIdx.x >> 6); r < n_rows; r += gridDim.x * 4) {
+        const bool own = r < N;
+        const uint32_t n = own ? r : N - 1;
+        const float ox = rays_o[n * 3], oy = rays_o[n * 3 + 1], oz = rays_o[n * 3 + 2], dx = rays_d[n * 3], dy = rays_d[n * 3 + 1], dz = rays_d[n * 3 + 2];
+        float near, far;
+        rm_near_far(ox, oy, oz, dx, dy, dz, box.a0, box.a1, box.a2, box.a3, box.a4, box.a5, min_near, near, far);
+        if (lane == 0 && own) { nears_out[n] = near; fars_out[n] = far; }
+        const FsGeom g = fs_geom_of(near, far, T);
+        for (uint32_t i = lane; i < T; i += 64) {
+            const float z = fs_z(g, i, T, noise, (uint64_t)n * T + i);
+            float x, y, w;
+            fs_point(ox, oy, oz, dx, dy, dz, z, box, x, y, w);
+            const uint64_t s = ray_block ? fs_block_row(r, i, T) : (uint64_t)r * T + i;
+            if (xyzs) { xyzs[s * 3] = x; xyzs[s * 3 + 1] = y; xyzs[s * 3 + 2] = w; }
+            if (enc_in) { enc_in[s * 3] = fs_norm(x, bound, two_b); enc_in[s * 3 + 1] = fs_norm(y, bound, two_b); enc_in[s * 3 + 2] = fs_norm(w, bound, two_b); }
+        }
+        if (ray_sh && lane == 0 && own) {
+            h8 lo, hi;
+            foc_sh16_h(dx, dy, dz, lo, hi);
             h8 *dst = reinterpret_cast<h8 *>(ray_sh + (uint64_t)n * 16);
             dst[0] = lo; dst[1] = hi;
         }
@@ -405,6 +438,21 @@
     return FOC_OK;
 }
 
+int foc_fixed_sample_near_far(const float *rays_o, const float *rays_d, const float *aabb, float min_near, const float *noise, uint32_t N, uint32_t T,
+                              float bound, float *nears, float *fars, float *xyzs, float *enc_in, void *ray_sh, uint32_t ray_block, void *stream) {
+    FocDeviceGuard foc_guard_(stream, rays_o);
+    if (N == 0) return FOC_OK;
+    FOC_REQUIRE(rays_o && rays_d && nears && fars && aabb && (xyzs || enc_in), FOC_E_INVALID, "fixed_sample_near_far: null pointer");
+    FOC_REQUIRE(T >= 2, FOC_E_INVALID, "fixed_sample_near_far: T must be >= 2");
+    FOC_REQUIRE(ray_block == 0 || ray_block == FS_RAY_BLOCK, FOC_E_INVALID, "fixed_sample_near_far: ray_block must be 0 (ray-major) or %u (got %u)", FS_RAY_BLOCK,
+                ray_block);
+    const uint64_t n_rows = ray_block ? (uint64_t)foc_div_up(N, FS_RAY_BLOCK) * FS_RAY_BLOCK : N;
+    hipLaunchKernelGGL(k_fs_sample_nf, dim3(foc_grid_1d(n_rows, 4, 256 * 64)), dim3(256), 0, (hipStream_t)stream, rays_o, rays_d, aabb, min_near, noise, N, T,
+                       bound, nears, fars, xyzs, enc_in, (_Float16 *)ray_sh, ray_block);
+    FOC_CHECK_LAUNCH("fixed_sample_near_far");
+    return FOC_OK;
+}
+
 int foc_fixed_head_forward(const void *h, const float *rays_d, const float *nears, const float *fars, const float *noise, uint32_t N, uint32_t T,
                            float density_scale, float *sigma, float *trans, float *weights, float *weights_sum, float *depth, void *cin,
                            const void *obj_feat, uint32_t cin_width, void *stream) {
diff --git a/focnerf_amd/csrc/fs_common.h b/focnerf_amd/csrc/fs_common.h
--- a/focnerf_amd/csrc/fs_common.h
+++ b/focnerf_amd/csrc/fs_common.h
@@ -9,13 +9,16 @@
     return (uint64_t)(n / FS_RAY_BLOCK) * FS_RAY_BLOCK * T + (uint64_t)i * FS_RAY_BLOCK + n % FS_RAY_BLOCK;
 }
 
-__device__ __forceinline__ FsGeom fs_geom(const float *__restrict__ nears, const float *__restrict__ fars, uint32_t n, uint32_t T) {
+__device__ __forceinline__ FsGeom fs_geom_of(float near, float far, uint32_t T) {
     FsGeom g;
-    g.near = nears[n]; g.far = fars[n];
+    g.near = near; g.far = far;
     g.span = g.far - g.near;
     g.sample_dist = g.span / (float)T;
     g.step = 1.0f / (float)(T - 1);
     return g;
+}
+__device__ __forceinline__ FsGeom fs_geom(const float *__restrict__ nears, const float *__restrict__ fars, uint32_t n, uint32_t T) {
+    return fs_geom_of(nears[n], fars[n], T);
 }
 __device__ __forceinline__ float fs_z0(const FsGeom &g, uint32_t i, uint32_t T) {
     const float lin = (i < T / 2) ? (g.step * (float)i) : fmaf(-g.step, (float)(T - 1 - i), 1.0f);
diff --git a/focnerf_amd/csrc/mlp_common.h b/focnerf_amd/csrc/mlp_common.h
--- a/focnerf_amd/csrc/mlp_common.h
+++ b/focnerf_amd/csrc/mlp_common.h
@@ -156,14 +156,27 @@
     return head_shift(v, h == 0 ? nxt : 0u);
 }
 
-template <int HIDDEN>
-__device__ void stage_weights_fwd(const _Float16 *__restrict__ W, _Float16 *lds, uint32_t in_dim, uint32_t num_layers, bool with_out = true, uint32_t ld0 = 0) {
+__device__ __forceinline__ _Float16 ld_w(const _Float16 *p) { return *p; }
+__device__ __forceinline__ _Float16 ld_w(const float *p) { return (_Float16)*p; }
+__device__ __forceinline__ h4 ld_w4(const _Float16 *p) { return *reinterpret_cast<const h4 *>(p); }
+__device__ __forceinline__ h4 ld_w4(const float *p) {
+    typedef float f4 __attribute__((ext_vector_type(4)));
+    const f4 a = *reinterpret_cast<const f4 *>(p);
+    return h4{(_Float16)a.x, (_Float16)a.y, (_Float16)a.z, (_Float16)a.w};
+}
+__device__ __forceinline__ h8 ld_w8(const _Float16 *p) { return *reinterpret_cast<const h8 *>(p); }
+__device__ __forceinline__ h8 ld_w8(const float *p) {
+    const h4 lo = ld_w4(p), hi = ld_w4(p + 4);
+    return h8{lo[0], lo[1], lo[2], lo[3], hi[0], hi[1], hi[2], hi[3]};
+}
+template <int HIDDEN, typename WT = _Float16>
+__device__ void stage_weights_fwd(const WT *__restrict__ W, _Float16 *lds, uint32_t in_dim, uint32_t num_layers, bool with_out = true, uint32_t ld0 = 0) {
     constexpr int MT = (HIDDEN + 31) / 32, KC = HIDDEN / 16;
     const uint32_t KS0 = in_dim / 16;
     if (!ld0) ld0 = in_dim;
     const uint32_t n0 = MT * KS0, nh = (num_layers - 1) * MT * KC, total = n0 + nh + (with_out ? KC : 0);
-    const _Float16 *Wh = W + (size_t)HIDDEN * ld0;
-    const _Float16 *Wo = Wh + (size_t)(num_layers - 1) * HIDDEN * HIDDEN;
+    const WT *Wh = W + (size_t)HIDDEN * ld0;
+    const WT *Wo = Wh + (size_t)(num_layers - 1) * HIDDEN * HIDDEN;
     for (uint32_t idx = threadIdx.x; idx < total * 64; idx += MLP_BLOCK) {
         const uint32_t f = idx >> 6, lane = idx & 63, r = lane & 31, h = lane >> 5;
         h8 v;
@@ -171,20 +184,20 @@
         for (int j = 0; j < 8; j++) v[j] = (_Float16)0;
         if (f < n0) {
             const uint32_t mt = f / KS0, kc = f % KS0, row = 32 * mt + r;
-            if (row < HIDDEN) v = *reinterpret_cast<const h8 *>(W + (size_t)row * ld0 + 16 * kc + 8 * h);
+            if (row < HIDDEN) v = ld_w8(W + (size_t)row * ld0 + 16 * kc + 8 * h);
         } else if (f < n0 + nh) {
             const uint32_t g = f - n0, l = g / (MT * KC), mt = (g / KC) % MT, kc = g % KC, row = 32 * mt + r;
             if (row < HIDDEN) {
-                const _Float16 *p = Wh + (size_t)l * HIDDEN * HIDDEN + (size_t)row * HIDDEN + 16 * kc + 4 * h;
-                const h4 lo = *reinterpret_cast<const h4 *>(p), hi = *reinterpret_cast<const h4 *>(p + 8);
+                const WT *p = Wh + (size_t)l * HIDDEN * HIDDEN + (size_t)row * HIDDEN + 16 * kc + 4 * h;
+                const h4 lo = ld_w4(p), hi = ld_w4(p + 8);
 #pragma unroll
                 for (int j = 0; j < 4; j++) { v[j] = lo[j]; v[4 + j] = hi[j]; }
             }
         } else {
             const uint32_t kc = f - n0 - nh;
             if (r < 16) {
-                const _Float16 *p = Wo + (size_t)r * HIDDEN + 16 * kc + 4 * h;
-                const h4 lo = *reinterpret_cast<const h4 *>(p), hi = *reinterpret_cast<const h4 *>(p + 8);
+                const WT *p = Wo + (size_t)r * HIDDEN + 16 * kc + 4 * h;
+                const h4 lo = ld_w4(p), hi = ld_w4(p + 8);
 #pragma unroll
                 for (int j = 0; j < 4; j++) { v[j] = lo[j]; v[4 + j] = hi[j]; }
             }
@@ -193,15 +206,15 @@
     }
 }
 
-template <int HIDDEN>
-__device__ void stage_weights_bwd(const _Float16 *__restrict__ W, _Float16 *lds, uint32_t in_dim, uint32_t num_layers, bool with_dx, bool head = false,
+template <int HIDDEN, typename WT = _Float16>
+__device__ void stage_weights_bwd(const WT *__restrict__ W, _Float16 *lds, uint32_t in_dim, uint32_t num_layers, bool with_dx, bool head = false,
                                   uint32_t ld0 = 0) {
     constexpr int MT = (HIDDEN + 31) / 32, KC = HIDDEN / 16;
     const uint32_t MT0 = (in_dim + 31) / 32;
     if (!ld0) ld0 = in_dim;
     const uint32_t no = MT, nh = (num_layers - 1) * MT * KC, nx = with_dx ? MT0 * KC : 0, total = no + nh + nx;
-    const _Float16 *Wh = W + (size_t)HIDDEN * ld0;
-    const _Float16 *Wo = Wh + (size_t)(num_layers - 1) * HIDDEN * HIDDEN;
+    const WT *Wh = W + (size_t)HIDDEN * ld0;
+    const WT *Wo = Wh + (size_t)(num_layers - 1) * HIDDEN * HIDDEN;
     for (uint32_t idx = threadIdx.x; idx < total * 64; idx += MLP_BLOCK) {
         const uint32_t f = idx >> 6, lane = idx & 63, r = lane & 31, h = lane >> 5;
         h8 v;
@@ -211,24 +224,24 @@
             const uint32_t i = 32 * f + r;
             if (i < HIDDEN) {
 #pragma unroll
-                for (int j = 0; j < 8; j++) v[j] = Wo[(size_t)(8 * h + j) * HIDDEN + i];
+                for (int j = 0; j < 8; j++) v[j] = ld_w(Wo + (size_t)(8 * h + j) * HIDDEN + i);
             }
         } else if (f < no + nh) {
             const uint32_t g = f - no, l = g / (MT * KC), mt = (g / KC) % MT, kc = g % KC, i = 32 * mt + r;
             if (i < HIDDEN) {
 #pragma unroll
-                for (int j = 0; j < 8; j++) v[j] = Wh[(size_t)l * HIDDEN * HIDDEN + (size_t)chain_k(kc, h, j) * HIDDEN + i];
+                for (int j = 0; j < 8; j++) v[j] = ld_w(Wh + (size_t)l * HIDDEN * HIDDEN + (size_t)chain_k(kc, h, j) * HIDDEN + i);
             }
         } else {
             const uint32_t g = f - no - nh, mt0 = g / KC, kc = g % KC, i = 32 * mt0 + r;
             if (head) {
                 if (i >= 17 && i < 32) {
 #pragma unroll
-                    for (int j = 0; j < 8; j++) v[j] = W[(size_t)chain_k(kc, h, j) * ld0 + (i - 1)];
+                    for (int j = 0; j < 8; j++) v[j] = ld_w(W + (size_t)chain_k(kc, h, j) * ld0 + (i - 1));
                 }
             } else if (i < in_dim) {
 #pragma unroll
-                for (int j = 0; j < 8; j++) v[j] = W[(size_t)chain_k(kc, h, j) * ld0 + i];
+                for (int j = 0; j < 8; j++) v[j] = ld_w(W + (size_t)chain_k(kc, h, j) * ld0 + i);
             }
         }
         *reinterpret_cast<h8 *>(lds + (size_t)f * 512 + lane * 8) = v;
diff --git a/focnerf_amd/csrc/raymarching.hip b/focnerf_amd/csrc/raymarching.hip
--- a/focnerf_amd/csrc/raymarching.hip
+++ b/focnerf_amd/csrc/raymarching.hip
@@ -8,30 +8,6 @@
 #define RM_RPI   0.3183098861837907f
 
 __device__ __forceinline__ float rm_sign(float x) { return copysignf(1.0f, x); }
-
-__device__ __forceinline__ void rm_near_far(float ox, float oy, float oz, float dx, float dy, float dz, float a0, float a1, float a2, float a3, float a4, float a5,
-                                            float min_near, float &near_out, float &far_out) {
-    const float rdx = 1 / dx, rdy = 1 / dy, rdz = 1 / dz;
-    float near = (a0 - ox) * rdx, far = (a3 - ox) * rdx, t;
-    if (near > far) { t = near; near = far; far = t; }
-    float near_y = (a1 - oy) * rdy, far_y = (a4 - oy) * rdy;
-    if (near_y > far_y) { t = near_y; near_y = far_y; far_y = t; }
-    bool miss = (near > far_y || near_y > far);
-    if (!miss) {
-        if (near_y > near) near = near_y;
-        if (far_y < far) far = far_y;
-        float near_z = (a2 - oz) * rdz, far_z = (a5 - oz) * rdz;
-        if (near_z > far_z) { t = near_z; near_z = far_z; far_z = t; }
-        miss = (near > far_z || near_z > far);
-        if (!miss) {
-            if (near_z > near) near = near_z;
-            if (far_z < far) far = far_z;
-            if (near < min_near) near = min_near;
-        }
-    }
-    near_out = miss ? FLT_MAX : near;
-    far_out = miss ? FLT_MAX : far;
-}
 
 __global__ void __launch_bounds__(256) k_near_far_from_aabb(const float *__restrict__ rays_o, const float *__restrict__ rays_d,
                                      const float *__restrict__ aabb, uint32_t N, float min_near,
diff --git a/focnerf_amd/csrc/sample_math.h b/focnerf_amd/csrc/sample_math.h
--- a/focnerf_amd/csrc/sample_math.h
+++ b/focnerf_amd/csrc/sample_math.h
@@ -1,5 +1,6 @@
 #pragma once
 #include "common.h"
+#include <float.h>
 
 typedef _Float16 h8 __attribute__((ext_vector_type(8)));
 
@@ -50,3 +51,27 @@
 __device__ __forceinline__ FocBg foc_bg(const float *__restrict__ bg_ray, float bg_scalar, uint32_t k) {
     return FocBg{bg_ray ? bg_ray[k * 3] : bg_scalar, bg_ray ? bg_ray[k * 3 + 1] : bg_scalar, bg_ray ? bg_ray[k * 3 + 2] : bg_scalar};
 }
+
+__device__ __forceinline__ void rm_near_far(float ox, float oy, float oz, float dx, float dy, float dz, float a0, float a1, float a2, float a3, float a4, float a5,
+                                            float min_near, float &near_out, float &far_out) {
+    const float rdx = 1 / dx, rdy = 1 / dy, rdz = 1 / dz;
+    float near = (a0 - ox) * rdx, far = (a3 - ox) * rdx, t;
+    if (near > far) { t = near; near = far; far = t; }
+    float near_y = (a1 - oy) * rdy, far_y = (a4 - oy) * rdy;
+    if (near_y > far_y) { t = near_y; near_y = far_y; far_y = t; }
+    bool miss = (near > far_y || near_y > far);
+    if (!miss) {
+        if (near_y > near) near = near_y;
+        if (far_y < far) far = far_y;
+        float near_z = (a2 - oz) * rdz, far_z = (a5 - oz) * rdz;
+        if (near_z > far_z) { t = near_z; near_z = far_z; far_z = t; }
+        miss = (near > far_z || near_z > far);
+        if (!miss) {
+            if (near_z > near) near = near_z;
+            if (far_z < far) far = far_z;
+            if (near < min_near) near = min_near;
+        }
+    }
+    near_out = miss ? FLT_MAX : near;
+    far_out = miss ? FLT_MAX : far;
+}
diff --git a/focnerf_amd/field.py b/focnerf_amd/field.py
--- a/focnerf_amd/field.py
+++ b/focnerf_amd/field.py
@@ -54,6 +54,7 @@
     occ_object: bool = False
     native_loop_object: bool = False
     normals: bool = False
+    step_direct: bool = False
 
 
 def pad_twin(name, pad, obj):
@@ -114,17 +115,18 @@
     native_common = infer and getattr(model, "density_scale", 1) == 1 and plain_grid and _on("FOC_RENDER_NATIVE")
     normals = (hash_grid and plain_grid and enc.offsets.numel() == 17 and sigma_32_64 and sigma_16 and sigma.activation == 0
                and 1 <= sigma.num_layers <= 3 and _on("FOC_FUSED_NORMALS"))
+    train_forward = field and tail and whole_field and sigma.output_activation == 6 and get_option("FOC_FIELD_FWD_FUSED") != 0
     return FieldPlan(
         grid=grid, levels=enc.offsets.numel() - 1 if grid is not None else 0, sigma=sigma, colour=colour, uses_object_feature=obj,
-        field=field, tail=tail, infer=infer,
-        train_forward=(field and tail and whole_field and sigma.output_activation == 6 and get_option("FOC_FIELD_FWD_FUSED") != 0),
+        field=field, tail=tail, infer=infer, train_forward=train_forward,
         occ=occ_common and not obj and (bg_radius <= 0 or background),
         native_loop=native_common and not obj,
         head=both and colour.input_dim == colour_in and colour_rows and pad == 0 and _on("FOC_FUSED_HEAD"), colour_input_pad=pad,
         background=background,
         occ_object=occ_common and obj and whole_field and bg_radius <= 0,
         native_loop_object=native_common and obj and bg_radius <= 0,
-        normals=normals)
+        normals=normals,
+        step_direct=(train_forward and sigma.activation == 0 and not obj and pad == 0 and get_option("FOC_STEP_DIRECT") != 0))
 
 
 def _raw_stream_of(device):
@@ -188,6 +190,10 @@
     return v
 
 
+def direct_blob(weights):
+    return weights.dtype == torch.float32 and weights.is_contiguous() and weights.data_ptr() % 16 == 0
+
+
 def _check_colour_branch(colour, B):
     cweights, shape, ray_sh, T, c_width, obj_feat = colour[:6]
     T = int(T)
@@ -216,8 +222,13 @@
             _check_colour_branch(colour, B)
         S, H, (gridtype, align_corners, interp) = grid.log2_scale, grid.base_resolution, grid.tail()
         L = offsets.shape[0] - 1
+        direct = colour is not None and len(colour) > 7 and bool(colour[7])
+        if direct and not (direct_blob(weights) and direct_blob(colour[0]) and sigma.activation == 0 and colour[5] is None
+                           and (len(colour) < 7 or float(colour[6]) == 0.0)):
+            raise RuntimeError("hashgrid_mlp colour branch: the direct route takes contiguous fp32 weight blobs of ReLU networks without an object "
+                               "feature or pad")
         emb = _half_of(embeddings)
-        w = _half_of(weights)
+        w = weights.detach() if direct else _half_of(weights)
         enc = torch.empty(L, B, 2, device=x.device, dtype=torch.half)
         ticket = _gridencoder.grid_encode_forward_counted(x, emb, offsets, enc, B, 3, 2, L, S, H, gridtype, align_corners, interp,
                                                           standalone=_gridencoder.precount_standalone()) if training else None
@@ -229,19 +240,27 @@
             from ._lib import ptr, stream_of, check
             cweights, cshape, ray_sh, T, c_width, obj_feat = colour[:6]
             pad = float(colour[6]) if len(colour) > 6 else 0.0
-            wc = _half_of(cweights)
-            obj16 = object_feature_half(obj_feat, "hashgrid_mlp colour branch")
             c = torch.empty(B, c_width, device=x.device, dtype=torch.half)
-            args = (ptr(enc), ptr(w), sigma.num_layers, ptr(ray_sh), int(T), ptr(wc), int(cshape.num_layers), 64, int(sigma.activation), B, ptr(h),
-                    ptr(c), int(c_width), ptr(obj16))
-            fn, extra = pad_twin("foc_field_forward_train", pad, obj16 is not None)
-            check(fn(*args, *extra, stream_of(enc)), "field_forward_train")
+            if direct:
+                from ._lib import lib, W32
+                wc = cweights.detach()
+                check(lib.foc_field_forward_train(W32, ptr(enc), ptr(w), sigma.num_layers, w.numel(), ptr(ray_sh), ray_sh.shape[0], int(T), ptr(wc),
+                                                  int(cshape.num_layers), wc.numel(), 64, int(sigma.activation), B, ptr(h), ptr(c), int(c_width),
+                                                  stream_of(enc)), "field_forward_train_w32")
+            else:
+                wc = _half_of(cweights)
+                obj16 = object_feature_half(obj_feat, "hashgrid_mlp colour branch")
+                args = (ptr(enc), ptr(w), sigma.num_layers, ptr(ray_sh), int(T), ptr(wc), int(cshape.num_layers), 64, int(sigma.activation), B, ptr(h),
+                        ptr(c), int(c_width), ptr(obj16))
+                fn, extra = pad_twin("foc_field_forward_train", pad, obj16 is not None)
+                check(fn(*args, *extra, stream_of(enc)), "field_forward_train")
         else:
             _ffmlp.ffmlp_forward_planar(enc, w, B, sigma.input_dim, 16, sigma.hidden_dim, sigma.num_layers, sigma.activation, sigma.output_activation, h)
         if training:
             ctx.save_for_backward(x, emb, w, offsets, enc)
             ctx.cfg = (grid, sigma, B, L)
             ctx.ticket = ticket
+            ctx.direct = direct
         if c is None:
             return h
         ctx.mark_non_differentiable(c)
@@ -258,8 +277,16 @@
         grad_h = grad_h.contiguous().half()
         g_enc = torch.empty_like(enc)
         g_w = torch.empty_like(w)
-        _ffmlp.ffmlp_backward_planar(grad_h, enc, w, B, sigma.input_dim, 16, sigma.hidden_dim, sigma.num_layers, sigma.activation,
-                                     sigma.output_activation, True, g_enc, g_w)
+        if ctx.direct:
+            from ._lib import lib, ptr, stream_of, check, W32
+            from .backend import _scratch
+            ws = _scratch.get("ffmlp_ws", lib.foc_ffmlp_backward_workspace_bytes(sigma.input_dim, sigma.hidden_dim, sigma.num_layers), grad_h.device)
+            check(lib.foc_ffmlp_backward_planar(W32, ptr(grad_h), ptr(enc), ptr(w), w.numel(), B, sigma.input_dim, sigma.hidden_dim, sigma.num_layers,
+                                                sigma.activation, ptr(g_enc), ptr(g_w), ptr(ws), ws.numel(), stream_of(grad_h)),
+                  "ffmlp_backward_planar_w32")
+        else:
+            _ffmlp.ffmlp_backward_planar(grad_h, enc, w, B, sigma.input_dim, 16, sigma.hidden_dim, sigma.num_layers, sigma.activation,
+                                         sigma.output_activation, True, g_enc, g_w)
         g_emb = torch.zeros_like(emb)
         _gridencoder.grid_encode_backward(g_enc, x, emb, offsets, g_emb, B, 3, 2, L, grid.log2_scale, grid.base_resolution, None, None, *grid.tail(),
                                           grad_bl=False, precount=ctx.ticket)
diff --git a/focnerf_amd/fixedstep.py b/focnerf_amd/fixedstep.py
--- a/focnerf_amd/fixedstep.py
+++ b/focnerf_amd/fixedstep.py
@@ -30,6 +30,23 @@
     if want_ray_sh:
         return enc_in, xyzs, ray_sh
     return enc_in, xyzs
+
+
+def fixed_sample_near_far(rays_o, rays_d, aabb, min_near, noise, T, bound, want_xyzs=False, want_ray_sh=False, ray_block=0):
+    N = rays_o.shape[0]
+    dev = rays_o.device
+    rows = blocked_rows(N, T, ray_block)
+    nears = torch.empty(N, dtype=torch.float32, device=dev)
+    fars = torch.empty(N, dtype=torch.float32, device=dev)
+    enc_in = torch.empty(rows, 3, dtype=torch.float32, device=dev)
+    xyzs = torch.empty(rows, 3, dtype=torch.float32, device=dev) if want_xyzs else None
+    ray_sh = torch.empty(N, 16, dtype=torch.float16, device=dev) if want_ray_sh else None
+    aabb = aabb.contiguous().float()
+    check(lib.foc_fixed_sample_near_far(ptr(rays_o), ptr(rays_d), ptr(aabb), float(min_near), ptr(noise), N, T, float(bound), ptr(nears), ptr(fars),
+                                        ptr(xyzs), ptr(enc_in), ptr(ray_sh), int(ray_block), stream_of(rays_o)), "fixed_sample_near_far")
+    if want_ray_sh:
+        return nears, fars, enc_in, xyzs, ray_sh
+    return nears, fars, enc_in, xyzs
 
 
 def ray_sh_rows(rays_d):
@@ -125,14 +142,21 @@
 
     @staticmethod
     def forward(ctx, h, cweights, ray_sh, nears, fars, noise, bg_ray, bg_scalar, N, T, density_scale, thresh, num_layers, activation, obj_feat=None,
-                want_sumsq=False, c_pre=None, w16_pre=None, input_pad=0.0, want_dist=False):
+                want_sumsq=False, c_pre=None, w16_pre=None, input_pad=0.0, want_dist=False, direct=False):
         from .field import _half_of, pad_twin, object_feature_half
         h = h.contiguous()
         assert h.dtype == torch.float16 and h.shape == (N * T, 16)
         assert ray_sh.dtype == torch.float16 and ray_sh.shape == (N, 16) and ray_sh.is_contiguous()
         dev, M = h.device, N * T
         st = stream_of(h)
-        w16 = w16_pre if w16_pre is not None else _half_of(cweights)
+        if direct:
+            from .field import direct_blob
+            if not (c_pre is not None and direct_blob(cweights) and obj_feat is None and float(input_pad) == 0.0 and int(activation) == 0):
+                raise RuntimeError("_render_tail: the direct route takes the colour logits of the fused forward and a contiguous fp32 blob of a ReLU "
+                                   "network without an object feature or pad")
+            w16 = cweights.detach()
+        else:
+            w16 = w16_pre if w16_pre is not None else _half_of(cweights)
         obj16 = object_feature_half(obj_feat, "_render_tail")
         assert obj16 is None or w16.numel() == 64 * (48 + 64 * (int(num_layers) - 1) + 16)
         if c_pre is not None:
@@ -167,6 +191,7 @@
         ctx.flags = (noise is not None, bg_ray is not None, obj16 is not None, obj_feat.dtype if obj_feat is not None else None,
                      tuple(obj_feat.shape) if obj_feat is not None else None)
         ctx.dims = (N, T, float(density_scale), float(thresh), float(bg_scalar), int(num_layers), int(activation), float(input_pad))
+        ctx.direct = bool(direct)
         ctx.mark_non_differentiable(sigma, weights, c)
         ctx.set_materialize_grads(False)
         return (image, ws, depth, sigma, weights, c) + ((sumsq,) if want_sumsq else ()) + ((dist,) if want_dist else ())
@@ -205,13 +230,18 @@
         g_w = torch.empty_like(w16)
         wsb = _scratch.get("ffmlp_ws", lib.foc_ffmlp_backward_workspace_bytes(48 if has_obj else 32, 64, num_layers), dev)
         g_obj32 = torch.empty(16, dtype=torch.float32, device=dev) if has_obj and ctx.needs_input_grad[14] else None
-        args = (ptr(grad_c), ptr(h), ptr(ray_sh), T, ptr(grad_h0), ptr(w16), M, 64, num_layers, activation, ptr(grad_h), ptr(g_w), ptr(wsb),
-                wsb.numel(), _C_WIDTH, ptr(obj16), ptr(g_obj32))
-        fn, extra = pad_twin("foc_color_head_backward", input_pad, has_obj)
-        check(fn(*args, *extra, st), "color_head_backward")
+        if ctx.direct:
+            from ._lib import W32
+            check(lib.foc_color_head_backward(W32, ptr(grad_c), ptr(h), ptr(ray_sh), N, T, ptr(grad_h0), ptr(w16), w16.numel(), M, 64, num_layers, activation,
+                                              ptr(grad_h), ptr(g_w), ptr(wsb), wsb.numel(), _C_WIDTH, st), "color_head_backward_w32")
+        else:
+            args = (ptr(grad_c), ptr(h), ptr(ray_sh), T, ptr(grad_h0), ptr(w16), M, 64, num_layers, activation, ptr(grad_h), ptr(g_w), ptr(wsb),
+                    wsb.numel(), _C_WIDTH, ptr(obj16), ptr(g_obj32))
+            fn, extra = pad_twin("foc_color_head_backward", input_pad, has_obj)
+            check(fn(*args, *extra, st), "color_head_backward")
         g_obj = g_obj32.to(obj_dtype).view(obj_shape) if g_obj32 is not None else None
         g_bg = g_image * (1 - ws).unsqueeze(-1) if ctx.bg_grad else None
-        return (grad_h, g_w, None, None, None, None, g_bg) + (None,) * 7 + (g_obj, None, None, None, None, None)
+        return (grad_h, g_w, None, None, None, None, g_bg) + (None,) * 7 + (g_obj, None, None, None, None, None, None)
 
 
 class _masked_norm(Function):
@@ -263,10 +293,12 @@
     N, T = rays_o.shape[0], int(num_steps)
     dev = rays_o.device
     aabb = model.aabb_train if model.training else model.aabb_infer
-    nears, fars = raymarching.near_far_from_aabb(rays_o, rays_d, aabb, model.min_near)
-    noise = torch.rand(N * T, dtype=torch.float32, device=dev) if perturb else None
     from .field import field_plan, field_infer
     plan = field_plan(model)
+    sample_near_far = plan.tail and plan.step_direct and model.training and torch.is_grad_enabled()
+    if not sample_near_far:
+        nears, fars = raymarching.near_far_from_aabb(rays_o, rays_d, aabb, model.min_near)
+    noise = torch.rand(N * T, dtype=torch.float32, device=dev) if perturb else None
     if getattr(model, "bg_radius", 0) > 0:
         bg_color = model._background_colour(rays_o, rays_d, bg_color)
     want_tail = plan.tail and model.training and torch.is_grad_enabled()
@@ -275,8 +307,11 @@
         raise ValueError("render_fixed_steps: distortion=True needs the training route (gradients enabled): the inference paths form no "
                          "differentiable weights; call it under torch.enable_grad() with model.train()")
     rb = ray_block_default() if fused_infer else 0
-    enc_in, _, ray_sh = fixed_sample(rays_o, rays_d, nears, fars, aabb, noise, T, model.bound, want_ray_sh=True) if want_tail else \
-        fixed_sample(rays_o, rays_d, nears, fars, aabb, noise, T, model.bound, ray_block=rb) + (None,)
+    if sample_near_far:
+        nears, fars, enc_in, _, ray_sh = fixed_sample_near_far(rays_o, rays_d, aabb, model.min_near, noise, T, model.bound, want_ray_sh=True)
+    else:
+        enc_in, _, ray_sh = fixed_sample(rays_o, rays_d, nears, fars, aabb, noise, T, model.bound, want_ray_sh=True) if want_tail else \
+            fixed_sample(rays_o, rays_d, nears, fars, aabb, noise, T, model.bound, ray_block=rb) + (None,)
 
     if fused_infer:
         obj_feat = model.encode_object_feature(yolo_details, dev) if plan.uses_object_feature else None
@@ -309,17 +344,23 @@
     enc = model.encoder
     from .field import hashgrid_mlp, fused_mlp
     c_pre = obj_feat = None
+    direct_step = False
     cweights = fused_mlp(model, "color_net").weights if want_tail else None
     with torch.autocast("cuda", dtype=torch.float16):
         if plan.uses_object_feature:
             obj_feat = model.encode_object_feature(yolo_details, dev)
         if plan.field:
             colour = wc16 = None
+            sigma_mlp = fused_mlp(model, "sigma_net")
             if want_tail and plan.train_forward:
-                from .field import _half_of
-                wc16 = _half_of(cweights)
-                colour = (wc16, plan.colour, ray_sh, T, _C_WIDTH, obj_feat, plan.colour_input_pad)
-            h = hashgrid_mlp(enc, fused_mlp(model, "sigma_net"), enc_in, None, colour)
+                from .field import _half_of, direct_blob
+                direct_step = plan.step_direct and obj_feat is None and direct_blob(cweights) and direct_blob(sigma_mlp.weights)
+                if direct_step:
+                    colour = (cweights, plan.colour, ray_sh, T, _C_WIDTH, None, 0.0, True)
+                else:
+                    wc16 = _half_of(cweights)
+                    colour = (wc16, plan.colour, ray_sh, T, _C_WIDTH, obj_feat, plan.colour_input_pad)
+            h = hashgrid_mlp(enc, sigma_mlp, enc_in, None, colour)
             if colour is not None:
                 h, c_pre = h
         else:
@@ -336,7 +377,7 @@
             bg_ray, bg_scalar = _background(bg_color, N, dev)
             outs = _render_tail.apply(h, cweights, ray_sh, nears, fars, noise, bg_ray, bg_scalar, N, T, model.density_scale, weight_thresh,
                                       cn.num_layers, cn.activation, obj_feat, want_crit and yolo_details[0].numel() == N, c_pre,
-                                      wc16 if c_pre is not None else None, plan.colour_input_pad, *((True,) if distortion else ()))
+                                      wc16 if c_pre is not None else None, plan.colour_input_pad, bool(distortion), c_pre is not None and direct_step)
             image, weights_sum, depth, sigma, weights, c = outs[:6]
             ray_dist = outs[-1] if distortion else None
             if len(outs) - bool(distortion) == 7:
diff --git a/include/focnerf.h b/include/focnerf.h
--- a/include/focnerf.h
+++ b/include/focnerf.h
@@ -252,6 +252,18 @@
                                   const void *color_weights, uint32_t color_layers, uint32_t hidden_dim, uint32_t activation, uint32_t B,
                                   void *h, void *c, uint32_t out_width, const void *obj_feat, float input_pad, void *stream);
 
+int foc_field_forward_train_w32(const void *planes, const float *sigma_weights, uint32_t sigma_layers, uint64_t sigma_weight_elems,
+                                const void *ray_sh, uint32_t ray_sh_rows, uint32_t samples_per_ray,
+                                const float *color_weights, uint32_t color_layers, uint64_t color_weight_elems,
+                                uint32_t hidden_dim, uint32_t activation, uint32_t B, void *h, void *c, uint32_t out_width, void *stream);
+int foc_ffmlp_backward_planar_w32(const void *grad, const void *inputs_planar, const float *weights, uint64_t weight_elems, uint32_t B,
+                                  uint32_t input_dim, uint32_t hidden_dim, uint32_t num_layers, uint32_t activation,
+                                  void *grad_inputs_planar, float *grad_weights, void *workspace, uint64_t workspace_bytes, void *stream);
+int foc_color_head_backward_w32(const void *grad, const void *h, const void *ray_sh, uint32_t ray_sh_rows, uint32_t samples_per_ray,
+                                const void *grad_h0, const float *weights, uint64_t weight_elems, uint32_t B, uint32_t hidden_dim,
+                                uint32_t num_layers, uint32_t activation, void *grad_h, float *grad_weights,
+                                void *workspace, uint64_t workspace_bytes, uint32_t out_width, void *stream);
+
 int foc_allocate_splitk(uint64_t size);
 int foc_free_splitk(void);
 
@@ -305,6 +317,9 @@
 int foc_fixed_sample(const float *rays_o, const float *rays_d, const float *nears, const float *fars,
                      const float *aabb, const float *noise, uint32_t N, uint32_t T, float bound,
                      float *xyzs, float *enc_in, void *ray_sh, uint32_t ray_block, void *stream);
+int foc_fixed_sample_near_far(const float *rays_o, const float *rays_d, const float *aabb, float min_near, const float *noise,
+                              uint32_t N, uint32_t T, float bound, float *nears, float *fars,
+                              float *xyzs, float *enc_in, void *ray_sh, uint32_t ray_block, void *stream);
 
 int foc_fixed_head_forward(const void *h, const float *rays_d, const float *nears, const float *fars,
                            const float *noise, uint32_t N, uint32_t T, float density_scale,
```

Result: no change. 1.412 billion, median of 2 (-0.2%).
